# Ryan-Faulkner/Simultaneous-Diffusion-for-Pointclouds

Hardware: AMD Instinct MI355X
Metric: Langevin denoising steps/sec on 64×1024 range images, 1/2/4/8 MI355X (higher is better)
Workload: dtype fp32x3; 1 GPU; Line.yml simultaneous sampling step (score-net fwd + Langevin update + consistency merge), 64x1024x2 range images; views_per_gpu=4, megabatch_views=4, mode=viewsplit, conv_arithmetic=fp32x3, parallelism=views1

## Files before the change

### include/sdp.h

```cpp
#ifndef SDP_H
#define SDP_H

#include <stddef.h>
#include <stdint.h>

#ifdef __cplusplus
extern "C" {
#endif

#define SDP_VERSION 100

enum sdp_precision {
  SDP_PREC_FP32 = 0,
  SDP_PREC_FP32X3 = 1,
  SDP_PREC_BF16 = 2
};

typedef struct sdp_net_desc {
  int ngf;
  int channels;
  int H, W;
  int num_classes;
  int precision;
} sdp_net_desc;

typedef struct sdp_net sdp_net;

int sdp_version(void);
const char* sdp_last_error(void);

int sdp_net_create(const sdp_net_desc* desc, sdp_net** out);
int sdp_net_set_param(sdp_net* net, const char* key, const float* host_data, const int64_t* shape, int ndim);
int sdp_net_finalize(sdp_net* net);
int sdp_net_workspace_size(const sdp_net* net, int B, size_t* bytes);
int sdp_net_forward(sdp_net* net, const float* x, const int64_t* labels, float* out, int B,
                    void* workspace, size_t workspace_bytes, void* stream);
int sdp_net_destroy(sdp_net* net);
typedef struct {
  const float* ref;
  const int32_t* mask;
  const float* noise;
  uint64_t seed, offset;
  float step_size, noise_scale, grad_ref;
  int nan_to_num;
  float* lik_out;
  uint32_t* absmax_bits;
  float* grad_out;
} sdp_langevin_params;
int sdp_net_forward_langevin(sdp_net* net, float* x, const int64_t* labels, int B, const sdp_langevin_params* params,
                             void* workspace, size_t workspace_bytes, void* stream);
int sdp_net_set_split(sdp_net* net, int ways);
int sdp_net_profile_enable(sdp_net* net, int enable);
int sdp_net_profile_read(sdp_net* net, char* buf, size_t cap, int* n_launches);

int sdp_net_param_arena_floats(const sdp_net* net, size_t* n);
int sdp_net_param_count(const sdp_net* net, int* n);
int sdp_net_param_info(const sdp_net* net, int i, char* key, size_t cap, size_t* offset, size_t* numel);
int sdp_net_bind_params(sdp_net* net, float* arena, void* stream);
int sdp_net_repack(sdp_net* net, void* stream);

int sdp_net_train_workspace_size(sdp_net* net, int B, size_t* bytes);
int sdp_net_set_tape(sdp_net* net, int bf16);
int sdp_net_forward_train(sdp_net* net, const float* x, const int64_t* labels, float* out, int B,
                          void* workspace, size_t workspace_bytes, void* stream);
int sdp_net_backward(sdp_net* net, const float* dscore, int B, void* workspace, size_t workspace_bytes,
                     float* grads, void* stream);
int sdp_net_backward_buckets(sdp_net* net, const float* dscore, int B, void* workspace, size_t workspace_bytes,
                             float* grads, int n_buckets, const size_t* bucket_end, void* const* events,
                             void* stream);
int sdp_dsm_loss(const float* score, const float* noise, const float* mask, const float* used_sigma, int B,
                 int n_img, float anneal_power, float* dscore, float* loss, float* loss_per, float* part,
                 void* stream);
int sdp_adam_ema_step(float* params, const float* grads, float* exp_avg, float* exp_avg_sq, float* ema_shadow,
                      size_t n, double lr, double beta1, double beta2, double eps, int step, double ema_mu,
                      void* stream);
enum sdp_optim_kind { SDP_OPTIM_ADAM = 0, SDP_OPTIM_RMSPROP = 1, SDP_OPTIM_SGD = 2 };
int sdp_optim_ema_step(int kind, float* params, const float* grads, float* state0, float* state1, float* state2,
                       float* ema_shadow, size_t n, double lr, double beta1, double beta2, double eps,
                       double weight_decay, int step, double ema_mu, void* stream);

int sdp_langevin_step(float* x, const float* grad, const float* ref, const int32_t* mask,
                      const float* noise_or_null, uint64_t seed, uint64_t offset,
                      float step_size, float noise_scale, float grad_ref, int nan_to_num,
                      int B, int C, int HW, float* lik_out, uint32_t* absmax_bits, void* stream);
int sdp_axpy_step(float* x, const float* g, float a, const float* lik, const int32_t* mask,
                  const float* ref, float b, int n, void* stream);

enum sdp_merge_variant { SDP_MERGE_POSES = 0, SDP_MERGE_ORIGINS = 1 };

typedef struct sdp_merge_params {
  int variant;
  int setting;
  float sigma;
  float allowance;
  float cc;
} sdp_merge_params;

int sdp_merge_workspace_size(int n_src, int n_out, int H, int W, size_t* bytes);
int sdp_merge_workspace_bytes(int n_src, int aB, int n_out, int H, int W, size_t* bytes);
int sdp_consistency_merge(float* x_all, int n_src, int aB, int o_begin, int n_out, int H, int W,
                          const double* toWorld, const double* fromWorld, const float* origins,
                          const uint8_t* exist, const uint8_t* sky, const int32_t* refmask,
                          const sdp_merge_params* params, const uint32_t* absmax_bits,
                          float* new_images, void* workspace, size_t workspace_bytes, void* stream);
int sdp_consistency_merge_ev(float* x_all, int n_src, int aB, int o_begin, int n_out, int H, int W,
                             const double* toWorld, const double* fromWorld, const float* origins,
                             const uint8_t* exist, const uint8_t* sky, const int32_t* refmask,
                             const sdp_merge_params* params, const uint32_t* absmax_bits,
                             float* new_images, void* workspace, size_t workspace_bytes, void* stream,
                             void* absmax_event);

int sdp_range_project_workspace_size(int H, int W, size_t* bytes);
int sdp_range_project(const double* points, int N, int stride, int has_intensity, const double* origin,
                      int H, int W, double* depth, double* intensity, uint8_t* obfuscation, uint8_t* sky,
                      int64_t* index, void* workspace, size_t workspace_bytes, void* stream);

enum sdp_view_variant { SDP_VIEW_8BATCH = 0, SDP_VIEW_ALLFORONE = 1, SDP_VIEW_DENSIFICATION = 2, SDP_VIEW_COMPLETION = 3 };
int sdp_view_transform(const float* points, int64_t n, const double* m1, const double* m2, double* out, void* stream);
int sdp_view_gather(const int64_t* index, int H, int W, int blank_cols, const float* points, double* out, int* count,
                    void* stream);
int sdp_view_finalize(const double* depth, const double* intensity, const uint8_t* obfuscation, const uint8_t* sky,
                      const double* goal_depth, const double* goal_intensity, int H, int W, int channels, int roll,
                      int variant, int first_view, double* real, uint8_t* notmask, uint8_t* notsky, double* goal,
                      void* stream);

int sdp_grid_subsample(const float* points, int64_t n, const float* features, int fdim, const int32_t* classes,
                       int ldim, float sample_dl, int method, float* out_points, float* out_features,
                       int32_t* out_classes, int64_t* out_n);

#ifdef __cplusplus
}
#endif
#endif
```

### simultaneous-diffusion-for-pointclouds_amd/csrc/aux.hip

```cpp
#include "common.h"
#include "langevin.h"

namespace sdp {

SDP_DEV float linspace01(int i, int n) {
  if (n == 1) return 0.f;
  const float step = 1.0f / (float)(n - 1);
  return i < n / 2 ? step * (float)i : 1.0f - step * (float)(n - 1 - i);
}

SDP_DEV float wave_sum(float v) {
#pragma unroll
  for (int o = 32; o > 0; o >>= 1) v += __shfl_xor(v, o);
  return v;
}

typedef float f32x2v __attribute__((ext_vector_type(2)));
typedef float f32x4v __attribute__((ext_vector_type(4)));
constexpr int BC_TP = 128, BC_RS = 132;
#ifndef SDP_BC_KO
#define SDP_BC_KO 0
#endif
constexpr int BC_WG_PER_CU = 3;
__global__ __launch_bounds__(256, BC_WG_PER_CU) void begin_conv_kernel(const float* __restrict__ x, const float* __restrict__ w,
// ... 619 lines not shown
      } else {
        if (out) *reinterpret_cast<float4*>(out + e) = g4;
        float4 l;
        const float4 o = langevin_group(lg, e / 4, g4, l);
        reinterpret_cast<float4*>(lg.x)[e / 4] = o;
        if (lg.lik) reinterpret_cast<float4*>(lg.lik)[e / 4] = l;
        if (co == 0) lmax = max(lmax, absmax4(o));
      }
    }
  }
  if constexpr (LGV) {
    if (lg.absmax) block_absmax<4>(lmax, lg.absmax);
  }
}

constexpr int INPP_CPB = 8, INPP_G = 1024 / INPP_CPB;
__global__ __launch_bounds__(1024) void inpp_moments_kernel(const float2* __restrict__ stats, int T, float cnt, int C,
                                                            double2* __restrict__ mv) {
  __shared__ double red[1024];
  const int tid = threadIdx.x, l = tid % INPP_CPB, g = tid / INPP_CPB;
  const int nb = C / INPP_CPB;
  const int b = blockIdx.x / nb, c = (blockIdx.x % nb) * INPP_CPB + l;
  const float2* st = stats + (size_t)b * T * C + c;
  auto group_sum = [&](double v) {
    red[tid] = v;
    __syncthreads();
    for (int s = INPP_G / 2; s > 0; s >>= 1) {
      if (g < s) red[tid] += red[tid + s * INPP_CPB];
      __syncthreads();
    }
    const double r = red[l];
    __syncthreads();
    return r;
  };
  double sm = 0.0;
  for (int t = g; t < T; t += INPP_G) sm += st[(size_t)t * C].x;
  const double mean = group_sum(sm) / T;
  double m2 = 0.0;
  for (int t = g; t < T; t += INPP_G) {
    const float2 v = st[(size_t)t * C];
    const double dm = (double)v.x - mean;
    m2 += (double)v.y + dm * dm * cnt;
  }
  m2 = group_sum(m2);
  if (g == 0) mv[(size_t)b * C + c] = make_double2(mean, m2 / ((double)T * cnt));
}

__global__ __launch_bounds__(1024) void inpp_ss_kernel(const double2* __restrict__ mv, int C,
                                                       const float* __restrict__ alpha, const float* __restrict__ gamma,
                                                       const float* __restrict__ beta, float2* __restrict__ ss,
                                                       float4* __restrict__ nst) {
  __shared__ double red[1024];
  const int b = blockIdx.x, c = threadIdx.x;
  const double2 m_v = mv[(size_t)b * C + c];
  const double mean = m_v.x, var = m_v.y;
  red[c] = mean;
  __syncthreads();
  for (int s = C / 2; s > 0; s >>= 1) {
    if (c < s) red[c] += red[c + s];
    __syncthreads();
  }
  const double m = red[0] / C;
  __syncthreads();
  red[c] = (mean - m) * (mean - m);
  __syncthreads();
  for (int s = C / 2; s > 0; s >>= 1) {
    if (c < s) red[c] += red[c + s];
    __syncthreads();
  }
  const double v = red[0] / (C - 1);
  const double inv = 1.0 / sqrt(var + 1e-5);
  const double mn = (mean - m) / sqrt(v + 1e-5);
  const double gm = gamma[c];
  const double scale = gm * inv;
  const double shift = gm * (-mean * inv + mn * (double)alpha[c]) + (double)beta[c];
  ss[(size_t)b * C + c] = make_float2((float)scale, (float)shift);
  if (nst) nst[(size_t)b * C + c] = make_float4((float)mean, (float)inv, (float)mn, (float)(1.0 / sqrt(v + 1e-5)));
}

#ifndef SDP_MP_MIN_BLOCKS
#define SDP_MP_MIN_BLOCKS 512
#endif
constexpr int MP_COLS = 8, MP_NS = 6, MP_D = 2, MP_MIN_BLOCKS = SDP_MP_MIN_BLOCKS;
template <bool IDX>
__global__ __launch_bounds__(256) void maxpool5_kernel(const float* __restrict__ in, float* __restrict__ out,
                                                       uchar4* __restrict__ idx, int B, int H, int W, int C,
                                                       int rows) {
  constexpr int SC = MP_COLS + 4;
  constexpr int NUNIT = SC * 32;
  static_assert(NUNIT == 384 && MP_NS >= MP_D + 1 && 4 + MP_D <= MP_NS, "maxpool5 ring layout");
  __shared__ __attribute__((aligned(16))) float4 row_buf[MP_NS][NUNIT];
  const int tid = threadIdx.x, c4 = tid & 31, xl = tid >> 5;
  const int wave = tid >> 6;
  const int C4 = C / 4, CG = C4 / 32;
  const int strips = W / MP_COLS, RB = (H + rows - 1) / rows;
  const int nwg = gridDim.x;
  int t = (nwg & 7) ? (int)blockIdx.x : ((int)blockIdx.x & 7) * (nwg >> 3) + ((int)blockIdx.x >> 3);
  const int cg = t % CG;
  t /= CG;
  const int strip = t % strips;
  t /= strips;
  const int rb = t % RB, b = t / RB;
  const int x0 = strip * MP_COLS, y0 = rb * rows, y1 = min(H, y0 + rows);
  const int x = x0 + xl;
  const float NEG = -INFINITY;
  const i32x4 rs = buffer_desc(in + (size_t)b * H * W * C, (uint32_t)H * W * C * 4);
  const uint32_t ring = (uint32_t)reinterpret_cast<uintptr_t>(&row_buf[0][0]);
  int colo[2];
  bool colok[2];
#pragma unroll
  for (int k = 0; k < 2; ++k) {
    const int i = tid + k * 256, xx = x0 - 2 + (i >> 5);
    colok[k] = xx >= 0 && xx < W;
    colo[k] = ((min(max(xx, 0), W - 1) * C4) + cg * 32 + (i & 31)) * 16;
  }
  auto dma_row = [&](int yy, int slot) {
    const int rowo = min(max(yy, 0), H - 1) * W * C4 * 16;
#pragma unroll
    for (int k = 0; k < 2; ++k) {
      if (k == 1 && wave >= 2) break;
      dma16_lds_opaque(rs, ring + (slot * NUNIT + (tid & ~63) + k * 256) * 16, colo[k], rowo);
    }
  };
  auto pad_row = [&](int yy, int slot) {
    if constexpr (IDX) {
      const bool rowok = yy >= 0 && yy < H;
#pragma unroll
      for (int k = 0; k < 2; ++k)
        if ((k == 0 || wave < 2) && !(rowok && colok[k])) row_buf[slot][tid + k * 256] = make_float4(NEG, NEG, NEG, NEG);
    }
  };
  auto hmax = [&](int slot, float4& m, uchar4& c) {
    m = make_float4(NEG, NEG, NEG, NEG);
    c = make_uchar4(2, 2, 2, 2);
#pragma unroll
    for (int dx = 0; dx < 5; ++dx) {
      const float4 v = row_buf[slot][(xl + dx) * 32 + c4];
      const unsigned char k = (unsigned char)dx;
      if (v.x > m.x) { m.x = v.x; c.x = k; }
      if (v.y > m.y) { m.y = v.y; c.y = k; }
      if (v.z > m.z) { m.z = v.z; c.z = k; }
      if (v.w > m.w) { m.w = v.w; c.w = k; }
    }
  };
  float4 hm[5];
  uchar4 hc[5];
#pragma unroll
  for (int ri = 0; ri < 4 + MP_D; ++ri) dma_row(y0 - 2 + ri, ri);
  __builtin_amdgcn_s_waitcnt(0x0f70);
#pragma unroll
  for (int ri = 0; ri < 4 + MP_D; ++ri) pad_row(y0 - 2 + ri, ri);
  __syncthreads();
#pragma unroll
  for (int k = 0; k < 4; ++k) hmax(k, hm[k], hc[k]);
  constexpr int S = IDX ? 2 : 1;
  constexpr int WAIT01 = S + (MP_D - 1) * (2 + S), WAIT23 = S + (MP_D - 1) * (1 + S);
  static_assert(WAIT01 < 64, "vmcnt field");
  for (int y = y0; y < y1; ++y) {
    const int j = y - y0;
    const int slot = (j + 4) % MP_NS;
    if (wave < 2) __builtin_amdgcn_s_waitcnt(0x0f70 | (WAIT01 & 15) | ((WAIT01 >> 4) << 14));
    else __builtin_amdgcn_s_waitcnt(0x0f70 | (WAIT23 & 15) | ((WAIT23 >> 4) << 14));
    if (j >= MP_D) pad_row(y + 2, slot);
    __syncthreads();
    hmax(slot, hm[4], hc[4]);
    dma_row(y + 2 + MP_D, (j + 4 + MP_D) % MP_NS);
    float4 m = hm[0];
    uchar4 bi = hc[0];
#pragma unroll
    for (int r = 1; r < 5; ++r) {
      const unsigned char ro = (unsigned char)(5 * r);
      if (hm[r].x > m.x) { m.x = hm[r].x; bi.x = ro + hc[r].x; }
      if (hm[r].y > m.y) { m.y = hm[r].y; bi.y = ro + hc[r].y; }
      if (hm[r].z > m.z) { m.z = hm[r].z; bi.z = ro + hc[r].z; }
      if (hm[r].w > m.w) { m.w = hm[r].w; bi.w = ro + hc[r].w; }
    }
    const size_t o = (((size_t)b * H + y) * W + x) * C4 + cg * 32 + c4;
    reinterpret_cast<float4*>(out)[o] = m;
    if constexpr (IDX) idx[o] = bi;
#pragma unroll
    for (int r = 0; r < 4; ++r) {
      hm[r] = hm[r + 1];
      hc[r] = hc[r + 1];
    }
  }
  __builtin_amdgcn_s_waitcnt(0x0f70);
}

constexpr int MPH_COLS = 16, MPH_SC = MPH_COLS + 4, MPH_U = MPH_SC * 16;
__global__ __launch_bounds__(256) void maxpool5_h16_kernel(const __bf16* __restrict__ in, __bf16* __restrict__ out,
                                                           unsigned char* __restrict__ idx, int B, int H, int W, int C,
                                                           int rows) {
  __shared__ uint4 srow[2][MPH_U];
  const int tid = threadIdx.x, c8 = tid & 15, xl = tid >> 4;
  const int CG = C / 128, strips = W / MPH_COLS, RB = (H + rows - 1) / rows;
  int t = blockIdx.x;
  const int cg = t % CG;
  t /= CG;
  const int strip = t % strips;
  t /= strips;
  const int rb = t % RB, b = t / RB;
  const int x0 = strip * MPH_COLS, y0 = rb * rows, y1 = min(H, y0 + rows);
  constexpr uint32_t NEG2 = 0xff80ff80u;
  uint4 pre[2];
  auto fetch = [&](int yy) {
#pragma unroll
    for (int k = 0; k < 2; ++k) {
      const int i = tid + 256 * k, col = i >> 4, cc = i & 15, xx = x0 - 2 + col;
      pre[k] = make_uint4(NEG2, NEG2, NEG2, NEG2);
      if (i < MPH_U && yy >= 0 && yy < H && xx >= 0 && xx < W)
        pre[k] = *reinterpret_cast<const uint4*>(in + (((size_t)b * H + yy) * W + xx) * C + cg * 128 + cc * 8);
    }
  };
  auto put = [&](int slot) {
#pragma unroll
    for (int k = 0; k < 2; ++k) {
      const int i = tid + 256 * k;
      if (i < MPH_U) srow[slot][i] = pre[k];
    }
  };
  auto hmax = [&](int slot, float (&m)[8], unsigned char (&c)[8]) {
#pragma unroll
    for (int e = 0; e < 8; ++e) {
      m[e] = -INFINITY;
      c[e] = 2;
    }
#pragma unroll
    for (int dx = 0; dx < 5; ++dx) {
      const uint4 u = srow[slot][(xl + dx) * 16 + c8];
      const float4 lo = bf4_to_f4(make_uint2(u.x, u.y)), hi = bf4_to_f4(make_uint2(u.z, u.w));
      const float v[8] = {lo.x, lo.y, lo.z, lo.w, hi.x, hi.y, hi.z, hi.w};
#pragma unroll
      for (int e = 0; e < 8; ++e)
        if (v[e] > m[e]) {
          m[e] = v[e];
          c[e] = (unsigned char)dx;
        }
    }
  };
  float hm[5][8];
  unsigned char hc[5][8];
  fetch(y0 - 2);
#pragma unroll
  for (int r = 0; r < 5; ++r) {
    __syncthreads();
    put(r & 1);
    fetch(y0 - 1 + r);
    __syncthreads();
    if (r < 4) hmax(r & 1, hm[r], hc[r]);
  }
  int slot = 0;
  for (int y = y0; y < y1; ++y) {
    hmax(slot, hm[4], hc[4]);
    __syncthreads();
    slot ^= 1;
    put(slot);
    fetch(y + 4);
    float m[8];
    unsigned char bi[8];
#pragma unroll
    for (int e = 0; e < 8; ++e) {
// ... 39 lines not shown
  }
  if (mode != MODE_F32 && !SDP_HEAD_DIRECT) {
    const dim3 grid(std::min(ntiles, 256 * BM_WG_PER_CU));
    if (mode == MODE_F32X3)
      hipLaunchKernelGGL(begin_conv_mfma_kernel<MODE_F32X3>, grid, dim3(256), 0, st, x, w, bias, out, stats, B, H, W);
    else
      hipLaunchKernelGGL(begin_conv_mfma_kernel<MODE_BF16>, grid, dim3(256), 0, st, x, w, bias, out, stats, B, H, W);
    return hipGetLastError();
  }
  hipLaunchKernelGGL(begin_conv_kernel, dim3(std::min(ntiles, 256 * BC_WG_PER_CU)), dim3(256), 0, st, x, w, bias, out,
                     stats, B, H, W);
  return hipGetLastError();
}

hipError_t end_conv(const float* in, const float* ss, const float* w, const float* bias, const float* sigmas,
                    const int64_t* labels, float* out, int B, int H, int W, int Cin, hipStream_t st,
                    const LangevinArgs* lg, int mode, bool h16) {
  if (Cin != EC_CIN) return hipErrorInvalidValue;
  if (h16) {
    if (mode != MODE_BF16 || lg || H % E2_TR || W % E2_TC) return hipErrorInvalidValue;
    hipLaunchKernelGGL((end_conv_mfma_kernel<MODE_BF16, false, __bf16>), dim3(B * (H / E2_TR) * (W / E2_TC)), dim3(256), 0, st,
                       reinterpret_cast<const __bf16*>(in), ss, w, bias, sigmas, labels, out, H, W, LangevinArgs{});
    return hipGetLastError();
  }
  if (mode != MODE_F32 && !SDP_HEAD_DIRECT && H % E2_TR == 0 && W % E2_TC == 0) {
    const dim3 grid(B * (H / E2_TR) * (W / E2_TC));
    const LangevinArgs la = lg ? *lg : LangevinArgs{};
    if (mode == MODE_F32X3) {
      if (lg) hipLaunchKernelGGL((end_conv_mfma_kernel<MODE_F32X3, true>), grid, dim3(256), 0, st, in, ss, w, bias, sigmas, labels, out, H, W, la);
      else hipLaunchKernelGGL((end_conv_mfma_kernel<MODE_F32X3, false>), grid, dim3(256), 0, st, in, ss, w, bias, sigmas, labels, out, H, W, la);
    } else {
      if (lg) hipLaunchKernelGGL((end_conv_mfma_kernel<MODE_BF16, true>), grid, dim3(256), 0, st, in, ss, w, bias, sigmas, labels, out, H, W, la);
      else hipLaunchKernelGGL((end_conv_mfma_kernel<MODE_BF16, false>), grid, dim3(256), 0, st, in, ss, w, bias, sigmas, labels, out, H, W, la);
    }
    return hipGetLastError();
  }
  if (H % 4 || W % 64) return hipErrorInvalidValue;
  const dim3 grid(B * (H / 4) * (W / 64));
  if (lg)
    hipLaunchKernelGGL(end_conv_kernel<true>, grid, dim3(256), 0, st, in, ss, w, bias, sigmas, labels, out, H, W, *lg);
  else
    hipLaunchKernelGGL(end_conv_kernel<false>, grid, dim3(256), 0, st, in, ss, w, bias, sigmas, labels, out, H, W,
                       LangevinArgs{});
  return hipGetLastError();
}

hipError_t inpp_finalize(const float* stats, int B, int T, float cnt, int C, const float* alpha, const float* gamma,
                         const float* beta, float* ss, hipStream_t st, float* nst, void* scratch) {
  if (C % 64 || C > 1024 || (C & (C - 1))) return hipErrorInvalidValue;
  double2* mv = reinterpret_cast<double2*>(scratch);
  hipLaunchKernelGGL(inpp_moments_kernel, dim3(B * (C / INPP_CPB)), dim3(1024), 0, st,
                     reinterpret_cast<const float2*>(stats), T, cnt, C, mv);
  hipLaunchKernelGGL(inpp_ss_kernel, dim3(B), dim3(C), 0, st, mv, C, alpha, gamma, beta, reinterpret_cast<float2*>(ss),
                     reinterpret_cast<float4*>(nst));
  return hipGetLastError();
}

__global__ __launch_bounds__(256) void avgpool2_kernel(const float4* __restrict__ in, float4* __restrict__ out, int H,
                                                       int W, int C4, size_t n4) {
  const int Ho = H / 2, Wo = W / 2;
  for (size_t i = blockIdx.x * (size_t)blockDim.x + threadIdx.x; i < n4; i += (size_t)gridDim.x * blockDim.x) {
    const int c = (int)(i % C4);
    size_t p = i / C4;
    const int x = (int)(p % Wo);
    p /= Wo;
    const int y = (int)(p % Ho);
    const size_t b = p / Ho;
    const size_t r0 = ((b * H + 2 * y) * W + 2 * x) * C4 + c, r1 = r0 + (size_t)W * C4;
    const float4 a00 = in[r0], a01 = in[r0 + C4], a10 = in[r1], a11 = in[r1 + C4];
    out[i] = make_float4((((a00.x + a10.x) + a01.x) + a11.x) / 4.0f, (((a00.y + a10.y) + a01.y) + a11.y) / 4.0f,
                         (((a00.z + a10.z) + a01.z) + a11.z) / 4.0f, (((a00.w + a10.w) + a01.w) + a11.w) / 4.0f);
  }
}

hipError_t avgpool2(const float* in, float* out, int B, int H, int W, int C, hipStream_t st) {
  if ((H & 1) || (W & 1) || (C & 3)) return hipErrorInvalidValue;
  const size_t n4 = (size_t)B * (H / 2) * (W / 2) * (C / 4);
  const int grid = (int)std::min<size_t>((n4 + 255) / 256, 256 * 32);
  hipLaunchKernelGGL(avgpool2_kernel, dim3(grid), dim3(256), 0, st, reinterpret_cast<const float4*>(in),
                     reinterpret_cast<float4*>(out), H, W, C / 4, n4);
  return hipGetLastError();
}

hipError_t maxpool5(const float* in, float* out, int B, int H, int W, int C, hipStream_t st, uint8_t* idx, bool h16) {
  if (C % 128 || W % MP_COLS) return hipErrorInvalidValue;
  if (h16) {
    if (W % MPH_COLS) return hipErrorInvalidValue;
    auto hb = [&](int rows) { return B * ((H + rows - 1) / rows) * (W / MPH_COLS) * (C / 128); };
    const int rows = hb(32) >= 1024 ? 32 : (hb(16) >= 1024 ? 16 : 8), grid = hb(rows);
    hipLaunchKernelGGL(maxpool5_h16_kernel, dim3(grid), dim3(256), 0, st, reinterpret_cast<const __bf16*>(in),
                       reinterpret_cast<__bf16*>(out), idx, B, H, W, C, rows);
    return hipGetLastError();
  }
  auto blocks = [&](int rows) { return B * ((H + rows - 1) / rows) * (W / MP_COLS) * (C / 128); };
  const int rows = blocks(32) >= MP_MIN_BLOCKS ? 32 : 16, grid = blocks(rows);
  if (idx)
    hipLaunchKernelGGL(maxpool5_kernel<true>, dim3(grid), dim3(256), 0, st, in, out, reinterpret_cast<uchar4*>(idx), B, H,
                       W, C, rows);
  else
    hipLaunchKernelGGL(maxpool5_kernel<false>, dim3(grid), dim3(256), 0, st, in, out, nullptr, B, H, W, C, rows);
  return hipGetLastError();
}

}
```

### simultaneous-diffusion-for-pointclouds_amd/csrc/common.h

```cpp
#pragma once
#include <hip/hip_runtime.h>
#include <stdint.h>
#include <stdlib.h>

#include <type_traits>

#define SDP_DEV __device__ __forceinline__

typedef __attribute__((ext_vector_type(8))) __bf16 bf16x8;
typedef __attribute__((ext_vector_type(4))) __bf16 bf16x4;
typedef __attribute__((ext_vector_type(16))) float f32x16;
typedef __attribute__((ext_vector_type(4))) float f32x4;

namespace sdp {

template <int B, int E, class F>
SDP_DEV void static_for(F&& f) {
  if constexpr (B < E) {
    f(std::integral_constant<int, B>{});
    static_for<B + 1, E>(f);
  }
}

enum { MODE_F32 = 0, MODE_F32X3 = 1, MODE_BF16 = 2 };
enum { PRO_NONE = 0, PRO_ELU = 1, PRO_AFFINE_ELU = 2 };

typedef __attribute__((ext_vector_type(4))) int i32x4;
SDP_DEV i32x4 buffer_desc(const void* base, uint32_t bytes) {
  const uint64_t p = reinterpret_cast<uint64_t>(base);
  return i32x4{__builtin_amdgcn_readfirstlane((int)(uint32_t)p), __builtin_amdgcn_readfirstlane((int)((p >> 32) & 0xffff)),
               __builtin_amdgcn_readfirstlane((int)bytes), 0x00020000};
}
SDP_DEV void dma16_lds_opaque(i32x4 rsrc, uint32_t lds_byte, int voff, int soff) {
  asm volatile("s_mov_b32 m0, %0\n\ts_nop 0\n\tbuffer_load_dwordx4 %1, %2, %3 offen lds"
               :
               : "s"(__builtin_amdgcn_readfirstlane((int)lds_byte)), "v"(voff), "s"(rsrc),
                 "s"(__builtin_amdgcn_readfirstlane(soff))
               : "memory");
}

SDP_DEV float4 ldg4(const float* p, size_t i) { return *reinterpret_cast<const float4*>(p + i); }
SDP_DEV float4 bf4_to_f4(uint2 u) {
  return make_float4(__uint_as_float(u.x << 16), __uint_as_float(u.x & 0xffff0000u), __uint_as_float(u.y << 16),
                     __uint_as_float(u.y & 0xffff0000u));
}
SDP_DEV float4 ldg4(const __bf16* p, size_t i) { return bf4_to_f4(*reinterpret_cast<const uint2*>(p + i)); }
SDP_DEV uint32_t pack_bf2(float a, float b) {
  typedef __attribute__((ext_vector_type(2))) __bf16 bf16x2_t;
  const bf16x2_t v = {(__bf16)a, (__bf16)b};
  return __builtin_bit_cast(uint32_t, v);
}
SDP_DEV uint2 f4_to_bf4(float4 v) { return make_uint2(pack_bf2(v.x, v.y), pack_bf2(v.z, v.w)); }
SDP_DEV void stg4(float* p, size_t i, float4 v) { *reinterpret_cast<float4*>(p + i) = v; }
SDP_DEV void stg4(__bf16* p, size_t i, float4 v) { *reinterpret_cast<uint2*>(p + i) = f4_to_bf4(v); }
SDP_DEV float ldg1(const float* p, size_t i) { return p[i]; }
SDP_DEV float ldg1(const __bf16* p, size_t i) { return (float)p[i]; }

SDP_DEV float elu(float x) { return x > 0.f ? x : (__expf(x) - 1.0f); }
SDP_DEV float elu_max(float x) { return fmaxf(x, __expf(fminf(x, 0.f)) - 1.0f); }
SDP_DEV float elu_grad(float t, int form) {
  if (form == 2) return t > 0.f ? 1.f : t + 1.f;
  return t > 0.f ? 1.f : __expf(t);
}

struct ConvArgs {
  const float* in;
  const uint4* wf;
  const uint4* wf16;
  const float* bias;
  float* out;
  const float* res;
  float* out2;
  const float* res2;
  const float* up;
  const float* pro_ss;
  int ss_bstride;
  float* stats;
  int B, H, W, Cin, Cout;
  int dil, circular, pro_mode, epi_elu;
  int tiles_per_img;
  int strip_w;
  int groups_per_img;
  int cpair;
  unsigned long long* dbg;
  const float* aux;
  const float* epi_ss;
  int dact;
  int io16;
  int s2;
};

struct WgradArgs {
  const float* in;
  const float* pro_ss;
  int ss_bstride;
  int pro_mode;
  const float* dy;
  float* part;
  size_t part_floats;
  float* bpart;
  int B, H, W, Cin, Cout, dil, circular;
};

inline int conv_strip_w(int tile_rows, int tile_cols) {
  int sw = 1;
  while (sw * 2 * tile_rows <= 32 && tile_cols % (sw * 2) == 0) sw *= 2;
  return sw;
}
// ... 3 lines not shown
```

### simultaneous-diffusion-for-pointclouds_amd/csrc/conv.hip

```cpp
#include "conv_launch.h"

namespace sdp {

#ifndef SDP_CONV_NJ2
#define SDP_CONV_NJ2 1
#endif
#ifndef SDP_CONV_NJ2_BF16_W8
#define SDP_CONV_NJ2_BF16_W8 1
#endif

template <int MODE, bool PELU>
static hipError_t launch_elu(const ConvArgs& a, int ks, bool pool, int wm, int tc, bool half, hipStream_t st) {
  if (ks == 1)
    return pool ? conv_launch<MODE, 1, 64, 1, true, PELU>(a, st) : conv_launch<MODE, 1, 64, 1, false, PELU>(a, st);
  if (pool) return conv_launch<MODE, 1, 64, 3, true, PELU>(a, st);
  if constexpr (MODE != MODE_F32) {
    if (half) return SDP_CONV_NJ2 ? conv_launch_nj2<MODE, PELU, 4>(a, st) : conv_launch_half<MODE, PELU>(a, st);
    if (tc == 16) {
      if (!SDP_CONV_NJ2) return conv_launch<MODE, 1, 16, 3, false, PELU>(a, st);
      return (MODE == MODE_BF16 && SDP_CONV_NJ2_BF16_W8) ? conv_launch_nj2<MODE, PELU, 8>(a, st)
                                                         : conv_launch_nj2<MODE, PELU, 4>(a, st);
    }
  }
  if (wm == 2) return conv_launch<MODE, 2, 32, 3, false, PELU>(a, st);
  return tc == 64 ? conv_launch<MODE, 1, 64, 3, false, PELU>(a, st) : conv_launch<MODE, 1, 32, 3, false, PELU>(a, st);
}

template <int MODE>
static hipError_t launch_mode(const ConvArgs& a, int ks, bool pool, int wm, int tc, hipStream_t st, bool half = false) {
#ifdef SDP_CONV_BENCH_ONLY
  if constexpr (MODE != MODE_F32) {
    if (half) return SDP_CONV_NJ2 ? conv_launch_nj2<MODE, true, 4>(a, st) : conv_launch_half<MODE, true>(a, st);
    if (!SDP_CONV_NJ2) return conv_launch<MODE, 1, 16, 3, false, true>(a, st);
    return (MODE == MODE_BF16 && SDP_CONV_NJ2_BF16_W8) ? conv_launch_nj2<MODE, true, 8>(a, st)
                                                       : conv_launch_nj2<MODE, true, 4>(a, st);
  }
  if (wm == 2) return conv_launch<MODE, 2, 32, 3, false, true>(a, st);
  return conv_launch<MODE, 1, 32, 3, false, true>(a, st);
#else
  return a.pro_mode == PRO_NONE ? launch_elu<MODE, false>(a, ks, pool, wm, tc, half, st)
                                : launch_elu<MODE, true>(a, ks, pool, wm, tc, half, st);
#endif
}

hipError_t conv_mfma(int mode, ConvArgs a, int ks, bool pool, hipStream_t st, const char** why) {
  const int d = a.dil;
  if (a.Cin % 64 || a.Cout % 128) { *why = "conv: Cin%64 and Cout%128 required"; return hipErrorInvalidValue; }
  if (a.H % d || a.W % d) { *why = "conv: H,W must be multiples of the dilation"; return hipErrorInvalidValue; }
  const int Hs = a.H / d, Ws = a.W / d;
  const int wm = (a.Cout % 256 == 0) ? 1 : 2;
  const bool sh16 = mode != MODE_F32;
  int tc;
  if (sh16 && Ws % 16 == 0 && Hs % 8 == 0) tc = 16;
  else if (wm == 2) tc = 32;
  else tc = (Ws % 32 == 0 && Hs % 4 == 0) ? 32 : 64;
  if (!sh16 && tc == 16) tc = 32;
  if (ks == 1 || pool) tc = 64;
  const bool half = sh16 && wm == 2 && tc == 16 && ks == 3 && !pool;
  const int tr = (half ? 128 : wm * 128) / tc;
  if (Ws % tc || Hs % tr) { *why = "conv: sub-grid not divisible by the pixel tile"; return hipErrorInvalidValue; }
  if (sh16 && !a.wf16) { *why = "conv: bf16 modes need the 16x16 weight packing (#frag16)"; return hipErrorInvalidValue; }
  if (!sh16 && !a.wf) { *why = "conv: exact fp32 needs the 32x32 weight packing (#frag)"; return hipErrorInvalidValue; }
  if (ks == 1 && !pool && (d != 1 || wm != 1)) { *why = "conv: 1x1 needs d=1 and 256-multiple Cout"; return hipErrorInvalidValue; }
  if (pool && (d != 1 || wm != 1 || (a.H & 1) || (a.W & 1))) {
    *why = "conv: pooling needs d=1, even H,W and 256-multiple Cout";
    return hipErrorInvalidValue;
  }
  if (a.up && ((a.H & 1) || (a.W & 1) || a.H < 2 || a.W < 2)) { *why = "conv: upsample needs even H,W"; return hipErrorInvalidValue; }
  if (!a.circular && d != 1) { *why = "conv: zero padding only for d=1"; return hipErrorInvalidValue; }
  if (!a.pro_ss) { *why = "conv: prologue scale/shift table missing"; return hipErrorInvalidValue; }
  if (a.Cin > 1024 && a.ss_bstride == 0) { *why = "conv: identity table holds 1024 channels"; return hipErrorInvalidValue; }
  if (a.s2) {
    if (!sh16 || a.io16 || ks != 3 || pool || d != 1 || a.circular || a.up || a.pro_mode == PRO_NONE || a.dact ||
        (a.H % 16) || (a.W % 32)) {
      *why = "conv: the 4x4 stride-2 form needs a bf16 mode, a zero-padded 3x3 with an ELU prologue, H%16 and W%32";
      return hipErrorInvalidValue;
    }
#ifndef SDP_CONV_BENCH_ONLY
    return mode == MODE_F32X3 ? conv_launch_s2<MODE_F32X3>(a, st) : conv_launch_s2<MODE_BF16>(a, st);
#else
    *why = "conv: the 4x4 stride-2 form is not built into conv_bench";
    return hipErrorInvalidValue;
#endif
  }
  if (a.io16) {
#ifdef SDP_CONV_BENCH_ONLY
    if (mode == MODE_BF16 && ks == 3 && tc == 16 && !pool) return conv_launch_nj2<MODE_BF16, true, 4, true>(a, st);
#else
    if (mode != MODE_BF16) { *why = "conv: bf16 tensors (io16) need bf16 mode"; return hipErrorInvalidValue; }
    const bool pe = a.pro_mode != PRO_NONE;
    if (pool && ks == 1) return pe ? conv_launch<MODE_BF16, 1, 64, 1, true, true, true>(a, st)
                                   : conv_launch<MODE_BF16, 1, 64, 1, true, false, true>(a, st);
    if (pool) return pe ? conv_launch<MODE_BF16, 1, 64, 3, true, true, true>(a, st)
                        : conv_launch<MODE_BF16, 1, 64, 3, true, false, true>(a, st);
    if (ks == 3 && tc == 16)
      return pe ? conv_launch_nj2<MODE_BF16, true, 4, true>(a, st) : conv_launch_nj2<MODE_BF16, false, 4, true>(a, st);
#endif
    *why = "conv: no bf16-tensor (io16) kernel for this shape";
    return hipErrorInvalidValue;
  }
  switch (mode) {
    case MODE_F32: return launch_mode<MODE_F32>(a, ks, pool, wm, tc, st);
    case MODE_F32X3: return launch_mode<MODE_F32X3>(a, ks, pool, wm, tc, st, half);
    default: return launch_mode<MODE_BF16>(a, ks, pool, wm, tc, st, half);
  }
}

}
```

### simultaneous-diffusion-for-pointclouds_amd/csrc/conv_inst.hip

```cpp
#include "conv_kernel.h"
#include "conv_launch.h"

namespace sdp {


#ifndef SDP_FWD_TRN
#define SDP_FWD_TRN 0
#endif

#ifndef SDP_CONV_CPAIR
#define SDP_CONV_CPAIR 1
#endif

#ifndef SDP_NJ2_STRIP
#define SDP_NJ2_STRIP 1
#endif

template <int MODE, int WM, int TC, int KS, bool POOL, bool PELU, bool IO16>
hipError_t conv_launch(ConvArgs a, hipStream_t st) {
  using T = ConvTile<WM, TC, KS, 4, 4, IO16>;
  a.tiles_per_img = a.H * a.W / (T::TR * TC);
  a.groups_per_img = a.H * a.W / 128;
  a.strip_w = conv_strip_w(a.H / a.dil / T::TR, a.W / a.dil / TC);
  dim3 grid(a.B * a.tiles_per_img, a.Cout / T::NTILE);
  if constexpr (MODE != MODE_F32) {
    hipLaunchKernelGGL((conv_mfma_kernel<MODE, WM, TC, KS, POOL, POOL, PELU, 16, 4, (SDP_FWD_TRN && TC == 16 && !POOL), 4, IO16>),
                       grid, dim3(256), 0, st, a);
    return hipGetLastError();
  } else if constexpr (TC >= 32) {
    hipLaunchKernelGGL((conv_mfma_kernel<MODE, WM, TC, KS, POOL, POOL, PELU>), grid, dim3(256), 0, st, a);
    return hipGetLastError();
  }
  return hipErrorInvalidValue;
}

template <int MODE, bool PELU>
hipError_t conv_launch_half(ConvArgs a, hipStream_t st) {
  using T = ConvTile<1, 16, 3, 2>;
  a.tiles_per_img = a.H * a.W / (T::TR * 16);
  a.groups_per_img = a.H * a.W / 128;
  a.strip_w = 0;
  dim3 grid(a.B * a.tiles_per_img, a.Cout / T::NTILE);
  hipLaunchKernelGGL((conv_mfma_kernel<MODE, 1, 16, 3, false, false, PELU, 16, 2, (SDP_FWD_TRN != 0)>), grid,
                     dim3(T::NTH), 0, st, a);
  return hipGetLastError();
}

template <int MODE, bool PELU, int NW, bool IO16>
hipError_t conv_launch_nj2(ConvArgs a, hipStream_t st) {
  using T = ConvTile<1, 16, 3, NW, 2, IO16>;
  a.tiles_per_img = a.H * a.W / (T::TR * 16);
  a.groups_per_img = a.H * a.W / 128;
  a.cpair = (SDP_CONV_CPAIR && a.Cout == 2 * T::NTILE) ? 1 : 0;
  const bool strip = NW == 8 || SDP_NJ2_STRIP == 2 || (SDP_NJ2_STRIP == 1 && a.cpair);
  a.strip_w = strip ? conv_strip_w(a.H / a.dil / T::TR, a.W / a.dil / 16) : 0;
  dim3 grid(a.B * a.tiles_per_img * (a.cpair ? 2 : 1), a.cpair ? 1 : a.Cout / T::NTILE);
  hipLaunchKernelGGL((conv_mfma_kernel<MODE, 1, 16, 3, false, false, PELU, 16, NW, false, 2, IO16>), grid, dim3(T::NTH), 0,
                     st, a);
  return hipGetLastError();
}

template <int MODE>
hipError_t conv_launch_s2(ConvArgs a, hipStream_t st) {
  using T = ConvTile<1, 16, 3, 4, 2>;
  const int Ho = a.H / 2, Wo = a.W / 2;
  a.tiles_per_img = Ho * Wo / (T::TR * 16);
  a.groups_per_img = Ho * Wo / 128;
  a.cpair = (SDP_CONV_CPAIR && a.Cout == 2 * T::NTILE) ? 1 : 0;
  a.strip_w = a.cpair ? conv_strip_w(Ho / T::TR, Wo / 16) : 0;
  dim3 grid(a.B * a.tiles_per_img * (a.cpair ? 2 : 1), a.cpair ? 1 : a.Cout / T::NTILE);
  hipLaunchKernelGGL((conv_mfma_kernel<MODE, 1, 16, 3, false, true, true, 16, 4, false, 2, false, true>), grid, dim3(T::NTH),
                     0, st, a);
  return hipGetLastError();
}

template <int MODE, int WM, int TC, int KS, bool ZP, bool IO16>
hipError_t dgrad_launch(ConvArgs a, hipStream_t st) {
  using T = ConvTile<WM, TC, KS, 4, 4, IO16>;
  a.tiles_per_img = a.H * a.W / (T::TR * TC);
  a.groups_per_img = a.H * a.W / 128;
  dim3 grid(a.B * a.tiles_per_img, a.Cout / T::NTILE);
  if constexpr (TC < 32) {
    hipLaunchKernelGGL((conv_mfma_kernel<MODE, WM, TC, KS, false, ZP, false, 16, 4, true, 4, IO16>), grid, dim3(256), 0, st, a);
  } else {
    hipLaunchKernelGGL((conv_mfma_kernel<MODE, WM, TC, KS, false, ZP, false, 16, 4, false, 4, IO16>), grid, dim3(256), 0, st, a);
  }
  return hipGetLastError();
}

template <int S> struct FwdShape;
template <> struct FwdShape<0> { static constexpr int WM = 1, TC = 64, KS = 1; static constexpr bool POOL = true; };
template <> struct FwdShape<1> { static constexpr int WM = 1, TC = 64, KS = 3; static constexpr bool POOL = true; };
template <> struct FwdShape<2> { static constexpr int WM = 2, TC = 32, KS = 3; static constexpr bool POOL = false; };
template <> struct FwdShape<3> { static constexpr int WM = 1, TC = 64, KS = 3; static constexpr bool POOL = false; };
template <> struct FwdShape<4> { static constexpr int WM = 1, TC = 32, KS = 3; static constexpr bool POOL = false; };
template <> struct FwdShape<5> { static constexpr int WM = 1, TC = 16, KS = 3; static constexpr bool POOL = false; };
template <> struct FwdShape<8> { static constexpr int WM = 1, TC = 64, KS = 1; static constexpr bool POOL = false; };
template <int MODE>
hipError_t dgrad_launch_half(ConvArgs a, hipStream_t st) {
  using T = ConvTile<1, 16, 3, 2>;
  a.tiles_per_img = a.H * a.W / (T::TR * 16);
  a.groups_per_img = a.H * a.W / 128;
  dim3 grid(a.B * a.tiles_per_img, a.Cout / T::NTILE);
  hipLaunchKernelGGL((conv_mfma_kernel<MODE, 1, 16, 3, false, false, false, 16, 2, true>), grid, dim3(T::NTH), 0, st, a);
  return hipGetLastError();
}

template <int MODE, int NW, bool IO16>
hipError_t dgrad_launch_nj2(ConvArgs a, hipStream_t st) {
  using T = ConvTile<1, 16, 3, NW, 2, IO16>;
  a.tiles_per_img = a.H * a.W / (T::TR * 16);
  a.groups_per_img = a.H * a.W / 128;
  dim3 grid(a.B * a.tiles_per_img, a.Cout / T::NTILE);
  hipLaunchKernelGGL((conv_mfma_kernel<MODE, 1, 16, 3, false, false, false, 16, NW, true, 2, IO16>), grid, dim3(T::NTH), 0,
                     st, a);
  return hipGetLastError();
}

template <int S> struct DgradShape;
template <> struct DgradShape<0> { static constexpr int WM = 2, TC = 32, KS = 1; static constexpr bool ZP = false; };
template <> struct DgradShape<1> { static constexpr int WM = 2, TC = 32, KS = 3; static constexpr bool ZP = true; };
template <> struct DgradShape<2> { static constexpr int WM = 2, TC = 32, KS = 3; static constexpr bool ZP = false; };
template <> struct DgradShape<3> { static constexpr int WM = 1, TC = 64, KS = 3; static constexpr bool ZP = false; };
template <> struct DgradShape<4> { static constexpr int WM = 1, TC = 32, KS = 3; static constexpr bool ZP = false; };
template <> struct DgradShape<5> { static constexpr int WM = 1, TC = 16, KS = 3; static constexpr bool ZP = false; };

#if defined(SDP_INST) && SDP_INST >= 4000
static_assert(SDP_INST - 4000 == MODE_F32X3 || SDP_INST - 4000 == MODE_BF16, "SDP_INST: bad 4x4 stride-2 code");
template hipError_t conv_launch_s2<SDP_INST - 4000>(ConvArgs, hipStream_t);
#elif defined(SDP_INST) && SDP_INST >= 3000
constexpr int kS = SDP_INST % 10;
static_assert(kS == 0 || kS == 1 || kS == 7 || kS == 8, "SDP_INST: bad IO16 dgrad code");
#if SDP_INST % 10 == 0
template hipError_t dgrad_launch<MODE_BF16, 2, 32, 1, false, true>(ConvArgs, hipStream_t);
#elif SDP_INST % 10 == 1
template hipError_t dgrad_launch<MODE_BF16, 2, 32, 3, true, true>(ConvArgs, hipStream_t);
#else
template hipError_t dgrad_launch_nj2<MODE_BF16, kS == 7 ? 4 : 8, true>(ConvArgs, hipStream_t);
#endif
#elif defined(SDP_INST) && SDP_INST >= 2000
constexpr int kPelu = (SDP_INST / 10) % 10, kS = SDP_INST % 10;
static_assert(kPelu <= 1 && (kS == 0 || kS == 1 || kS == 6 || kS == 9), "SDP_INST: bad IO16 forward code");
#if SDP_INST % 10 == 0
template hipError_t conv_launch<MODE_BF16, 1, 64, 1, true, (kPelu != 0), true>(ConvArgs, hipStream_t);
#elif SDP_INST % 10 == 1
template hipError_t conv_launch<MODE_BF16, 1, 64, 3, true, (kPelu != 0), true>(ConvArgs, hipStream_t);
#else
template hipError_t conv_launch_nj2<MODE_BF16, (kPelu != 0), kS == 9 ? 4 : 8, true>(ConvArgs, hipStream_t);
#endif
#elif defined(SDP_INST) && SDP_INST < 1000 && (SDP_INST % 10 == 6 || SDP_INST % 10 == 9)
constexpr int kMode = SDP_INST / 100 - 1, kPelu = (SDP_INST / 10) % 10;
static_assert(kMode >= 1 && kMode <= 2 && kPelu <= 1, "SDP_INST: bad 32-Cout-wave forward code");
template hipError_t conv_launch_nj2<kMode, (kPelu != 0), SDP_INST % 10 == 9 ? 4 : 8>(ConvArgs, hipStream_t);
#elif defined(SDP_INST) && SDP_INST < 1000 && SDP_INST % 10 == 7
constexpr int kMode = SDP_INST / 100 - 1, kPelu = (SDP_INST / 10) % 10;
static_assert(kMode >= 1 && kMode <= 2 && kPelu <= 1, "SDP_INST: bad 2-wave forward code");
template hipError_t conv_launch_half<kMode, (kPelu != 0)>(ConvArgs, hipStream_t);
#elif defined(SDP_INST) && SDP_INST < 1000
constexpr int kMode = SDP_INST / 100 - 1, kPelu = (SDP_INST / 10) % 10, kShape = SDP_INST % 10;
static_assert(kMode >= 0 && kMode <= 2 && kPelu <= 1 && (kShape <= 5 || kShape == 8) &&
                  (kShape < 5 || kShape == 8 || kMode != MODE_F32),
              "SDP_INST: bad forward code");
using FS = FwdShape<kShape>;
template hipError_t conv_launch<kMode, FS::WM, FS::TC, FS::KS, FS::POOL, (kPelu != 0)>(ConvArgs, hipStream_t);
#elif defined(SDP_INST) && (SDP_INST % 10 == 7 || SDP_INST % 10 == 8)
constexpr int kMode = (SDP_INST / 10) % 10;
static_assert(SDP_INST / 100 == 10 && (kMode == MODE_F32X3 || kMode == MODE_BF16), "SDP_INST: bad dgrad code");
template hipError_t dgrad_launch_nj2<kMode, SDP_INST % 10 == 7 ? 4 : 8>(ConvArgs, hipStream_t);
#elif defined(SDP_INST) && SDP_INST % 10 == 6
constexpr int kMode = (SDP_INST / 10) % 10;
static_assert(SDP_INST / 100 == 10 && (kMode == MODE_F32X3 || kMode == MODE_BF16), "SDP_INST: bad dgrad code");
template hipError_t dgrad_launch_half<kMode>(ConvArgs, hipStream_t);
#elif defined(SDP_INST)
constexpr int kMode = (SDP_INST / 10) % 10, kShape = SDP_INST % 10;
static_assert(SDP_INST / 100 == 10 && (kMode == MODE_F32X3 || kMode == MODE_BF16) && kShape <= 5,
              "SDP_INST: bad dgrad code");
using DS = DgradShape<kShape>;
template hipError_t dgrad_launch<kMode, DS::WM, DS::TC, DS::KS, DS::ZP>(ConvArgs, hipStream_t);
#elif defined(SDP_CONV_BENCH_ONLY)
template hipError_t conv_launch<MODE_F32, 2, 32, 3, false, true>(ConvArgs, hipStream_t);
template hipError_t conv_launch<MODE_F32, 1, 32, 3, false, true>(ConvArgs, hipStream_t);
template hipError_t conv_launch<MODE_F32X3, 1, 16, 3, false, true>(ConvArgs, hipStream_t);
template hipError_t conv_launch<MODE_BF16, 1, 16, 3, false, true>(ConvArgs, hipStream_t);
template hipError_t conv_launch_half<MODE_F32X3, true>(ConvArgs, hipStream_t);
template hipError_t conv_launch_half<MODE_BF16, true>(ConvArgs, hipStream_t);
template hipError_t conv_launch_nj2<MODE_F32X3, true, 4>(ConvArgs, hipStream_t);
template hipError_t conv_launch_nj2<MODE_F32X3, true, 8>(ConvArgs, hipStream_t);
template hipError_t conv_launch_nj2<MODE_BF16, true, 4>(ConvArgs, hipStream_t);
template hipError_t conv_launch_nj2<MODE_BF16, true, 8>(ConvArgs, hipStream_t);
template hipError_t conv_launch_nj2<MODE_BF16, true, 4, true>(ConvArgs, hipStream_t);
template hipError_t dgrad_launch_nj2<MODE_BF16, 4, true>(ConvArgs, hipStream_t);
#else
#error "conv_inst.hip: build with -DSDP_INST=<code> (Makefile) or -DSDP_CONV_BENCH_ONLY (tools/conv_bench)"
#endif

}
```

### simultaneous-diffusion-for-pointclouds_amd/csrc/conv_kernel.h

```cpp
#pragma once
#include <type_traits>

#include "common.h"

namespace sdp {

#ifndef SDP_KO
#define SDP_KO 0
#endif

#ifndef SDP_DMA_AUX
#define SDP_DMA_AUX 0
#endif
#ifndef SDP_STORE_AUX
#define SDP_STORE_AUX 0
#endif
#ifndef SDP_STORE_AUX16
#define SDP_STORE_AUX16 SDP_STORE_AUX
#endif

#ifndef SDP_S2_RING
#define SDP_S2_RING 4
#endif

#ifdef SDP_TIMING
#define SDP_T(i) do { if (tid == 0) tclk[i] = __builtin_amdgcn_s_memtime(); } while (0)
#else
#define SDP_T(i) do { } while (0)
#endif

constexpr int PSTRIDE = 144;

template <int WM, int TC, int KS, int NW = 4, int NJ = 4, bool IO16 = false>
struct ConvTile {
  static constexpr int NTH = 64 * NW;
  static constexpr int WN = NW / WM;
  static constexpr int RW = 128 / TC;
  static constexpr int TR = WM * RW;
  static constexpr int NTILE = WN * 16 * NJ;
  static constexpr int WPC = 4 * (NJ == 2 ? 2 : 1) / NW;
  static constexpr int HALO = KS == 3 ? 1 : 0;
  static constexpr int PC = TC + 2 * HALO;
  static constexpr int PR = TR + 2 * HALO;
  static constexpr int NPIX = PR * PC;
  static constexpr int UPP = IO16 ? 4 : 8;
  static constexpr int NU = (NPIX * UPP + NTH - 1) / NTH;
  static constexpr int PATCH_BYTES = NU * (NTH / UPP) * PSTRIDE;
  static constexpr int RAW_BYTES = NU * NTH * 16;
  static constexpr int PIPE_BYTES = 2 * PATCH_BYTES + RAW_BYTES;
  static constexpr int EPI_BYTES = WM * 64 * (NTILE + 8) * 4;
  static constexpr int LDS_BYTES = PIPE_BYTES > EPI_BYTES ? PIPE_BYTES : EPI_BYTES;
  static_assert(LDS_BYTES * WPC <= 160 * 1024, "LDS budget (WPC workgroups per CU)");
};

SDP_DEV float4 ld4(const float* p) { return *reinterpret_cast<const float4*>(p); }

template <int NU, int NT, int NSTG_ = 5>
struct XformPlan {
  static constexpr int tap_of(int k) { return k * NT / NU; }
  static constexpr int first(int tap) {
    int k = 0;
    while (k < NU && tap_of(k) < tap) ++k;
    return k;
  }
  static constexpr int count(int tap) {
    int n = 0;
    for (int k = 0; k < NU; ++k) n += tap_of(k) == tap ? 1 : 0;
    return n;
  }
  static constexpr int max_count() {
    int m = 0;
    for (int t = 0; t < NT; ++t) m = count(t) > m ? count(t) : m;
    return m;
  }
  static constexpr int NSTG = NSTG_;
  static constexpr int stage_blk(int q, int Q, int NBLK) { return 2 + q * (NBLK - 2) / (Q > 0 ? Q : 1); }
};

constexpr int s2_pos(int phase, int t) {
  const int rho = phase >> 1, gamma = phase & 1;
  return ((rho ? 0 : 1) + (t >> 1)) * 3 + (gamma ? 0 : 1) + (t & 1);
}

template <int MODE, int WM, int TC, int KS, bool POOL, bool ZP, bool PELU, int SH = 32, int NW = 4, bool TRN = false,
          int NJ = 4, bool IO16 = false, bool S2 = false>
__global__ __launch_bounds__(64 * NW, NJ == 2 ? 2 : 1) void conv_mfma_kernel(ConvArgs a) {
#if defined(__HIP_DEVICE_COMPILE__)
  static_assert(!IO16 || MODE == MODE_BF16, "the bf16 tape runs in bf16 mode");
  constexpr int ES = IO16 ? 2 : 4;
  constexpr int CPU = IO16 ? 8 : 4;
  constexpr int USH = IO16 ? 2 : 3;
  constexpr int PPU = CPU / 2;
  constexpr bool COPY = IO16 && !PELU;
  static_assert((SH == 32) == (MODE == MODE_F32), "bf16 modes: 16x16 shape; exact fp32: 32x32");
  static_assert(NW == 4 || (SH == 16 && !POOL), "2-wave workgroups: the 16x16 non-pooled forward only");
  static_assert(NJ == 4 || (SH == 16 && !POOL && KS == 3 && WM == 1), "32-Cout waves: the 16x16 3x3 tiles only");
  static_assert(!S2 || (NJ == 2 && NW == 4 && TC == 16 && ZP && !TRN && !IO16), "4x4 stride-2: zero-padded 32-Cout-wave tiles");
  using T = ConvTile<WM, TC, KS, NW, NJ, IO16>;
  constexpr int NTH = T::NTH;
  constexpr int NT = S2 ? 4 : KS * KS;
  constexpr bool TRANS = TRN && SH == 16 && !POOL;
  constexpr int NU = T::NU;
  constexpr int XT = NT >= 4 ? 4 : NT;
  __shared__ __attribute__((aligned(16))) char lds[T::LDS_BYTES];
  char* const raw = lds + 2 * T::PATCH_BYTES;

  const int tid = threadIdx.x, lane = tid & 63, wave = tid >> 6;
#ifdef SDP_TIMING
  unsigned long long tclk[8] = {0, 0, 0, 0, 0, 0, 0, 0};
  unsigned long long tbar = 0;
  const unsigned long long rt0 = __builtin_amdgcn_s_memrealtime();
#endif
  SDP_T(0);
  const int wm = WM == 1 ? 0 : (wave & 1), wn = WM == 1 ? wave : (wave >> 1);
  const int d = S2 ? 2 : a.dil, Hs = a.H / d, Ws = a.W / d;
  const int tiles_c = Ws / TC, tiles_rc = (Hs / T::TR) * tiles_c;
  const int nwg = gridDim.x;
  int t = (nwg & 7) ? (int)blockIdx.x : ((int)blockIdx.x & 7) * (nwg >> 3) + ((int)blockIdx.x >> 3);
  const int cblk = a.cpair ? (t & 1) : (int)blockIdx.y;
  if (a.cpair) t >>= 1;
  const int b = t / a.tiles_per_img;
  const int tile = t - b * a.tiles_per_img;
  t = tile;
  const int ph = t / tiles_rc;
  t -= ph * tiles_rc;
  const int ph_r = ph / d, ph_c = ph - (ph / d) * d;
  int trow, tcol;
  if (a.strip_w) {
    const int R = Hs / T::TR, sw = a.strip_w;
    const int strip = t / (R * sw), w_ = t - strip * (R * sw);
    trow = w_ / sw;
    tcol = strip * sw + (w_ - trow * sw);
  } else {
    trow = t / tiles_c;
    tcol = t % tiles_c;
  }
  const int sr0 = trow * T::TR, sc0 = tcol * TC;
  const int n0 = cblk * T::NTILE;
  const int wrow0 = wm * T::RW;

  const int Cin = a.Cin, Cout = a.Cout;
  const int nck = Cin / 32;
  const int nchunks = S2 ? 4 * nck : nck;
  const int NB = Cout / 32;
  const int f0 = n0 / 16 + wn * NJ;
  const int nbg0 = f0 / 2;

  f32x16 acc[4][2];
  f32x4 acc4[8][NJ];
  if constexpr (SH == 32) {
    static_for<0, 4>([&](auto i) {
      static_for<0, 2>([&](auto j) {
#pragma unroll
        for (int r = 0; r < 16; ++r) acc[i][j][r] = 0.f;
      });
    });
  } else {
    static_for<0, 8>([&](auto i) {
      static_for<0, NJ>([&](auto j) {
#pragma unroll
        for (int r = 0; r < 4; ++r) acc4[i][j][r] = 0.f;
      });
    });
  }

  const bool c16 = SH == 16 && a.wf16 != nullptr;
  const __amdgpu_buffer_rsrc_t wrs =
      __builtin_amdgcn_make_buffer_rsrc((void*)(c16 ? a.wf16 : a.wf), 0, 0x7fffffff, 0x00020000);
  const int wv0 = ((nbg0 + 0) * 64 + lane) * 64, wv1 = ((nbg0 + 1) * 64 + lane) * 64;
  typedef __attribute__((ext_vector_type(4))) unsigned u32x4;
  constexpr int NBUF = S2 ? SDP_S2_RING : (NT % 3 == 0) ? 3 : 2;
  uint4 bq[NBUF][NJ / 2][4];
  int wq16[NJ];
  const int wlo16 = __builtin_amdgcn_readfirstlane(c16 ? 1024 : 16);
  {
    const int g = lane >> 4, h = g & 1, sg = g >> 1;
    static_for<0, NJ>([&](auto njc) {
      constexpr int nj = decltype(njc)::value;
      const int L = 16 * (nj & 1) + (lane & 15) + 32 * h;
      wq16[nj] = c16 ? ((f0 + nj) * 128 + lane) * 16 : ((nbg0 + (nj >> 1)) * 64 + L) * 64 + sg * 32;
    });
  }
  auto load_b = [&](auto buf, int chunk, int tap) __attribute__((always_inline)) {
    constexpr int J = decltype(buf)::value;
    if constexpr (SDP_KO & 4) return;
    const int so = __builtin_amdgcn_readfirstlane(((chunk * NT + tap) * NB) * 4096);
    if constexpr (SH == 32) {
      static_for<0, 4>([&](auto q) {
        const u32x4 v0 = __builtin_amdgcn_raw_buffer_load_b128(wrs, wv0 + q * 16, so, 0);
        const u32x4 v1 = __builtin_amdgcn_raw_buffer_load_b128(wrs, wv1 + q * 16, so, 0);
        bq[J][0][q] = make_uint4(v0.x, v0.y, v0.z, v0.w);
        bq[J][1][q] = make_uint4(v1.x, v1.y, v1.z, v1.w);
      });
    } else {
      static_for<0, NJ>([&](auto njc) {
        constexpr int nj = decltype(njc)::value;
        const u32x4 vh = __builtin_amdgcn_raw_buffer_load_b128(wrs, wq16[nj], so, 0);
        bq[J][nj >> 1][2 * (nj & 1)] = make_uint4(vh.x, vh.y, vh.z, vh.w);
        if constexpr (MODE != MODE_BF16) {
          const u32x4 vl = __builtin_amdgcn_raw_buffer_load_b128(wrs, wq16[nj] + wlo16, so, 0);
          bq[J][nj >> 1][2 * (nj & 1) + 1] = make_uint4(vl.x, vl.y, vl.z, vl.w);
        }
      });
    }
  };

  const char* inb = reinterpret_cast<const char*>(a.in) + (size_t)b * a.H * a.W * Cin * ES;
  const float* ssb = a.pro_ss + (size_t)b * a.ss_bstride;
  auto chunk_cc = [&](int c) __attribute__((always_inline)) {
    if constexpr (S2) return (c >= 2 * nck ? c - 2 * nck : c) >> 1;
    else return c;
  };
  auto chunk_soff = [&](int c) __attribute__((always_inline)) {
    if constexpr (S2) {
      c = min(c, nchunks - 1);
      const int rho = c >= 2 * nck ? 1 : 0, r = c - rho * 2 * nck;
      return ((rho * a.W + (r & 1)) * Cin + (r >> 1) * 32) * ES;
    } else {
      return c * 32 * ES;
    }
  };
  const int my_cv = tid & (T::UPP - 1);
  float4 ssv[2][PPU];
  auto load_ss = [&](auto buf, int chunk) __attribute__((always_inline)) {
    constexpr int SB = decltype(buf)::value;
    static_for<0, PPU>([&](auto kc) { ssv[SB][kc] = ld4(ssb + (chunk * 32 + my_cv * CPU) * 2 + 4 * decltype(kc)::value); });
  };

  const __amdgpu_buffer_rsrc_t irs =
      __builtin_amdgcn_make_buffer_rsrc((void*)inb, 0, a.H * a.W * Cin * ES, 0x00020000);
  int uoff[NU];
  unsigned uvalid = 0;
  static_for<0, NU>([&](auto kc) {
    constexpr int k = decltype(kc)::value;
    int u = tid + k * NTH;
    bool valid = u < T::NPIX * T::UPP;
    u = valid ? u : 0;
    const int pix = u >> USH, cv = u & (T::UPP - 1);
    const int pr = pix / T::PC, pc = pix - pr * T::PC;
    int sr = sr0 - T::HALO + pr, sc = sc0 - T::HALO + pc;
    if (a.circular) {
      sr = sr < 0 ? sr + Hs : (sr >= Hs ? sr - Hs : sr);
      sc = sc < 0 ? sc + Ws : (sc >= Ws ? sc - Ws : sc);
    } else {
      valid = valid && sr >= 0 && sr < Hs && sc >= 0 && sc < Ws;
      sr = min(max(sr, 0), Hs - 1);
      sc = min(max(sc, 0), Ws - 1);
    }
    const int y = sr * d + ph_r, x = sc * d + ph_c;
    uoff[k] = ((y * a.W + x) * Cin + cv * CPU) * ES;
    uvalid |= (valid ? 1u : 0u) << k;
  });
  auto load_unit = [&](auto kc, int chunk) __attribute__((always_inline)) {
    constexpr int k = decltype(kc)::value;
    if constexpr (SDP_KO & 1) return;
    const int base = __builtin_amdgcn_readfirstlane(((tid & ~63) + k * NTH) * 16);
    __builtin_amdgcn_raw_ptr_buffer_load_lds(
        irs, reinterpret_cast<__attribute__((address_space(3))) void*>(reinterpret_cast<uintptr_t>(raw + base)), 16,
        uoff[k], chunk_soff(chunk), 0, SDP_DMA_AUX);
  };
  const i32x4 irs_o = buffer_desc(inb, (uint32_t)(a.H * a.W * Cin * ES));
  auto load_unit_o = [&](auto kc, int chunk) __attribute__((always_inline)) {
    constexpr int k = decltype(kc)::value;
    if constexpr (SDP_KO & 1) return;
    const uint32_t base = (uint32_t)(uintptr_t)(raw + ((tid & ~63) + k * NTH) * 16);
    dma16_lds_opaque(irs_o, base, uoff[k], chunk_soff(chunk));
  };
  auto xform_load = [&](auto kc) __attribute__((always_inline)) {
    constexpr int k = decltype(kc)::value;
    return *reinterpret_cast<const float4*>(raw + (tid + k * NTH) * 16);
  };
  auto xform_store = [&](auto kc, auto pb, float4 v) __attribute__((always_inline)) {
    constexpr int k = decltype(kc)::value;
    constexpr int PB = decltype(pb)::value;
    const int pix = (tid + k * NTH) >> USH;
    if constexpr (COPY) {
      uint4 u = __builtin_bit_cast(uint4, v);
      if constexpr (ZP) {
        if (!((uvalid >> k) & 1u)) u = make_uint4(0u, 0u, 0u, 0u);
      }
      *reinterpret_cast<uint4*>(lds + PB * T::PATCH_BYTES + pix * PSTRIDE + my_cv * 16) = u;
      return;
    }
    if constexpr (IO16) {
      const uint4 u = __builtin_bit_cast(uint4, v);
      const float4 lo = bf4_to_f4(make_uint2(u.x, u.y)), hi = bf4_to_f4(make_uint2(u.z, u.w));
      float x8[8] = {lo.x, lo.y, lo.z, lo.w, hi.x, hi.y, hi.z, hi.w};
#pragma unroll
      for (int e = 0; e < 8; ++e) {
        const float4 sv = ssv[PB][e >> 1];
        x8[e] = fmaf(x8[e], (e & 1) ? sv.z : sv.x, (e & 1) ? sv.w : sv.y);
        if constexpr (PELU) x8[e] = elu_max(x8[e]);
        if constexpr (ZP) {
          if (!((uvalid >> k) & 1u)) x8[e] = 0.f;
        }
      }
      *reinterpret_cast<uint4*>(lds + PB * T::PATCH_BYTES + pix * PSTRIDE + my_cv * 16) =
          make_uint4(pack_bf2(x8[0], x8[1]), pack_bf2(x8[2], x8[3]), pack_bf2(x8[4], x8[5]), pack_bf2(x8[6], x8[7]));
      return;
    }
    const float4 ssv0 = ssv[PB][0], ssv1 = ssv[PB][1];
    v.x = fmaf(v.x, ssv0.x, ssv0.y);
    v.y = fmaf(v.y, ssv0.z, ssv0.w);
    v.z = fmaf(v.z, ssv1.x, ssv1.y);
    v.w = fmaf(v.w, ssv1.z, ssv1.w);
    if constexpr (PELU) {
      v.x = elu_max(v.x); v.y = elu_max(v.y); v.z = elu_max(v.z); v.w = elu_max(v.w);
    }
    if constexpr (ZP) {
      if (!((uvalid >> k) & 1u)) v = make_float4(0.f, 0.f, 0.f, 0.f);
    }
    char* dst = lds + PB * T::PATCH_BYTES + pix * PSTRIDE;
    if constexpr (MODE == MODE_F32) {
      *reinterpret_cast<float4*>(dst + my_cv * 16) = v;
    } else {
      bf16x4 hi;
      hi[0] = (__bf16)v.x; hi[1] = (__bf16)v.y; hi[2] = (__bf16)v.z; hi[3] = (__bf16)v.w;
      *reinterpret_cast<bf16x4*>(dst + my_cv * 8) = hi;
      if constexpr (MODE == MODE_F32X3) {
        bf16x4 lo;
        lo[0] = (__bf16)(v.x - (float)hi[0]);
        lo[1] = (__bf16)(v.y - (float)hi[1]);
        lo[2] = (__bf16)(v.z - (float)hi[2]);
        lo[3] = (__bf16)(v.w - (float)hi[3]);
        *reinterpret_cast<bf16x4*>(dst + 64 + my_cv * 8) = lo;
      }
    }
  };
  auto xform_unit = [&](auto kc, auto pb) __attribute__((always_inline)) { xform_store(kc, pb, xform_load(kc)); };
  auto xform_piece = [&](auto kc, auto hc, auto pb, float4 v4) __attribute__((always_inline)) {
    constexpr int k = decltype(kc)::value, h = decltype(hc)::value, PB = decltype(pb)::value;
    if constexpr (SDP_KO & 2) return;
    const int pix = (tid + k * NTH) >> USH;
    float x0, x1;
    if constexpr (IO16) {
      const uint32_t w = __float_as_uint(h == 0 ? v4.x : h == 1 ? v4.y : h == 2 ? v4.z : v4.w);
      x0 = __uint_as_float(w << 16);
      x1 = __uint_as_float(w & 0xffff0000u);
    } else {
      x0 = h ? v4.z : v4.x;
      x1 = h ? v4.w : v4.y;
    }
    const float4 sv = ssv[PB][h];
    x0 = fmaf(x0, sv.x, sv.y);
    x1 = fmaf(x1, sv.z, sv.w);
    if constexpr (PELU) {
      x0 = elu_max(x0);
      x1 = elu_max(x1);
    }
    if constexpr (ZP) {
      const bool ok = (uvalid >> k) & 1u;
      x0 = ok ? x0 : 0.f;
      x1 = ok ? x1 : 0.f;
    }
    typedef __attribute__((ext_vector_type(2))) __bf16 bf16x2;
    bf16x2 hi;
    hi[0] = (__bf16)x0;
    hi[1] = (__bf16)x1;
    char* dst = lds + PB * T::PATCH_BYTES + pix * PSTRIDE + my_cv * (2 * CPU) + h * 4;
    *reinterpret_cast<bf16x2*>(dst) = hi;
    if constexpr (MODE == MODE_F32X3) {
      bf16x2 lo;
      lo[0] = (__bf16)(x0 - (float)hi[0]);
      lo[1] = (__bf16)(x1 - (float)hi[1]);
      *reinterpret_cast<bf16x2*>(dst + 64) = lo;
    }
  };

  SDP_T(1);
  load_b(std::integral_constant<int, 0>{}, 0, 0);
  static_for<1, NBUF - 1>([&](auto j) { load_b(j, 0, decltype(j)::value); });
  load_ss(std::integral_constant<int, 0>{}, 0);
  static_for<0, NU>([&](auto k) { load_unit(k, 0); });
  static_for<0, NU>([&](auto k) { xform_unit(k, std::integral_constant<int, 0>{}); });
  if (nchunks > 1) {
    load_ss(std::integral_constant<int, 1>{}, chunk_cc(1));
    static_for<0, NU>([&](auto k) { load_unit(k, 1); });
  }
  __syncthreads();
  SDP_T(2);

  const int a_lane_off16 = (lane & 15) * PSTRIDE + (lane >> 4) * 16;
  auto read_a = [&](const char* pat, auto tap_c, auto s_c, bf16x8* hi, bf16x8* lo) __attribute__((always_inline)) {
    constexpr int tap = decltype(tap_c)::value, s = decltype(s_c)::value;
    constexpr int kh = (KS == 3) ? tap / 3 : 0, kw = (KS == 3) ? tap % 3 : 0;
    static_for<0, 4>([&](auto mbc) {
      constexpr int i = decltype(mbc)::value, mb = 4 * s + i;
      constexpr int mr = mb / (TC / 16), mc = (mb % (TC / 16)) * 16;
      const char* src = pat + ((wrow0 + mr + kh) * T::PC + mc + kw) * PSTRIDE + a_lane_off16;
      hi[i] = *reinterpret_cast<const bf16x8*>(src);
      if constexpr (MODE == MODE_F32X3) lo[i] = *reinterpret_cast<const bf16x8*>(src + 64);
    });
  };

  auto do_chunk = [&](auto parity, int chunk) __attribute__((always_inline)) {
    constexpr int P = decltype(parity)::value;
    const char* pat = lds + P * T::PATCH_BYTES;
    bf16x8 pre_hi[4], pre_lo[4];
    if constexpr (MODE != MODE_F32) read_a(pat, std::integral_constant<int, 0>{}, std::integral_constant<int, 0>{},
                                           pre_hi, pre_lo);
    static_for<0, NT>([&](auto tap_c) {
      constexpr int tap = decltype(tap_c)::value;
      constexpr int DIST = NBUF - 1;
      constexpr int CUR = NBUF >= 3 ? tap % NBUF : (tap + P) & 1;
      constexpr int NXT = NBUF >= 3 ? (tap + DIST) % NBUF : (tap + 1 + P) & 1;
      if constexpr (tap + DIST < NT) load_b(std::integral_constant<int, NXT>{}, chunk, tap + DIST);
      else load_b(std::integral_constant<int, NXT>{}, min(chunk + 1, nchunks - 1), tap + DIST - NT);
      __builtin_amdgcn_sched_barrier(0);
      constexpr int NX = (tap < XT) ? (NU - tap + XT - 1) / XT : 0;
      float4 xv[NX > 0 ? NX : 1];
      auto xform_loads = [&]() __attribute__((always_inline)) {
        static_for<0, NX>([&](auto j) { xv[j] = xform_load(std::integral_constant<int, tap + XT * j>{}); });
      };
      auto xform_stores = [&]() __attribute__((always_inline)) {
        static_for<0, NX>([&](auto j) {
          xform_store(std::integral_constant<int, tap + XT * j>{}, std::integral_constant<int, 1 - P>{}, xv[j]);
        });
      };
      auto dmas = [&]() __attribute__((always_inline)) {
        if constexpr (tap == NT - 1) load_ss(std::integral_constant<int, P>{}, min(chunk + 2, nchunks - 1));
        static_for<0, NU>([&](auto kc) {
          constexpr int dt = NT > XT ? XT : 0;
          if constexpr (dt == tap) load_unit(kc, chunk + 2);
        });
      };
      if constexpr (MODE == MODE_F32) {
        xform_loads();
        xform_stores();
        if constexpr (NT == 1) __builtin_amdgcn_sched_barrier(0);
        dmas();
        const int kh = (KS == 3) ? tap / 3 : 0, kw = (KS == 3) ? tap % 3 : 0;
#pragma unroll
        for (int half = 0; half < 2; ++half) {
          float av[4][8];
          static_for<0, 4>([&](auto mbc) {
            constexpr int mb = decltype(mbc)::value;
            constexpr int mr = mb / (TC / 32), mc = (mb % (TC / 32)) * 32;
            const int pix = (wrow0 + mr + kh) * T::PC + mc + (lane & 31) + kw;
            const char* src = pat + pix * PSTRIDE + (lane >> 5) * 64 + half * 32;
            const float4 f0 = *reinterpret_cast<const float4*>(src);
            const float4 f1 = *reinterpret_cast<const float4*>(src + 16);
            av[mb][0] = f0.x; av[mb][1] = f0.y; av[mb][2] = f0.z; av[mb][3] = f0.w;
            av[mb][4] = f1.x; av[mb][5] = f1.y; av[mb][6] = f1.z; av[mb][7] = f1.w;
          });
#pragma unroll
          for (int kk = 0; kk < 8; ++kk) {
            const int k = half * 8 + kk;
            static_for<0, 2>([&](auto nbc) {
              constexpr int nb = decltype(nbc)::value;
              const uint4 bv = bq[CUR][nb][k >> 2];
              const uint32_t bw = (k & 3) == 0 ? bv.x : (k & 3) == 1 ? bv.y : (k & 3) == 2 ? bv.z : bv.w;
              const float bf = __uint_as_float(bw);
              static_for<0, 4>([&](auto mbc) {
                constexpr int mb = decltype(mbc)::value;
                acc[mb][nb] = __builtin_amdgcn_mfma_f32_32x32x2f32(av[mb][kk], bf, acc[mb][nb], 0, 0, 0);
              });
            });
          }
        }
      } else {
        float4 xv[NX > 0 ? NX : 1];
        static_for<0, NX>([&](auto j) { xv[j] = xform_load(std::integral_constant<int, tap + XT * j>{}); });
        bf16x8 c0_hi[4], c0_lo[4], c1_hi[4], c1_lo[4];
        static_for<0, 4>([&](auto mb) {
          c0_hi[mb] = pre_hi[mb];
          if constexpr (MODE == MODE_F32X3) c0_lo[mb] = pre_lo[mb];
        });
        read_a(pat, tap_c, std::integral_constant<int, 1>{}, c1_hi, c1_lo);
        if constexpr (tap + 1 < NT)
          read_a(pat, std::integral_constant<int, tap + 1>{}, std::integral_constant<int, 0>{}, pre_hi, pre_lo);
        if constexpr (NT > 1) dmas();
        constexpr int NBLK = 8 * NJ;
        static_for<0, NBLK>([&](auto blk_c) {
          constexpr int blk = decltype(blk_c)::value;
          {
            constexpr int s = blk / (4 * NJ), nj = (blk / 4) % NJ, i = blk & 3, mb = 4 * s + i;
            const uint4 h4 = bq[CUR][nj >> 1][2 * (nj & 1)], l4 = bq[CUR][nj >> 1][2 * (nj & 1) + 1];
            const bf16x8 bhi = *reinterpret_cast<const bf16x8*>(&h4);
            const bf16x8 blo = *reinterpret_cast<const bf16x8*>(&l4);
            const bf16x8 ahi = s == 0 ? c0_hi[i] : c1_hi[i];
            if constexpr (TRANS) {
              if constexpr (MODE == MODE_F32X3) {
                const bf16x8 alo = s == 0 ? c0_lo[i] : c1_lo[i];
                acc4[mb][nj] = __builtin_amdgcn_mfma_f32_16x16x32_bf16(bhi, alo, acc4[mb][nj], 0, 0, 0);
                acc4[mb][nj] = __builtin_amdgcn_mfma_f32_16x16x32_bf16(blo, ahi, acc4[mb][nj], 0, 0, 0);
              }
              acc4[mb][nj] = __builtin_amdgcn_mfma_f32_16x16x32_bf16(bhi, ahi, acc4[mb][nj], 0, 0, 0);
            } else {
              if constexpr (MODE == MODE_F32X3) {
                const bf16x8 alo = s == 0 ? c0_lo[i] : c1_lo[i];
                acc4[mb][nj] = __builtin_amdgcn_mfma_f32_16x16x32_bf16(alo, bhi, acc4[mb][nj], 0, 0, 0);
                acc4[mb][nj] = __builtin_amdgcn_mfma_f32_16x16x32_bf16(ahi, blo, acc4[mb][nj], 0, 0, 0);
              }
              acc4[mb][nj] = __builtin_amdgcn_mfma_f32_16x16x32_bf16(ahi, bhi, acc4[mb][nj], 0, 0, 0);
            }
          }
          if constexpr (COPY) {
            if constexpr (blk < NX) xform_store(std::integral_constant<int, tap + XT * blk>{}, std::integral_constant<int, 1 - P>{},
                                                xv[blk]);
          } else if constexpr (blk < PPU * NX) {
            xform_piece(std::integral_constant<int, tap + XT * (blk / PPU)>{}, std::integral_constant<int, blk % PPU>{},
                        std::integral_constant<int, 1 - P>{}, xv[blk / PPU]);
          }
          __builtin_amdgcn_sched_barrier(0);
        });
        if constexpr (NT == 1) dmas();
      }
    });
#ifdef SDP_TIMING
    const unsigned long long tb0 = __builtin_amdgcn_s_memtime();
#endif
    __builtin_amdgcn_s_waitcnt(0xc07f);
    if constexpr (!(SDP_KO & 8)) __builtin_amdgcn_s_barrier();
#ifdef SDP_TIMING
    tbar += __builtin_amdgcn_s_memtime() - tb0;
#endif
  };
  using XP = XformPlan<NU, NT, (MODE == MODE_BF16 && !IO16 && !S2) ? 8 : 5>;
  constexpr int NQ = MODE == MODE_F32X3 ? 8 : 4;
  constexpr int NWL = NJ * (MODE == MODE_F32X3 ? 2 : 1);
  constexpr int NBLK = 8 * NJ;
  static_assert(NQ <= NBLK / 2 && 2 * NWL <= NBLK, "the tap's fillers fit its blocks");
  using I0 = std::integral_constant<int, 0>;
  using I1 = std::integral_constant<int, 1>;
  auto read_a1 = [&](const char* pat, auto pos_c, auto s_c, auto i_c, auto lo_c) __attribute__((always_inline)) {
    constexpr int pos = decltype(pos_c)::value, s = decltype(s_c)::value, i = decltype(i_c)::value;
    constexpr int kh = pos / 3, kw = pos % 3, mb = 4 * s + i;
    constexpr int mr = mb / (TC / 16), mc = (mb % (TC / 16)) * 16;
    return *reinterpret_cast<const bf16x8*>(pat + ((wrow0 + mr + kh) * T::PC + mc + kw) * PSTRIDE + a_lane_off16 +
                                            (decltype(lo_c)::value ? 64 : 0));
  };
  auto load_b1 = [&](auto buf, auto q_c, int chunk, int tap) __attribute__((always_inline)) {
    constexpr int J = decltype(buf)::value, q = decltype(q_c)::value;
    constexpr int nj = MODE == MODE_F32X3 ? (q >> 1) : q, part = MODE == MODE_F32X3 ? (q & 1) : 0;
    if constexpr (SDP_KO & 4) return;
    const int so = __builtin_amdgcn_readfirstlane(((chunk * NT + tap) * NB) * 4096 + (part ? wlo16 : 0));
    const u32x4 v = __builtin_amdgcn_raw_buffer_load_b128(wrs, wq16[nj], so, 0);
    bq[J][nj >> 1][2 * (nj & 1) + part] = make_uint4(v.x, v.y, v.z, v.w);
  };
  auto do_chunk9 = [&](auto parity, auto phase_c, int chunk) __attribute__((always_inline)) {
    constexpr int P = decltype(parity)::value, PHS = decltype(phase_c)::value;
    const char* pat = lds + P * T::PATCH_BYTES;
    bf16x8 ca[2][4], cb[2][4];
    static_for<0, 4>([&](auto i) {
      using POS0 = std::integral_constant<int, S2 ? s2_pos(PHS, 0) : 0>;
      ca[0][i] = read_a1(pat, POS0{}, I0{}, i, I0{});
      if constexpr (MODE == MODE_F32X3) ca[1][i] = read_a1(pat, POS0{}, I0{}, i, I1{});
    });
    load_ss(std::integral_constant<int, P>{}, chunk_cc(min(chunk + 2, nchunks - 1)));
    static_for<0, NT>([&](auto tap_c) {
      constexpr int tap = decltype(tap_c)::value;
      constexpr int DIST = NBUF - 1;
      constexpr int CUR = tap % NBUF, NXT = (tap + DIST) % NBUF;
      using POS = std::integral_constant<int, S2 ? s2_pos(PHS, tap) : tap>;
      using POSN = std::integral_constant<int, S2 ? s2_pos(PHS, tap + 1 < NT ? tap + 1 : 0) : tap + 1>;
      constexpr int U0 = XP::first(tap), UN = XP::count(tap), Q = COPY ? UN : UN * PPU * XP::NSTG;
      constexpr int UNA = UN > 0 ? UN : 1;
      const int wchunk = tap + DIST < NT ? chunk : min(chunk + 1, nchunks - 1);
      constexpr int wtap = tap + DIST < NT ? tap + DIST : tap + DIST - NT;
      float4 xr[UNA];
      float py0[PPU * UNA], py1[PPU * UNA], pe0[PPU * UNA], pe1[PPU * UNA];
      uint32_t phi[PPU * UNA], plo[PPU * UNA];
      auto stage = [&](auto pc_c, auto st_c) __attribute__((always_inline)) {
        constexpr int pc = decltype(pc_c)::value, st = decltype(st_c)::value;
        constexpr int j = pc / PPU, h = pc % PPU, k = U0 + j, PB = 1 - P;
        if constexpr (SDP_KO & 2) return;
        if constexpr (COPY) {
          xform_store(std::integral_constant<int, U0 + decltype(pc_c)::value>{}, std::integral_constant<int, PB>{},
                      xr[decltype(pc_c)::value]);
          return;
        }
        auto raw2 = [&](float& r0, float& r1) __attribute__((always_inline)) {
          const float4 v = xr[j];
          if constexpr (IO16) {
            const uint32_t w = __float_as_uint(h == 0 ? v.x : h == 1 ? v.y : h == 2 ? v.z : v.w);
            r0 = __uint_as_float(w << 16);
            r1 = __uint_as_float(w & 0xffff0000u);
          } else {
            r0 = h ? v.z : v.x;
            r1 = h ? v.w : v.y;
          }
        };
        if constexpr (XP::NSTG == 8) {
          const float4 v = xr[j];
          const float4 sv = ssv[PB][h];
          if constexpr (st == 0) {
            py0[pc] = fmaf(h ? v.z : v.x, sv.x, sv.y);
            if constexpr (PELU) pe0[pc] = fminf(py0[pc], 0.f);
          } else if constexpr (st == 1) {
            py1[pc] = fmaf(h ? v.w : v.y, sv.z, sv.w);
            if constexpr (PELU) pe1[pc] = fminf(py1[pc], 0.f);
          } else if constexpr (st == 2) {
            if constexpr (PELU) pe0[pc] = __expf(pe0[pc]);
          } else if constexpr (st == 3) {
            if constexpr (PELU) pe1[pc] = __expf(pe1[pc]);
          } else if constexpr (st == 4) {
            if constexpr (PELU) py0[pc] = fmaxf(py0[pc], pe0[pc] - 1.0f);
            if constexpr (ZP) py0[pc] = ((uvalid >> k) & 1u) ? py0[pc] : 0.f;
          } else if constexpr (st == 5) {
            if constexpr (PELU) py1[pc] = fmaxf(py1[pc], pe1[pc] - 1.0f);
            if constexpr (ZP) py1[pc] = ((uvalid >> k) & 1u) ? py1[pc] : 0.f;
          } else if constexpr (st == 6) {
            typedef __attribute__((ext_vector_type(2))) __bf16 bf16x2;
            bf16x2 hi;
            hi[0] = (__bf16)py0[pc];
            hi[1] = (__bf16)py1[pc];
            phi[pc] = *reinterpret_cast<const uint32_t*>(&hi);
          } else {
            const int pix = (tid + k * NTH) >> 3;
            *reinterpret_cast<uint32_t*>(lds + PB * T::PATCH_BYTES + pix * PSTRIDE + my_cv * 8 + h * 4) = phi[pc];
          }
          return;
        }
        if constexpr (st == 0) {
          float r0, r1;
          raw2(r0, r1);
          const float4 sv = ssv[PB][h];
          py0[pc] = fmaf(r0, sv.x, sv.y);
          py1[pc] = fmaf(r1, sv.z, sv.w);
          if constexpr (PELU) {
            pe0[pc] = fminf(py0[pc], 0.f);
            pe1[pc] = fminf(py1[pc], 0.f);
          }
        } else if constexpr (st == 1) {
          if constexpr (PELU) {
            pe0[pc] = __expf(pe0[pc]);
            pe1[pc] = __expf(pe1[pc]);
          }
        } else if constexpr (st == 2) {
          if constexpr (PELU) {
            py0[pc] = fmaxf(py0[pc], pe0[pc] - 1.0f);
            py1[pc] = fmaxf(py1[pc], pe1[pc] - 1.0f);
          }
          if constexpr (ZP) {
            const bool ok = (uvalid >> k) & 1u;
            py0[pc] = ok ? py0[pc] : 0.f;
            py1[pc] = ok ? py1[pc] : 0.f;
          }
        } else if constexpr (st == 3) {
          typedef __attribute__((ext_vector_type(2))) __bf16 bf16x2;
          bf16x2 hi;
          hi[0] = (__bf16)py0[pc];
          hi[1] = (__bf16)py1[pc];
          phi[pc] = *reinterpret_cast<const uint32_t*>(&hi);
          if constexpr (MODE == MODE_F32X3) {
            bf16x2 lo;
            lo[0] = (__bf16)(py0[pc] - (float)hi[0]);
            lo[1] = (__bf16)(py1[pc] - (float)hi[1]);
            plo[pc] = *reinterpret_cast<const uint32_t*>(&lo);
          }
        } else {
          const int pix = (tid + k * NTH) >> USH;
          char* dst = lds + PB * T::PATCH_BYTES + pix * PSTRIDE + my_cv * (2 * CPU) + h * 4;
          *reinterpret_cast<uint32_t*>(dst) = phi[pc];
          if constexpr (MODE == MODE_F32X3) *reinterpret_cast<uint32_t*>(dst + 64) = plo[pc];
        }
      };
      static_for<0, NBLK>([&](auto blk_c) {
        constexpr int blk = decltype(blk_c)::value;
        constexpr int s = blk / (4 * NJ), nj = (blk / 4) % NJ, i = blk & 3, mb = 4 * s + i;
        if constexpr (blk < UN) xr[blk] = xform_load(std::integral_constant<int, U0 + blk>{});
        {
          const uint4 h4 = bq[CUR][nj >> 1][2 * (nj & 1)], l4 = bq[CUR][nj >> 1][2 * (nj & 1) + 1];
          const bf16x8 bhi = *reinterpret_cast<const bf16x8*>(&h4);
          const bf16x8 blo = *reinterpret_cast<const bf16x8*>(&l4);
          const bf16x8 ahi = s == 0 ? ca[0][i] : cb[0][i];
          if constexpr (TRANS) {
            if constexpr (MODE == MODE_F32X3) {
              const bf16x8 alo = s == 0 ? ca[1][i] : cb[1][i];
              acc4[mb][nj] = __builtin_amdgcn_mfma_f32_16x16x32_bf16(bhi, alo, acc4[mb][nj], 0, 0, 0);
              acc4[mb][nj] = __builtin_amdgcn_mfma_f32_16x16x32_bf16(blo, ahi, acc4[mb][nj], 0, 0, 0);
            }
            acc4[mb][nj] = __builtin_amdgcn_mfma_f32_16x16x32_bf16(bhi, ahi, acc4[mb][nj], 0, 0, 0);
          } else {
            if constexpr (MODE == MODE_F32X3) {
              const bf16x8 alo = s == 0 ? ca[1][i] : cb[1][i];
              acc4[mb][nj] = __builtin_amdgcn_mfma_f32_16x16x32_bf16(alo, bhi, acc4[mb][nj], 0, 0, 0);
              acc4[mb][nj] = __builtin_amdgcn_mfma_f32_16x16x32_bf16(ahi, blo, acc4[mb][nj], 0, 0, 0);
            }
            acc4[mb][nj] = __builtin_amdgcn_mfma_f32_16x16x32_bf16(ahi, bhi, acc4[mb][nj], 0, 0, 0);
          }
        }
        if constexpr (blk < NQ) {
          constexpr int q = blk, ii = MODE == MODE_F32X3 ? (q >> 1) : q, lo = MODE == MODE_F32X3 ? (q & 1) : 0;
          cb[lo][ii] = read_a1(pat, POS{}, I1{}, std::integral_constant<int, ii>{}, std::integral_constant<int, lo>{});
        }
        if constexpr ((blk & 1) && (blk >> 1) < NWL)
          load_b1(std::integral_constant<int, NXT>{}, std::integral_constant<int, (blk >> 1)>{}, wchunk, wtap);
        if constexpr (tap + 1 < NT && blk >= NBLK / 2 && blk < NBLK / 2 + NQ) {
          constexpr int q = blk - NBLK / 2, ii = MODE == MODE_F32X3 ? (q >> 1) : q, lo = MODE == MODE_F32X3 ? (q & 1) : 0;
          ca[lo][ii] = read_a1(pat, POSN{}, I0{}, std::integral_constant<int, ii>{},
                               std::integral_constant<int, lo>{});
        }
        static_for<0, Q>([&](auto q_c) {
          constexpr int q = decltype(q_c)::value;
          if constexpr (XP::stage_blk(q, Q, NBLK) == blk) {
            if constexpr (COPY) stage(std::integral_constant<int, q>{}, std::integral_constant<int, 0>{});
            else stage(std::integral_constant<int, q / XP::NSTG>{}, std::integral_constant<int, q % XP::NSTG>{});
          }
        });
        if constexpr (UN > 0 && blk >= NBLK - UN)
          load_unit_o(std::integral_constant<int, U0 + blk - (NBLK - UN)>{}, chunk + 2);
        __builtin_amdgcn_sched_barrier(0);
      });
    });
    __builtin_amdgcn_s_waitcnt(0xc07f);
    if constexpr (!(SDP_KO & 8)) __builtin_amdgcn_s_barrier();
  };
  static_assert(NT % 2 == 1 || (S2 && NT % NBUF == 0), "weight-ring slots repeat from chunk to chunk");
#ifndef SDP_DGRAD16_TAPS
#define SDP_DGRAD16_TAPS 0
#endif
  if constexpr (S2) {
    static_assert(MODE != MODE_F32 && NT % NBUF == 0, "4x4 stride-2: the tap schedule of the bf16 modes");
    static_assert(XP::max_count() * PPU * XP::NSTG <= 2 * (NBLK - 2), "at most two transform stages per block");
    for (int chunk = 0; chunk < 2 * nck; chunk += 2) {
      do_chunk9(I0{}, I0{}, chunk);
      do_chunk9(I1{}, I1{}, chunk + 1);
    }
    for (int chunk = 2 * nck; chunk < nchunks; chunk += 2) {
      do_chunk9(I0{}, std::integral_constant<int, 2>{}, chunk);
      do_chunk9(I1{}, std::integral_constant<int, 3>{}, chunk + 1);
    }
  } else if constexpr (MODE != MODE_F32 && NT == 9 && (!TRANS || (IO16 && SDP_DGRAD16_TAPS))) {
    static_assert(XP::max_count() * PPU * XP::NSTG <= 2 * (NBLK - 2), "at most two transform stages per block");
    for (int chunk = 0; chunk < nchunks; chunk += 2) {
      do_chunk9(I0{}, I0{}, chunk);
      do_chunk9(I1{}, I0{}, chunk + 1);
    }
  } else {
    for (int chunk = 0; chunk < nchunks; chunk += 2) {
      do_chunk(std::integral_constant<int, 0>{}, chunk);
      do_chunk(std::integral_constant<int, 1>{}, chunk + 1);
    }
  }

  SDP_T(3);
  if (TRANS && (!a.dact || TC < 32 || NW != 4)) {
    if constexpr (TRANS) {
    __builtin_amdgcn_s_waitcnt(0);
    const int Ho = a.H, Wo = a.W;
    const size_t bo = (size_t)b * Ho * Wo * Cout;
    const int img_bytes = Ho * Wo * Cout * ES;
    auto rs = [&](const float* p) {
      return __builtin_amdgcn_make_buffer_rsrc((void*)(reinterpret_cast<const char*>(p) + bo * ES), 0, img_bytes, 0x00020000);
    };
    const int lq = lane >> 4, lcol = lane & 15;
    constexpr int CB = TC / 16;
    const int voff = (lcol * d * Cout + 4 * lq) * ES;
    auto soff = [&](int mb, int nj) {
      const int mr = mb / CB, mc = (mb % CB) * 16;
      const int y = (sr0 + wrow0 + mr) * d + ph_r, x = (sc0 + mc) * d + ph_c;
      return __builtin_amdgcn_readfirstlane(((y * Wo + x) * Cout + n0 + wn * 16 * NJ + nj * 16) * ES);
    };
    auto ld = [&](__amdgpu_buffer_rsrc_t r, int so) {
      if constexpr (IO16) {
        typedef __attribute__((ext_vector_type(2))) unsigned u32x2;
        const u32x2 q = __builtin_amdgcn_raw_buffer_load_b64(r, voff, so, 0);
        return bf4_to_f4(make_uint2(q.x, q.y));
      } else {
        const u32x4 q = __builtin_amdgcn_raw_buffer_load_b128(r, voff, so, 0);
        return make_float4(__uint_as_float(q.x), __uint_as_float(q.y), __uint_as_float(q.z), __uint_as_float(q.w));
      }
    };
    auto st = [&](float4 v, __amdgpu_buffer_rsrc_t r, int so, auto aux_c) {
      constexpr int AUX = decltype(aux_c)::value;
      if constexpr (IO16) {
        typedef __attribute__((ext_vector_type(2))) unsigned u32x2;
        const uint2 w = f4_to_bf4(v);
        __builtin_amdgcn_raw_buffer_store_b64(u32x2{w.x, w.y}, r, voff, so, AUX);
      } else {
        const u32x4 q = {__float_as_uint(v.x), __float_as_uint(v.y), __float_as_uint(v.z), __float_as_uint(v.w)};
        __builtin_amdgcn_raw_buffer_store_b128(q, r, voff, so, AUX);
      }
    };
    auto rs_or_out = [&](const float* p) { return rs(p ? p : a.out); };
    const __amdgpu_buffer_rsrc_t ors = rs(a.out), xrs = rs_or_out(a.aux), rrs = rs_or_out(a.res), o2rs = rs_or_out(a.out2),
                                 r2rs = rs_or_out(a.res2);
    static_for<0, NJ>([&](auto njc) {
      constexpr int nj = decltype(njc)::value;
      __builtin_amdgcn_sched_barrier(0);
      const int co0 = n0 + wn * 16 * NJ + nj * 16 + 4 * lq;
      float4 hq[8], rq[8], s0 = make_float4(1.f, 0.f, 1.f, 0.f), s1 = s0;
      if (a.dact) static_for<0, 8>([&](auto mb) { hq[mb] = ld(xrs, soff(mb, nj)); });
      if (a.dact == 3) {
        s0 = ld4(a.epi_ss + ((size_t)b * Cout + co0) * 2);
        s1 = ld4(a.epi_ss + ((size_t)b * Cout + co0) * 2 + 4);
      }
      if (a.res) static_for<0, 8>([&](auto mb) { rq[mb] = ld(rrs, soff(mb, nj)); });
      const float4 bias4 = a.bias ? ld4(a.bias + co0) : make_float4(0.f, 0.f, 0.f, 0.f);
      const float4 esc = make_float4(s0.x, s0.z, s1.x, s1.z), esh = make_float4(s0.y, s0.w, s1.y, s1.w);
      float4 v[8];
      static_for<0, 8>([&](auto mbc) {
        constexpr int mb = decltype(mbc)::value;
        const f32x4 q = acc4[mb][nj];
        v[mb] = make_float4(q[0] + bias4.x, q[1] + bias4.y, q[2] + bias4.z, q[3] + bias4.w);
      });
      if (a.up) {
        const int Hi = a.H / 2, Wi = a.W / 2;
        const float shh = (float)(Hi - 1) / (float)(a.H - 1), sww = (float)(Wi - 1) / (float)(a.W - 1);
        const size_t ub = (size_t)b * Hi * Wi * Cout + co0;
        auto lup = [&](size_t e) { return IO16 ? ldg4(reinterpret_cast<const __bf16*>(a.up), e) : ldg4(a.up, e); };
#pragma unroll
        for (int mb = 0; mb < 8; ++mb) {
          const int mr = mb / CB, mc = (mb % CB) * 16;
          const int y = (sr0 + wrow0 + mr) * d + ph_r, x = (sc0 + mc + lcol) * d + ph_c;
          const float fy = shh * (float)y, fx = sww * (float)x;
          const int y0 = (int)fy, x0 = (int)fx;
          const int yp = y0 < Hi - 1 ? 1 : 0, xp = x0 < Wi - 1 ? 1 : 0;
          const float ly1 = fy - (float)y0, ly0 = 1.f - ly1, lx1 = fx - (float)x0, lx0 = 1.f - lx1;
          const float4 v00 = lup(ub + ((size_t)y0 * Wi + x0) * Cout), v01 = lup(ub + ((size_t)y0 * Wi + x0 + xp) * Cout);
// ... 61 lines not shown
          m2[r] = q2;
        });
        auto merge = [&](auto ctl_c, float n) {
          constexpr int CTL = decltype(ctl_c)::value;
#pragma unroll
          for (int r = 0; r < 4; ++r) {
            const float mp = __int_as_float(__builtin_amdgcn_mov_dpp(__float_as_int(mean[r]), CTL, 0xf, 0xf, false));
            const float qp = __int_as_float(__builtin_amdgcn_mov_dpp(__float_as_int(m2[r]), CTL, 0xf, 0xf, false));
            const float dm = mean[r] - mp;
            m2[r] = m2[r] + qp + dm * dm * (0.5f * n);
            mean[r] = 0.5f * (mean[r] + mp);
          }
        };
        merge(std::integral_constant<int, 0xB1>{}, 8.f);
        merge(std::integral_constant<int, 0x4E>{}, 16.f);
        merge(std::integral_constant<int, 0x141>{}, 32.f);
        merge(std::integral_constant<int, 0x140>{}, 64.f);
        if (lcol == 0) {
          float4* sp = reinterpret_cast<float4*>(reinterpret_cast<float2*>(a.stats) +
                                                 ((size_t)b * a.groups_per_img + tile * WM + wm) * Cout + co0);
          sp[0] = make_float4(mean[0], m2[0], mean[1], m2[1]);
          sp[1] = make_float4(mean[2], m2[2], mean[3], m2[3]);
        }
      }
    });
    }
  } else if (SH == 16 && !TRANS && (!a.dact || TC < 32 || NW != 4)) {
    if constexpr (SH == 16 && !TRANS) {
    __builtin_amdgcn_s_waitcnt(0);
    const int Ho = (POOL || S2) ? a.H / 2 : a.H, Wo = (POOL || S2) ? a.W / 2 : a.W;
    const int de = S2 ? 1 : d;
    const size_t bo = (size_t)b * Ho * Wo * Cout;
    const int img_bytes = Ho * Wo * Cout * ES;
    auto rs = [&](const float* p) {
      return __builtin_amdgcn_make_buffer_rsrc((void*)(reinterpret_cast<const char*>(p ? p : a.out) + bo * ES), 0, img_bytes,
                                               0x00020000);
    };
    const __amdgpu_buffer_rsrc_t ors = rs(a.out), rrs = rs(a.res), o2rs = rs(a.out2), r2rs = rs(a.res2), xrs = rs(a.aux);
    const int lq = lane >> 4, lcol = lane & 15;
    constexpr int CB = TC / 16;
    constexpr int NF = POOL ? CB : 8;
    constexpr int PER = POOL ? 2 : 4;
    constexpr int NV = NF * PER;
    const int xs = (POOL ? 1 : de) * Cout * ES;
    int vbase[NF];
    static_for<0, NF>([&](auto fc) {
      constexpr int f = decltype(fc)::value;
      const int co = n0 + wn * 16 * NJ + lcol;
      if constexpr (POOL) {
        vbase[f] = (((sr0 >> 1) * Wo + ((sc0 + f * 16) >> 1) + 2 * lq) * Cout + co) * ES;
      } else {
        constexpr int mr = f / CB, mc = (f % CB) * 16;
        const int y = (sr0 + wrow0 + mr) * de + ph_r, x = (sc0 + mc + 4 * lq) * de + ph_c;
        vbase[f] = ((y * Wo + x) * Cout + co) * ES;
      }
    });
#define SDP_EPI16_OFF(i, nj) vbase[(i) / PER], __builtin_amdgcn_readfirstlane(((i) % PER) * xs + (nj) * 16 * ES)
    auto ld1 = [&](__amdgpu_buffer_rsrc_t r, int vo, int so) __attribute__((always_inline)) {
      if constexpr (IO16) return __uint_as_float((uint32_t)__builtin_amdgcn_raw_buffer_load_b16(r, vo, so, 0) << 16);
      else return __uint_as_float(__builtin_amdgcn_raw_buffer_load_b32(r, vo, so, 0));
    };
    auto store_vals = [&](const float (&w)[NV], __amdgpu_buffer_rsrc_t r, auto nj_c, auto aux_c) __attribute__((always_inline)) {
      constexpr int NJC = decltype(nj_c)::value, AUX = decltype(aux_c)::value;
      if constexpr (IO16) {
        constexpr int HP = PER / 2;
        const bool odd = lane & 1;
#pragma unroll
        for (int f = 0; f < NF; ++f) {
          const int vb = vbase[f] + (odd ? HP * xs - 2 : 0);
#pragma unroll
          for (int k = 0; k < HP; ++k) {
            const float mine = odd ? w[f * PER + HP + k] : w[f * PER + k];
            const float send = odd ? w[f * PER + k] : w[f * PER + HP + k];
            const float got = __int_as_float(__builtin_amdgcn_mov_dpp(__float_as_int(send), 0xB1, 0xf, 0xf, false));
            const uint32_t pk = odd ? pack_bf2(got, mine) : pack_bf2(mine, got);
            __builtin_amdgcn_raw_buffer_store_b32(pk, r, vb, __builtin_amdgcn_readfirstlane(k * xs + NJC * 16 * ES), AUX);
          }
        }
      } else {
#pragma unroll
        for (int i = 0; i < NV; ++i) __builtin_amdgcn_raw_buffer_store_b32(__float_as_uint(w[i]), r, SDP_EPI16_OFF(i, NJC), AUX);
      }
    };
    float pre[NJ][NV], biasv[NJ];
    static_for<0, NJ>([&](auto nj) { biasv[nj] = a.bias ? a.bias[n0 + wn * 16 * NJ + nj * 16 + lcol] : 0.f; });
    if (a.res || a.out2) {
      const __amdgpu_buffer_rsrc_t prs = a.res ? rrs : r2rs;
      static_for<0, NJ>([&](auto njc) {
#pragma unroll
        for (int i = 0; i < NV; ++i) pre[njc][i] = ld1(prs, SDP_EPI16_OFF(i, decltype(njc)::value));
      });
    }
    static_for<0, NJ>([&](auto njc) {
      constexpr int nj = decltype(njc)::value;
      const int co = n0 + wn * 16 * NJ + nj * 16 + lcol;
      const float bias = biasv[nj];
      float v[NV];
      if constexpr (POOL) {
        static_for<0, CB>([&](auto fc) {
          constexpr int f = decltype(fc)::value;
          static_for<0, 2>([&](auto kc) {
            constexpr int k = decltype(kc)::value;
            const float a00 = acc4[f][nj][2 * k], a01 = acc4[f][nj][2 * k + 1];
            const float a10 = acc4[f + CB][nj][2 * k], a11 = acc4[f + CB][nj][2 * k + 1];
            v[f * 2 + k] = ((((a00 + bias) + (a10 + bias)) + (a01 + bias)) + (a11 + bias)) / 4.0f;
          });
        });
      } else {
        static_for<0, 8>([&](auto fc) {
          constexpr int f = decltype(fc)::value;
#pragma unroll
          for (int r = 0; r < 4; ++r) v[f * 4 + r] = acc4[f][nj][r] + bias;
        });
      }
      if (!S2 && a.up) {
        const int Hi = a.H / 2, Wi = a.W / 2;
        const float shh = (float)(Hi - 1) / (float)(a.H - 1), sww = (float)(Wi - 1) / (float)(a.W - 1);
        const size_t ub = (size_t)b * Hi * Wi * Cout + co;
        auto lu = [&](size_t e) { return IO16 ? ldg1(reinterpret_cast<const __bf16*>(a.up), e) : ldg1(a.up, e); };
#pragma unroll
        for (int i = 0; i < NV; ++i) {
          const int f = i / PER, k = i % PER;
          const int mr = f / CB, mc = (f % CB) * 16;
          const int y = (sr0 + wrow0 + mr) * de + ph_r, x = (sc0 + mc + 4 * lq + k) * de + ph_c;
          const float fy = shh * (float)y, fx = sww * (float)x;
          const int y0 = (int)fy, x0 = (int)fx;
          const int yp = y0 < Hi - 1 ? 1 : 0, xp = x0 < Wi - 1 ? 1 : 0;
          const float ly1 = fy - (float)y0, ly0 = 1.f - ly1, lx1 = fx - (float)x0, lx0 = 1.f - lx1;
          const float v00 = lu(ub + ((size_t)y0 * Wi + x0) * Cout), v01 = lu(ub + ((size_t)y0 * Wi + x0 + xp) * Cout);
          const float v10 = lu(ub + ((size_t)(y0 + yp) * Wi + x0) * Cout);
          const float v11 = lu(ub + ((size_t)(y0 + yp) * Wi + x0 + xp) * Cout);
          v[i] = v[i] + (ly0 * (lx0 * v00 + lx1 * v01) + ly1 * (lx0 * v10 + lx1 * v11));
        }
      }
      if (a.dact) {
        float esc = 1.f, esh = 0.f;
        if (a.dact == 3) {
          esc = a.epi_ss[((size_t)b * Cout + co) * 2];
          esh = a.epi_ss[((size_t)b * Cout + co) * 2 + 1];
        }
#pragma unroll
        for (int i = 0; i < NV; ++i) {
          float h = ld1(xrs, SDP_EPI16_OFF(i, nj));
          if (a.dact == 3) h = fmaf(h, esc, esh);
          v[i] = v[i] * elu_grad(h, a.dact);
        }
      }
      if (a.res) {
#pragma unroll
        for (int i = 0; i < NV; ++i) v[i] = pre[nj][i] + v[i];
      }
      if (a.out2) {
        float r2[NV];
#pragma unroll
        for (int i = 0; i < NV; ++i)
          r2[i] = a.res ? ld1(r2rs, SDP_EPI16_OFF(i, nj)) : pre[nj][i];
#pragma unroll
        for (int i = 0; i < NV; ++i) r2[i] = v[i] + r2[i];
        store_vals(r2, o2rs, njc, std::integral_constant<int, 0>{});
      }
      if (a.epi_elu) {
#pragma unroll
        for (int i = 0; i < NV; ++i) v[i] = elu(v[i]);
      }
      if constexpr (!(SDP_KO & 16))
        store_vals(v, ors, njc, std::integral_constant<int, IO16 ? SDP_STORE_AUX16 : SDP_STORE_AUX>{});
      if (a.stats) {
        float sum = 0.f;
#pragma unroll
        for (int i = 0; i < NV; ++i) sum += v[i];
        float mean = sum * (1.0f / NV);
        float m2 = 0.f;
#pragma unroll
        for (int i = 0; i < NV; ++i) {
          const float dv = v[i] - mean;
          m2 = fmaf(dv, dv, m2);
        }
        float mp = __shfl_xor(mean, 16), qp = __shfl_xor(m2, 16), dm = mean - mp;
        m2 = m2 + qp + dm * dm * (0.5f * NV);
        mean = 0.5f * (mean + mp);
        mp = __shfl_xor(mean, 32);
        qp = __shfl_xor(m2, 32);
        dm = mean - mp;
        m2 = m2 + qp + dm * dm * (float)NV;
        mean = 0.5f * (mean + mp);
        if (lq == 0) {
          float2* st = reinterpret_cast<float2*>(a.stats) + ((size_t)b * a.groups_per_img + tile * WM + wm) * Cout + co;
          *st = make_float2(mean, m2);
        }
      }
    });
#undef SDP_EPI16_OFF
    }
  } else if (a.dact) {
    if constexpr (TC >= 32 && NW == 4 && SH == 16) {
    __builtin_amdgcn_s_waitcnt(0);
    __syncthreads();
    constexpr int SROW = T::NTILE + 8;
    constexpr int SP = WM * 64;
    constexpr int CG = T::NTILE / 4;
    constexpr int PL = 256 / CG;
    constexpr int NPO = POOL ? SP / 4 : SP;
    static_assert(SP * SROW * 4 <= T::LDS_BYTES, "epilogue staging fits the LDS");
    float* stage = reinterpret_cast<float*>(lds);
    const int cg = tid % CG, pl = tid / CG;
    const int co0 = n0 + cg * 4;
    const float4 bias4 = a.bias ? ld4(a.bias + co0) : make_float4(0.f, 0.f, 0.f, 0.f);
    float4 es0 = make_float4(1.f, 0.f, 1.f, 0.f), es1 = es0;
    if (a.dact == 3) {
      es0 = ld4(a.epi_ss + ((size_t)b * Cout + co0) * 2);
      es1 = ld4(a.epi_ss + ((size_t)b * Cout + co0) * 2 + 4);
    }
    const int Ho = POOL ? a.H / 2 : a.H, Wo = POOL ? a.W / 2 : a.W;
    using TA = std::conditional_t<IO16, __bf16, float>;
    auto tp = [](const float* p) { return reinterpret_cast<const TA*>(p); };
    TA* const outb = reinterpret_cast<TA*>(a.out) + (size_t)b * Ho * Wo * Cout;
    float4 sK[WM], s1[WM], s2[WM];
    int sn[WM];
    static_for<0, WM>([&](auto g) {
      sK[g] = make_float4(0.f, 0.f, 0.f, 0.f); s1[g] = sK[g]; s2[g] = sK[g]; sn[g] = 0;
    });
    static_for<0, 2>([&](auto hc) {
      constexpr int h = decltype(hc)::value;
      {
        if constexpr (!POOL && TRANS) {
          static_for<0, 4>([&](auto ic) {
            constexpr int i = decltype(ic)::value;
            static_for<0, 4>([&](auto njc) {
              constexpr int nj = decltype(njc)::value;
              float* dst = stage + (wm * 64 + 16 * i + (lane & 15)) * SROW + wn * 64 + nj * 16 + 4 * (lane >> 4);
              const f32x4 q = acc4[4 * h + i][nj];
              *reinterpret_cast<float4*>(dst) = make_float4(q[0], q[1], q[2], q[3]);
            });
          });
        } else if constexpr (!POOL) {
          static_for<0, 4>([&](auto ic) {
            constexpr int i = decltype(ic)::value;
            static_for<0, 4>([&](auto njc) {
              constexpr int nj = decltype(njc)::value;
              float* dst = stage + (wm * 64 + 16 * i + 4 * (lane >> 4)) * SROW + wn * 64 + nj * 16 + (lane & 15);
  #pragma unroll
              for (int r = 0; r < 4; ++r) dst[r * SROW] = acc4[4 * h + i][nj][r];
            });
          });
        }
      }
      __syncthreads();
      auto pix = [&](int j, int& y, int& x, int& g) __attribute__((always_inline)) {
        if constexpr (POOL) {
// ... 278 lines not shown
```

### simultaneous-diffusion-for-pointclouds_amd/csrc/conv_launch.h

```cpp
#pragma once
#include "common.h"

namespace sdp {

template <int MODE, int WM, int TC, int KS, bool POOL, bool PELU, bool IO16 = false>
hipError_t conv_launch(ConvArgs a, hipStream_t st);

template <int MODE, bool PELU>
hipError_t conv_launch_half(ConvArgs a, hipStream_t st);

template <int MODE, bool PELU, int NW, bool IO16 = false>
hipError_t conv_launch_nj2(ConvArgs a, hipStream_t st);

template <int MODE>
hipError_t conv_launch_s2(ConvArgs a, hipStream_t st);

template <int MODE>
hipError_t dgrad_launch_half(ConvArgs a, hipStream_t st);

template <int MODE, int NW, bool IO16 = false>
hipError_t dgrad_launch_nj2(ConvArgs a, hipStream_t st);

template <int MODE, int WM, int TC, int KS, bool ZP, bool IO16 = false>
hipError_t dgrad_launch(ConvArgs a, hipStream_t st);


}
```

### simultaneous-diffusion-for-pointclouds_amd/csrc/kernel_entry.hip

```cpp
#include <string>

#include "../../include/sdp_kernels.h"
#include "kernels.h"

int sdp_fail(const std::string& m);

using namespace sdp;

namespace {

hipStream_t S(void* stream) { return reinterpret_cast<hipStream_t>(stream); }
const float* F(const void* p) { return reinterpret_cast<const float*>(p); }
float* F(void* p) { return reinterpret_cast<float*>(p); }

int done(hipError_t e, const char* what, const char* why = nullptr) {
  if (e == hipSuccess) return 0;
  return sdp_fail(std::string(what) + ": " + (why ? why : hipGetErrorString(e)));
}

ConvArgs conv_args(const sdpk_conv& c) {
  ConvArgs a{};
  a.in = F(c.in);
  a.wf = reinterpret_cast<const uint4*>(c.wf);
  a.wf16 = reinterpret_cast<const uint4*>(c.wf16);
// ... 6 lines not shown
  a.pro_ss = c.pro_ss;
  a.ss_bstride = c.ss_bstride;
  a.stats = c.stats;
  a.B = c.B;
  a.H = c.H;
  a.W = c.W;
  a.Cin = c.Cin;
  a.Cout = c.Cout;
  a.dil = c.dil;
  a.circular = c.circular;
  a.pro_mode = c.pro_mode;
  a.epi_elu = c.epi_elu;
  a.aux = F(c.aux);
  a.epi_ss = c.epi_ss;
  a.dact = c.dact;
  a.io16 = c.io16;
  a.s2 = c.s2;
  return a;
}

}

extern "C" {

int sdpk_pack_weights(const float* w, uint32_t* out, int Cout, int Cin, int k, int mode, int packing, void* desc_scratch,
                      void* stream) {
  if (!w || !out || !desc_scratch) return sdp_fail("sdpk_pack_weights: null argument");
  if (packing != SDPK_PACK_FRAG && packing != SDPK_PACK_FRAG16 && packing != SDPK_PACK_DFRAG16 &&
      packing != SDPK_PACK_POOL4X4)
    return sdp_fail("sdpk_pack_weights: unknown packing");
  if (packing == SDPK_PACK_POOL4X4 && k != 3) return sdp_fail("sdpk_pack_weights: the 4x4 stride-2 packing merges a 3x3");
  const int nt = packing == SDPK_PACK_POOL4X4 ? 16 : k * k;
  const PackDesc d{w, out, Cout, Cin, nt, packing, 0};
  static_assert(sizeof(PackDesc) <= 64, "sdpk_pack_weights: desc_scratch holds one descriptor");
  hipError_t e = hipMemcpyAsync(desc_scratch, &d, sizeof d, hipMemcpyHostToDevice, S(stream));
  if (e != hipSuccess) return done(e, "sdpk_pack_weights");
  return done(pack_weights_multi(reinterpret_cast<const PackDesc*>(desc_scratch), 1, (size_t)Cout * Cin * nt, mode,
                                 S(stream)),
              "sdpk_pack_weights");
}

int sdpk_conv_mfma(int mode, const sdpk_conv* c, int ks, int pool, void* stream) {
  if (!c) return sdp_fail("sdpk_conv_mfma: null argument");
  const char* why = nullptr;
  return done(conv_mfma(mode, conv_args(*c), ks, pool != 0, S(stream), &why), "sdpk_conv_mfma", why);
}

int sdpk_conv_dgrad(int mode, const sdpk_conv* c, int ks, void* stream) {
  if (!c) return sdp_fail("sdpk_conv_dgrad: null argument");
  const char* why = nullptr;
  return done(conv_dgrad(mode, conv_args(*c), ks, S(stream), &why), "sdpk_conv_dgrad", why);
}

int sdpk_conv_wgrad(int mode, const sdpk_wgrad* g, int ks, float* out, float* bias_out, int accumulate, int h16,
                    void* stream) {
  if (!g) return sdp_fail("sdpk_conv_wgrad: null argument");
  WgradArgs a{};
  a.in = F(g->in);
  a.pro_ss = g->pro_ss;
  a.ss_bstride = g->ss_bstride;
  a.pro_mode = g->pro_mode;
  a.dy = F(g->dy);
  a.part = g->part;
  a.part_floats = g->part_floats;
  a.bpart = g->bpart;
  a.B = g->B;
  a.H = g->H;
  a.W = g->W;
  a.Cin = g->Cin;
  a.Cout = g->Cout;
  a.dil = g->dil;
  a.circular = g->circular;
  const char* why = nullptr;
  return done(conv_wgrad(mode, a, ks, out, bias_out, accumulate, S(stream), &why, h16 != 0), "sdpk_conv_wgrad", why);
}

int sdpk_wgrad_splits(int B, int H, int W, int dil, int Cin, int Cout, int ks) {
  return wgrad_splits(B, H, W, dil, Cin, Cout, ks);
}

size_t sdpk_wgrad_part_floats(int splits, int Cin, int Cout, int ks) { return wgrad_part_floats(splits, Cin, Cout, ks); }

int sdpk_maxpool5(const void* in, void* out, uint8_t* idx, int B, int H, int W, int C, int h16, void* stream) {
  return done(maxpool5(F(in), F(out), B, H, W, C, S(stream), idx, h16 != 0), "sdpk_maxpool5");
}

int sdpk_maxpool5_backward(const uint8_t* idx, const void* dp, const void* res, void* dst, int B, int H, int W, int C,
                           int h16, void* stream) {
  return done(maxpool5_backward(idx, F(dp), F(res), F(dst), B, H, W, C, S(stream), h16 != 0), "sdpk_maxpool5_backward");
}

int sdpk_avgpool2(const float* in, float* out, int B, int H, int W, int C, void* stream) {
  return done(avgpool2(in, out, B, H, W, C, S(stream)), "sdpk_avgpool2");
}

int sdpk_unpool(const void* dout, void* dst, int B, int H, int W, int C, int h16, void* stream) {
  return done(unpool(F(dout), F(dst), B, H, W, C, S(stream), h16 != 0), "sdpk_unpool");
}

int sdpk_upsample_backward(const void* g, void* dlow, int B, int H, int W, int C, int accumulate, int h16, void* stream) {
  return done(upsample_backward(F(g), F(dlow), B, H, W, C, accumulate, S(stream), h16 != 0), "sdpk_upsample_backward");
}

int sdpk_elu_backward_post(const void* dy, const void* y, const void* res, void* dst, size_t n, int h16, void* stream) {
  return done(elu_backward_post(F(dy), F(y), F(res), F(dst), n, S(stream), h16 != 0), "sdpk_elu_backward_post");
}

int sdpk_add_tensors(const void* a, const void* b, void* dst, size_t n, int h16, void* stream) {
  return done(add_tensors(F(a), F(b), F(dst), n, S(stream), h16 != 0), "sdpk_add_tensors");
}

int sdpk_inpp_finalize(const float* stats, int B, int T, float cnt, int C, const float* alpha, const float* gamma,
                       const float* beta, float* ss, float* nst, void* scratch, void* stream) {
  return done(inpp_finalize(stats, B, T, cnt, C, alpha, gamma, beta, ss, S(stream), nst, scratch), "sdpk_inpp_finalize");
}

int sdpk_inpp_backward(const void* g, const void* h, const float* nst, const float* alpha, const float* gamma, int B,
                       int HW, int C, float* part, float* coef, float* ppart, float* dalpha, float* dgamma, float* dbeta,
                       const void* r1, const void* r2, void* out, int h16, void* stream) {
  return done(inpp_backward(F(g), F(h), nst, alpha, gamma, B, HW, C, part, coef, ppart, dalpha, dgamma, dbeta, F(r1), F(r2),
                            F(out), S(stream), h16 != 0),
              "sdpk_inpp_backward");
}

}
```

### simultaneous-diffusion-for-pointclouds_amd/csrc/kernels.h

```cpp
#pragma once
#include "common.h"
#include "langevin.h"

namespace sdp {

hipError_t conv_mfma(int mode, ConvArgs a, int ks, bool pool, hipStream_t st, const char** why);
hipError_t begin_conv(const float* x, const float* w, const float* bias, float* out, float* stats, int B, int H, int W,
                      hipStream_t st, int mode = MODE_F32, bool h16 = false);
hipError_t end_conv(const float* in, const float* ss, const float* w, const float* bias, const float* sigmas,
                    const int64_t* labels, float* out, int B, int H, int W, int Cin, hipStream_t st,
                    const LangevinArgs* lg = nullptr, int mode = MODE_F32, bool h16 = false);
hipError_t inpp_finalize(const float* stats, int B, int T, float cnt, int C, const float* alpha, const float* gamma,
                         const float* beta, float* ss, hipStream_t st, float* nst, void* scratch);
hipError_t maxpool5(const float* in, float* out, int B, int H, int W, int C, hipStream_t st, uint8_t* idx = nullptr,
                    bool h16 = false);
hipError_t avgpool2(const float* in, float* out, int B, int H, int W, int C, hipStream_t st);
hipError_t langevin_step(float* x, const float* g, const float* ref, const int32_t* mask, const float* noise,
                         uint64_t seed, uint64_t offset, float step, float nscale, float gref, int n2n, int B, int C,
                         int HW, float* lik_out, uint32_t* absmax, hipStream_t st);
hipError_t axpy_step(float* x, const float* g, float a, const float* lik, const int32_t* mask, const float* ref, float b,
                     size_t n, hipStream_t st);

struct PackDesc {
  const float* w;
  uint32_t* out;
  int Cout, Cin, NT, dgrad;
  size_t begin;
};
hipError_t pack_weights_multi(const PackDesc* d, int nd, size_t total, int mode, hipStream_t st);
hipError_t pack_weights(const float* w, uint32_t* out, int Cout, int Cin, int k, int mode, int dgrad, hipStream_t st);
hipError_t inpp_backward(const float* g, const float* h, const float* nst, const float* alpha, const float* gamma, int B,
                         int HW, int C, float* part, float* coef, float* ppart, float* dalpha, float* dgamma,
                         float* dbeta, const float* r1, const float* r2, float* out, hipStream_t st, bool h16 = false);
hipError_t unpool(const float* dout, float* dst, int B, int H, int W, int C, hipStream_t st, bool h16 = false);
hipError_t maxpool5_backward(const uint8_t* idx, const float* dp, const float* res, float* dst, int B, int H, int W, int C,
                             hipStream_t st, bool h16 = false);
hipError_t upsample_backward(const float* g, float* dlow, int B, int H, int W, int C, int accumulate, hipStream_t st,
                             bool h16 = false);
hipError_t elu_backward_post(const float* dy, const float* y, const float* res, float* dst, size_t n, hipStream_t st,
                             bool h16 = false);
hipError_t add_tensors(const float* a, const float* b, float* dst, size_t n, hipStream_t st, bool h16 = false);
size_t head_wgrad_part_floats(int B, int H, int W);
hipError_t begin_conv_wgrad(const float* x, const float* dy, float* part, float* dw, float* db, int B, int H, int W,
                            hipStream_t st, bool h16 = false);
hipError_t end_conv_backward(const float* dscore, const float* sigmas, const int64_t* labels, const float* w,
                             const float* o, const float* ss, float* g, float* part, float* dw, float* db, int B, int H,
                             int W, hipStream_t st, bool h16 = false);
hipError_t dsm_loss(const float* score, const float* noise, const float* mask, const float* used_sigma, int B, int n_img,
                    float power, float* dscore, float* loss, float* loss_per, float* part, hipStream_t st);
enum { OPT_ADAM = 0, OPT_RMSPROP = 1, OPT_SGD = 2 };
struct OptimHyper {
  float b1, b2;
  float eps, weight_decay;
  float step_size;
  float bc2_sqrt;
  float mu;
  float omb1, omb2, ommu;
  int first;
};
hipError_t optim_ema(int kind, float* p, const float* g, float* s0, float* s1, float* s2, float* shadow, size_t n,
                     const OptimHyper& h, hipStream_t st);
hipError_t conv_dgrad(int mode, ConvArgs a, int ks, hipStream_t st, const char** why);
#ifndef SDP_WGRAD_BLOCKS
#define SDP_WGRAD_BLOCKS 512
#endif
constexpr int WGRAD_TARGET_BLOCKS = SDP_WGRAD_BLOCKS;
int wgrad_splits(int B, int H, int W, int d, int Cin, int Cout, int ks);
size_t wgrad_part_floats(int S, int Cin, int Cout, int ks);
hipError_t conv_wgrad(int mode, WgradArgs a, int ks, float* out, float* bias_out, int accumulate, hipStream_t st,
                      const char** why, bool h16 = false);

}
```

### simultaneous-diffusion-for-pointclouds_amd/csrc/net.hip

```cpp
#include <algorithm>
#include <cmath>
#include <cstdlib>
#include <cstring>
#include <map>
#include <stdexcept>
#include <string>
#include <vector>


#include "net_internal.h"

using namespace sdp;

namespace {

struct Buf {
  float* p;
  int H, W, C;
};

struct Fwd {
  sdp_net* net;
  int B;
  hipStream_t st;
  float* stats;
  float* ss;
  float* mv;

  struct Opt {
    int pro = PRO_NONE;
    bool bias = true;
    const float* res = nullptr;
    const float* up = nullptr;
    float* out2 = nullptr;
    const float* res2 = nullptr;
    bool epi_elu = false;
    bool stats = false;
    int dil = 1;
    bool circular = true;
    bool pool = false;
    bool s2 = false;
  };

  void conv(const Buf& in, const std::string& wkey, const Buf& out, const Opt& o) {
    const auto& hp = net->host.at(wkey + ".weight");
    ConvArgs a{};
    a.in = in.p;
    a.wf = net->mode == MODE_F32 ? reinterpret_cast<const uint4*>(net->P(wkey + ".weight#frag")) : nullptr;
    a.wf16 = net->mode == MODE_F32 ? nullptr
                                   : reinterpret_cast<const uint4*>(net->P(wkey + (o.s2 ? ".weight#pool4x4" : ".weight#frag16")));
    a.s2 = o.s2 ? 1 : 0;
    a.bias = o.bias ? net->P(wkey + ".bias") : nullptr;
    a.out = out.p;
    a.res = o.res;
    a.out2 = o.out2;
    a.res2 = o.res2;
    a.up = o.up;
    a.pro_ss = o.pro == PRO_AFFINE_ELU ? ss : net->P("#ident_ss");
    a.ss_bstride = o.pro == PRO_AFFINE_ELU ? 2 * in.C : 0;
    a.stats = o.stats ? stats : nullptr;
    a.B = B;
    a.H = in.H;
    a.W = in.W;
    a.Cin = in.C;
    a.Cout = out.C;
    a.dil = o.dil;
    a.circular = o.circular ? 1 : 0;
    a.pro_mode = o.pro;
    a.epi_elu = o.epi_elu ? 1 : 0;
    if ((int)hp.shape[1] != in.C || (int)hp.shape[0] != out.C) throw std::runtime_error("conv shape mismatch " + wkey);
    const char* why = "conv launch";
    const int ks = (int)hp.shape[2];
    sdp_net::ProfRec rec;
    if (net->profile) {
      rec.cls = "conv" + std::to_string(ks) + "x" + std::to_string(ks) + " " + std::to_string(in.C) + "->" +
                std::to_string(out.C) + " @" + std::to_string(in.H) + "x" + std::to_string(in.W) + " d" +
                std::to_string(o.dil) + (o.pool ? " pool" : "");
      rec.flops = 2.0 * B * in.H * in.W * (double)in.C * out.C * ks * ks;
      if (o.s2) {
        rec.cls = "conv4x4s2 " + std::to_string(in.C) + "->" + std::to_string(out.C) + " @" + std::to_string(in.H) + "x" +
                  std::to_string(in.W);
        rec.flops = 2.0 * B * out.H * out.W * (double)in.C * out.C * 16;
      }
      rec.bytes = 4.0 * B * ((double)in.H * in.W * in.C + (double)out.H * out.W * out.C) + 4.0 * out.C * in.C * ks * ks;
      rec.a = net->event();
      rec.b = net->event();
      chk(hipEventRecord(rec.a, st), "hipEventRecord");
    }
    hipError_t e = conv_mfma(net->mode, a, ks, o.pool, st, &why);
    if (e != hipSuccess) throw std::runtime_error(std::string(why) + " (" + wkey + ")");
    if (net->profile) {
      chk(hipEventRecord(rec.b, st), "hipEventRecord");
      net->prof.push_back(rec);
    }
  }

  template <class F>
  void prof_launch(const std::string& cls, double bytes, F&& launch) {
    sdp_net::ProfRec rec;
    if (net->profile) {
      rec.cls = cls;
      rec.flops = 0;
      rec.bytes = bytes;
      rec.a = net->event();
      rec.b = net->event();
      chk(hipEventRecord(rec.a, st), "hipEventRecord");
    }
    launch();
    if (net->profile) {
      chk(hipEventRecord(rec.b, st), "hipEventRecord");
      net->prof.push_back(rec);
    }
  }

  void norm(const std::string& nkey, int T, float cnt, int C) {
    prof_launch("inpp_finalize C" + std::to_string(C), (double)B * T * C * 8 + (double)B * C * 8, [&] {
      chk(inpp_finalize(stats, B, T, cnt, C, net->P(nkey + ".alpha"), net->P(nkey + ".gamma"), net->P(nkey + ".beta"),
                        ss, st, nullptr, mv),
          "inpp_finalize");
    });
  }
  void pool(const Buf& X, const Buf& P) {
    const double bytes = 2.0 * B * X.H * X.W * X.C * 4;
    prof_launch("maxpool5 " + std::to_string(X.C) + " @" + std::to_string(X.H) + "x" + std::to_string(X.W), bytes,
                [&] { chk(maxpool5(X.p, P.p, B, X.H, X.W, X.C, st), "maxpool5"); });
  }
  static int tiles(const Buf& b) { return b.H * b.W / 128; }

  bool pool_as_s2() const { return net->mode != MODE_F32; }

  void resblock(const std::string& k, const Buf& x, const Buf& t1, const Buf& t2, const Buf& out, bool down, int dil,
                bool want_stats, int x_tiles, float x_cnt) {
    norm(k + ".normalize1", x_tiles, x_cnt, x.C);
    Opt o1;
    o1.pro = PRO_AFFINE_ELU;
    o1.stats = true;
    o1.dil = dil;
    conv(x, k + ".conv1", t1, o1);
    norm(k + ".normalize2", tiles(t1), 128.f, t1.C);
    Opt o2;
    o2.pro = PRO_AFFINE_ELU;
    o2.stats = want_stats;
    o2.dil = dil;
    if (down && dil == 1) {
      const Buf xp{out.p, x.H / 2, x.W / 2, x.C};
      prof_launch("avgpool2 " + std::to_string(x.C) + " @" + std::to_string(x.H) + "x" + std::to_string(x.W),
                  1.25 * B * x.H * x.W * x.C * 4, [&] { chk(avgpool2(x.p, xp.p, B, x.H, x.W, x.C, st), "avgpool2"); });
      Opt os;
      os.circular = false;
      conv(xp, k + ".shortcut.conv", t2, os);
      o2.circular = false;
      o2.pool = !pool_as_s2();
      o2.s2 = pool_as_s2();
      o2.res = t2.p;
      conv(t1, k + ".conv2.conv", out, o2);
    } else if (down) {
      Opt os;
      os.dil = dil;
      conv(x, k + ".shortcut", t2, os);
      o2.res = t2.p;
      conv(t1, k + ".conv2", out, o2);
    } else {
      o2.res = x.p;
      conv(t1, k + ".conv2", out, o2);
    }
  }

  Buf rcu(const std::string& k, Buf x, int nblocks, const Buf& tmp, const Buf& o0, const Buf& o1, bool final_elu,
          bool final_stats) {
    Buf outs[2] = {o0, o1};
    for (int i = 0; i < nblocks; ++i) {
      Opt a;
      a.pro = PRO_ELU;
      a.bias = false;
      conv(x, k + "." + std::to_string(i + 1) + "_1_conv", tmp, a);
      Opt b;
      b.pro = PRO_ELU;
      b.bias = false;
      b.res = x.p;
      b.epi_elu = final_elu && i == nblocks - 1;
      b.stats = final_stats && i == nblocks - 1;
      const Buf& y = outs[i & 1];
      conv(tmp, k + "." + std::to_string(i + 1) + "_2_conv", y, b);
      x = y;
    }
    return x;
  }

  Buf crp(const std::string& k, const Buf& X, const Buf& P, const Buf& Qp, const Buf& R, const Buf& S) {
    pool(X, P);
    Opt a;
    a.bias = false;
    a.out2 = R.p;
    a.res2 = X.p;
    conv(P, k + ".convs.0", Qp, a);
    pool(Buf{Qp.p, X.H, X.W, X.C}, P);
    Opt b;
    b.bias = false;
    b.res = R.p;
    conv(P, k + ".convs.1", S, b);
    return S;
  }
};

}

static void forward_impl(sdp_net* net, const float* x, const int64_t* labels, float* out, int B, void* ws,
                         size_t ws_bytes, hipStream_t st, const LangevinArgs* lg = nullptr) {
  const int H = net->d.H, W = net->d.W, C = net->d.ngf, C2 = 2 * C;
  const int h = H / 2, w = W / 2;
  const size_t F = (size_t)B * H * W * C, Q = (size_t)B * h * w * C2;
  char* p = reinterpret_cast<char*>(ws);
  char* end = p + ws_bytes;
  auto take = [&](size_t n) {
    float* q = reinterpret_cast<float*>(p);
    p += ((n * 4 + 255) / 256) * 256;
    if (p > end) throw std::runtime_error("workspace too small");
    return q;
  };
  Fwd f{net, B, st, nullptr, nullptr, nullptr};
  f.stats = take((size_t)B * (H * W / 64) * C2 * 2);
  f.ss = take((size_t)B * C2 * 2);
  f.mv = take((size_t)B * C2 * 4);
  auto full = [&]() { return Buf{take(F), H, W, C}; };
  auto half = [&]() { return Buf{take(Q), h, w, C2}; };
  Buf L1 = full(), FA = full(), FB = full(), FC = full(), FD = full(), FE = full();
  Buf L2 = half(), L3 = half(), L4 = half(), QA = half(), QB = half(), QC = half(), QD = half(), QE = half();
  auto half128 = [&](const Buf& b) { return Buf{b.p, h, w, C}; };

  using Opt = Fwd::Opt;
  f.prof_launch("begin_conv 4->128 @" + std::to_string(H) + "x" + std::to_string(W),
                (double)B * H * W * (2 * 4 + C * 4) + (double)B * (H * W / 64) * C * 8, [&] {
                  chk(begin_conv(x, net->P("begin_conv.weight"), net->P("begin_conv.bias"), FA.p, f.stats, B, H, W, st, net->mode),
                      "begin_conv");
                });
  f.resblock("res1.0", FA, FB, FD, FC, false, 1, true, H * W / 64, 64.f);
  f.resblock("res1.1", FC, FB, FD, L1, false, 1, true, Fwd::tiles(FC), 128.f);
  f.resblock("res2.0", L1, FB, QA, QB, true, 1, true, Fwd::tiles(L1), 128.f);
  if (f.pool_as_s2()) f.resblock("res2.1", QB, QA, QC, L2, false, 1, true, Fwd::tiles(QB), 128.f);
  else f.resblock("res2.1", QB, QA, QC, L2, false, 1, true, Fwd::tiles(L1), 32.f);
  f.resblock("res3.0", L2, QA, QB, QC, true, 2, true, Fwd::tiles(L2), 128.f);
  f.resblock("res3.1", QC, QA, QB, L3, false, 2, true, Fwd::tiles(QC), 128.f);
  f.resblock("res4.0", L3, QA, QB, QC, true, 4, true, Fwd::tiles(L3), 128.f);
  f.resblock("res4.1", QC, QA, QB, L4, false, 4, false, Fwd::tiles(QC), 128.f);

  Buf a1 = f.rcu("refine1.adapt_convs.0", L4, 2, QA, QB, QC, true, false);
  Buf x2 = f.crp("refine1.crp", a1, QA, QB, QD, QE);
  Buf ref1 = f.rcu("refine1.output_convs", x2, 1, QA, QB, QC, false, false);
  Buf hA = f.rcu("refine2.adapt_convs.0", L3, 2, QA, QC, QD, false, false);
  Buf hB = f.rcu("refine2.adapt_convs.1", ref1, 2, QA, QC, QE, false, false);
  {
    Opt o;
    f.conv(hA, "refine2.msf.convs.0", QA, o);
    Opt o1;
    o1.res = QA.p;
    o1.epi_elu = true;
    f.conv(hB, "refine2.msf.convs.1", QB, o1);
  }
  x2 = f.crp("refine2.crp", QB, QA, QC, QD, QE);
  Buf ref2 = f.rcu("refine2.output_convs", x2, 1, QA, QB, QC, false, false);
  hA = f.rcu("refine3.adapt_convs.0", L2, 2, QA, QC, QD, false, false);
  hB = f.rcu("refine3.adapt_convs.1", ref2, 2, QA, QC, QE, false, false);
  {
    Opt o;
    f.conv(hA, "refine3.msf.convs.0", half128(QA), o);
    Opt o1;
    o1.res = QA.p;
    o1.epi_elu = true;
    f.conv(hB, "refine3.msf.convs.1", half128(QB), o1);
  }
  x2 = f.crp("refine3.crp", half128(QB), half128(QA), half128(QC), half128(QD), half128(QE));
  Buf ref3 = f.rcu("refine3.output_convs", x2, 1, half128(QA), half128(QB), half128(QC), false, false);
  hA = f.rcu("refine4.adapt_convs.0", L1, 2, FA, FB, FC, false, false);
  hB = f.rcu("refine4.adapt_convs.1", ref3, 2, half128(QA), half128(QC), half128(QD), false, false);
  {
    Opt o;
    f.conv(hB, "refine4.msf.convs.1", half128(QA), o);
    Opt o1;
    o1.up = QA.p;
    o1.epi_elu = true;
    f.conv(hA, "refine4.msf.convs.0", FD, o1);
  }
  x2 = f.crp("refine4.crp", FD, FA, FB, FE, FC);
  Buf o = f.rcu("refine4.output_convs", x2, 3, FA, FB, FD, false, true);
  f.norm("normalizer", Fwd::tiles(o), 128.f, C);
  const double lg_bytes = lg ? (double)B * 2 * H * W * (20 + (out ? 4 : 0) + (lg->noise ? 4 : 0)) : B * 2.0 * H * W * 4;
  f.prof_launch(std::string(lg ? "end_conv+langevin" : "end_conv") + " 128->2 @" + std::to_string(H) + "x" +
                    std::to_string(W),
                (double)B * H * W * C * 4 + lg_bytes, [&] {
                  chk(end_conv(o.p, f.ss, net->P("end_conv.weight"), net->P("end_conv.bias"), net->P("sigmas"), labels,
                               out, B, H, W, C, st, lg, net->mode),
                      "end_conv");
                });
}

static size_t workspace_bytes_one(const sdp_net* net, int B) {
  const int H = net->d.H, W = net->d.W, C = net->d.ngf, C2 = 2 * C;
  const size_t F = (size_t)B * H * W * C, Q = (size_t)B * (H / 2) * (W / 2) * C2;
  auto r = [](size_t n) { return ((n * 4 + 255) / 256) * 256; };
  return r((size_t)B * (H * W / 64) * C2 * 2) + r((size_t)B * C2 * 2) + r((size_t)B * C2 * 4) + 6 * r(F) + 8 * r(Q);
}

constexpr int kSplitDefault = 2;
static int split_ways(const sdp_net* net) { return net->split > 0 ? net->split : kSplitDefault; }

static void split_part(int B, int k, int p, int& first, int& count) {
  first = (int)((long)B * p / k);
  count = (int)((long)B * (p + 1) / k) - first;
}

static size_t workspace_bytes(const sdp_net* net, int B) {
  size_t need = workspace_bytes_one(net, B);
  const int k = std::min(B, split_ways(net));
  if (k > 1) {
    size_t sum = 0;
    for (int p = 0; p < k; ++p) {
      int f, c;
      split_part(B, k, p, f, c);
      sum += workspace_bytes_one(net, c);
    }
    need = std::max(need, sum);
  }
  return need;
}

static void forward_split(sdp_net* net, const float* x, const int64_t* labels, float* out, int B, void* ws,
                          size_t ws_bytes, hipStream_t st, const LangevinArgs* lg) {
  const int k = std::min(B, split_ways(net));
  if (k < 2 || net->profile) {
    forward_impl(net, x, labels, out, B, ws, ws_bytes, st, lg);
    return;
  }
  for (int p = 0; p + 1 < k; ++p) {
    if (!net->aux_stream[p])
      chk(hipStreamCreateWithFlags(&net->aux_stream[p], hipStreamNonBlocking), "hipStreamCreate");
    if (!net->ev_join[p]) chk(hipEventCreateWithFlags(&net->ev_join[p], hipEventDisableTiming), "hipEventCreate");
  }
  if (!net->ev_fork) chk(hipEventCreateWithFlags(&net->ev_fork, hipEventDisableTiming), "hipEventCreate");
  const size_t per = (size_t)2 * net->d.H * net->d.W;
  char* w = reinterpret_cast<char*>(ws);
  chk(hipEventRecord(net->ev_fork, st), "hipEventRecord");
  for (int p = k - 1; p >= 0; --p) {
    int f, c;
    split_part(B, k, p, f, c);
    const size_t wb = workspace_bytes_one(net, c);
    hipStream_t s = p ? net->aux_stream[p - 1] : st;
    if (p) chk(hipStreamWaitEvent(s, net->ev_fork, 0), "hipStreamWaitEvent");
    LangevinArgs l{};
    if (lg) {
      l = *lg;
      l.x = lg->x + f * per;
      l.ref = lg->ref + f * per;
      l.mask = lg->mask + f * per;
      if (lg->noise) l.noise = lg->noise + f * per;
      if (lg->lik) l.lik = lg->lik + f * per;
      l.offset = lg->offset + f * per / 4;
    }
    forward_impl(net, x + f * per, labels + f, out ? out + f * per : nullptr, c, w, wb, s, lg ? &l : nullptr);
    w += wb;
    if (p) chk(hipEventRecord(net->ev_join[p - 1], s), "hipEventRecord");
  }
// ... 108 lines not shown
  return 0;
}

int sdp_net_param_info(const sdp_net* net, int i, char* key, size_t cap, size_t* offset, size_t* numel) {
  if (!net || !net->finalized || i < 0 || i >= (int)net->layout.size() || !key || cap == 0)
    return fail("sdp_net_param_info: bad argument");
  const auto& e = net->layout[i];
  std::strncpy(key, e.key.c_str(), cap - 1);
  key[cap - 1] = 0;
  if (offset) *offset = e.offset;
  if (numel) *numel = e.numel;
  return 0;
}

int sdp_net_bind_params(sdp_net* net, float* arena, void* stream) {
  if (!net || !arena || !net->finalized) return fail("sdp_net_bind_params: bad argument");
  try {
    hipStream_t st = reinterpret_cast<hipStream_t>(stream);
    if (arena != net->arena)
      chk(hipMemcpyAsync(arena, net->arena, net->arena_floats * 4, hipMemcpyDeviceToDevice, st), "hipMemcpyAsync");
    chk(hipStreamSynchronize(st), "hipStreamSynchronize");
    if (net->arena_owned) chk(hipFree(net->arena), "hipFree");
    net->arena = arena;
    net->arena_owned = false;
    for (auto& e : net->layout) net->dev[e.key] = arena + e.offset;
  } catch (const std::exception& e) {
    return fail(std::string("sdp_net_bind_params: ") + e.what());
  }
  return 0;
}

int sdp_net_repack(sdp_net* net, void* stream) {
  if (!net || !net->finalized) return fail("sdp_net_repack: finalize first");
  try {
    net->repack(reinterpret_cast<hipStream_t>(stream));
  } catch (const std::exception& e) {
    return fail(std::string("sdp_net_repack: ") + e.what());
  }
  return 0;
}

int sdp_net_workspace_size(const sdp_net* net, int B, size_t* bytes) {
  if (!net || !bytes || B <= 0) return fail("sdp_net_workspace_size: bad argument");
  *bytes = workspace_bytes(net, B);
  return 0;
}

int sdp_net_forward(sdp_net* net, const float* x, const int64_t* labels, float* out, int B, void* ws, size_t ws_bytes,
                    void* stream) {
  if (!net || !x || !labels || !out || !ws || B <= 0) return fail("sdp_net_forward: bad argument");
  if (!net->finalized) return fail("sdp_net_forward: call sdp_net_finalize first");
  if (ws_bytes < workspace_bytes(net, B)) return fail("sdp_net_forward: workspace too small");
  const hipStream_t st = reinterpret_cast<hipStream_t>(stream);
  try {
    forward_split(net, x, labels, out, B, ws, ws_bytes, st, nullptr);
  } catch (const std::exception& e) {
    return fail(std::string("sdp_net_forward: ") + e.what());
  }
  return 0;
}

int sdp_net_forward_langevin(sdp_net* net, float* x, const int64_t* labels, int B, const sdp_langevin_params* lp,
                             void* ws, size_t ws_bytes, void* stream) {
  if (!net || !x || !labels || !lp || !lp->ref || !lp->mask || !ws || B <= 0)
    return fail("sdp_net_forward_langevin: bad argument");
  if (!net->finalized) return fail("sdp_net_forward_langevin: call sdp_net_finalize first");
  if (ws_bytes < workspace_bytes(net, B)) return fail("sdp_net_forward_langevin: workspace too small");
  const LangevinArgs lg{x,         lp->ref,          lp->mask,  lp->noise,    lp->seed,         lp->offset, lp->step_size,
                        lp->noise_scale, lp->grad_ref, lp->nan_to_num, lp->lik_out, lp->absmax_bits};
  try {
    forward_split(net, x, labels, lp->grad_out, B, ws, ws_bytes, reinterpret_cast<hipStream_t>(stream), &lg);
  } catch (const std::exception& e) {
    return fail(std::string("sdp_net_forward_langevin: ") + e.what());
  }
  return 0;
}

int sdp_net_set_split(sdp_net* net, int ways) {
  if (!net || ways < 0 || ways > SDP_MAX_SPLIT) return fail("sdp_net_set_split: ways must be 0 (default) .. 4");
  net->split = ways;
  return 0;
}

int sdp_net_profile_enable(sdp_net* net, int enable) {
  if (!net) return fail("sdp_net_profile_enable: null net");
  net->profile = enable != 0;
  return 0;
}

int sdp_net_profile_read(sdp_net* net, char* buf, size_t cap, int* n_launches) {
  if (!net || !buf || cap == 0) return fail("sdp_net_profile_read: bad argument");
  struct Agg { int n = 0; double ms = 0, flops = 0, bytes = 0; };
  std::map<std::string, Agg> agg;
  try {
    for (auto& r : net->prof) {
      chk(hipEventSynchronize(r.b), "hipEventSynchronize");
      float ms = 0.f;
      chk(hipEventElapsedTime(&ms, r.a, r.b), "hipEventElapsedTime");
      Agg& g = agg[r.cls];
      g.n += 1;
      g.ms += ms;
      g.flops = r.flops;
      g.bytes = r.bytes;
      net->ev_pool.push_back(r.a);
      net->ev_pool.push_back(r.b);
    }
  } catch (const std::exception& e) {
    return fail(std::string("sdp_net_profile_read: ") + e.what());
  }
  if (n_launches) *n_launches = (int)net->prof.size();
  net->prof.clear();
  std::string out;
  for (auto& kv : agg)
    out += kv.first + "\t" + std::to_string(kv.second.n) + "\t" + std::to_string(kv.second.ms) + "\t" +
           std::to_string(kv.second.flops) + "\t" + std::to_string(kv.second.bytes) + "\n";
  std::strncpy(buf, out.c_str(), cap - 1);
  buf[cap - 1] = 0;
  return 0;
}

int sdp_net_destroy(sdp_net* net) {
  delete net;
  return 0;
}

int sdp_langevin_step(float* x, const float* grad, const float* ref, const int32_t* mask, const float* noise,
                      uint64_t seed, uint64_t offset, float step_size, float noise_scale, float grad_ref, int nan_to_num,
                      int B, int C, int HW, float* lik_out, uint32_t* absmax_bits, void* stream) {
  if (!x || !grad || !ref || !mask || B <= 0 || C <= 0 || HW <= 0) return fail("sdp_langevin_step: bad argument");
  if (HW % 4) return fail("sdp_langevin_step: H*W must be a multiple of 4");
  hipError_t e = langevin_step(x, grad, ref, mask, noise, seed, offset, step_size, noise_scale, grad_ref, nan_to_num, B,
                               C, HW, lik_out, absmax_bits, reinterpret_cast<hipStream_t>(stream));
  return e == hipSuccess ? 0 : fail(std::string("sdp_langevin_step: ") + hipGetErrorString(e));
}

int sdp_axpy_step(float* x, const float* g, float a, const float* lik, const int32_t* mask, const float* ref, float b,
                  int n, void* stream) {
  if (!x || n <= 0 || (g && !lik) || (!g && (!mask || !ref))) return fail("sdp_axpy_step: bad argument");
  hipError_t e = axpy_step(x, g, a, lik, mask, ref, b, (size_t)n, reinterpret_cast<hipStream_t>(stream));
  return e == hipSuccess ? 0 : fail(std::string("sdp_axpy_step: ") + hipGetErrorString(e));
}

}
```

### simultaneous-diffusion-for-pointclouds_amd/csrc/net_internal.h

```cpp
#pragma once
#include <cstring>
#include <map>
#include <memory>
#include <stdexcept>
#include <string>
#include <vector>

#include "../../include/sdp.h"
#include "kernels.h"

namespace sdp {

struct HostParam {
  std::vector<int64_t> shape;
  std::vector<float> data;
};

struct ParamEntry {
  std::string key;
  size_t offset, numel;
};

inline void chk(hipError_t e, const char* what) {
  if (e != hipSuccess) throw std::runtime_error(std::string(what) + ": " + hipGetErrorString(e));
}

constexpr int SDP_MAX_SPLIT = 4;

struct TrainPlan;
void destroy_plan(TrainPlan* p);

}

struct sdp_net {
  struct ProfRec {
    std::string cls;
    double flops;
    double bytes = 0;
    hipEvent_t a, b;
  };
  sdp_net_desc d;
  bool profile = false;
  std::vector<ProfRec> prof;
  std::vector<hipEvent_t> ev_pool;
  std::map<std::string, sdp::HostParam> host;
  std::map<std::string, void*> dev;
  std::vector<sdp::ParamEntry> layout;
  float* arena = nullptr;
  size_t arena_floats = 0;
  bool arena_owned = false;
  bool finalized = false;
  bool train_packs = false;
  bool tape16 = true;
  int mode = sdp::MODE_F32X3;
  sdp::TrainPlan* plan = nullptr;
  int split = 0;
  hipStream_t aux_stream[sdp::SDP_MAX_SPLIT - 1] = {};
  hipEvent_t ev_fork = nullptr, ev_join[sdp::SDP_MAX_SPLIT - 1] = {};

  ~sdp_net() {
    release();
    for (auto& s : aux_stream)
      if (s) (void)hipStreamDestroy(s);
    for (auto& e : ev_join)
      if (e) (void)hipEventDestroy(e);
    if (ev_fork) (void)hipEventDestroy(ev_fork);
    for (auto& r : prof) {
      (void)hipEventDestroy(r.a);
      (void)hipEventDestroy(r.b);
    }
    for (auto e : ev_pool) (void)hipEventDestroy(e);
  }
  void release() {
    for (auto& kv : dev) {
      const bool in_arena = arena && kv.second >= (void*)arena && kv.second < (void*)(arena + arena_floats);
      if (!in_arena) (void)hipFree(kv.second);
    }
    dev.clear();
    if (pack_dev) (void)hipFree(pack_dev);
    pack_dev = nullptr;
    pack_dev_n = 0;
    pack_host.clear();
    if (arena_owned && arena) (void)hipFree(arena);
    arena = nullptr;
    arena_owned = false;
    if (plan) sdp::destroy_plan(plan);
    plan = nullptr;
  }
  hipEvent_t event() {
    if (!ev_pool.empty()) {
      hipEvent_t e = ev_pool.back();
      ev_pool.pop_back();
      return e;
    }
    hipEvent_t e;
    if (hipEventCreate(&e) != hipSuccess) throw std::runtime_error("hipEventCreate");
    return e;
  }
  const float* P(const std::string& k) const {
    auto it = dev.find(k);
    if (it == dev.end()) throw std::runtime_error("missing parameter " + k);
    return reinterpret_cast<const float*>(it->second);
  }
  float* grad_of(float* grads, const std::string& k) const {
    for (auto& e : layout)
      if (e.key == k) return grads + e.offset;
    throw std::runtime_error("no parameter " + k);
  }
  bool is_conv_w(const std::string& k) const {
    auto it = host.find(k);
    return it != host.end() && it->second.shape.size() == 4 && k != "begin_conv.weight" && k != "end_conv.weight";
  }
  bool is_pool3x3_w(const std::string& k) const {
    static const std::string suffix = ".conv2.conv.weight";
    auto it = host.find(k);
    return k.size() > suffix.size() && k.compare(k.size() - suffix.size(), suffix.size(), suffix) == 0 &&
           it != host.end() && it->second.shape.size() == 4 && it->second.shape[2] == 3 && it->second.shape[3] == 3;
  }
  std::vector<sdp::PackDesc> pack_host;
  sdp::PackDesc* pack_dev = nullptr;
  size_t pack_dev_n = 0, pack_total = 0;
  void repack(hipStream_t st) {
    std::vector<sdp::PackDesc> d;
    size_t total = 0;
    for (auto& kv : host) {
      if (!is_conv_w(kv.first)) continue;
      const auto& s = kv.second.shape;
      for (int dg = 0; dg < 6; ++dg) {
        if (dg == 0 && mode != sdp::MODE_F32) continue;
        if (dg == 1 || dg == 2) continue;
        if (dg == 3 && mode == sdp::MODE_F32) continue;
        if (dg == 4 && (!train_packs || mode == sdp::MODE_F32)) continue;
        if (dg == 5 && (mode == sdp::MODE_F32 || !is_pool3x3_w(kv.first))) continue;
        const std::string fk = kv.first + (dg == 0 ? "#frag" : dg == 3 ? "#frag16" : dg == 4 ? "#dfrag16" : "#pool4x4");
        const int nt = dg == 5 ? 16 : (int)(s[2] * s[3]);
        const size_t n = (size_t)s[0] * s[1] * nt;
        if (!dev.count(fk)) {
          void* p = nullptr;
          sdp::chk(hipMalloc(&p, n * 4), "hipMalloc");
// ... 32 lines not shown
```

### simultaneous-diffusion-for-pointclouds_amd/sdp/_lib.py

```python
from __future__ import annotations

import ctypes as C
import os

import torch

_HERE = os.path.dirname(os.path.abspath(__file__))
LIB_PATH = os.environ.get("SDP_LIB", os.path.join(_HERE, "_lib", "libsdp.so"))

P = C.c_void_p
I = C.c_int
F = C.c_float
D = C.c_double
U64 = C.c_uint64
SZ = C.c_size_t


class NetDesc(C.Structure):
    _fields_ = [("ngf", I), ("channels", I), ("H", I), ("W", I), ("num_classes", I), ("precision", I)]


class MergeParams(C.Structure):
    _fields_ = [("variant", I), ("setting", I), ("sigma", F), ("allowance", F), ("cc", F)]


class LangevinParams(C.Structure):
    _fields_ = [("ref", P), ("mask", P), ("noise", P), ("seed", U64), ("offset", U64), ("step_size", F),
                ("noise_scale", F), ("grad_ref", F), ("nan_to_num", I), ("lik_out", P), ("absmax_bits", P),
                ("grad_out", P)]


PREC = {"fp32": 0, "fp32x3": 1, "bf16": 2}
MERGE_POSES, MERGE_ORIGINS = 0, 1

_SIGS = {
    "sdp_version": (I, []),
    "sdp_last_error": (C.c_char_p, []),
    "sdp_net_create": (I, [C.POINTER(NetDesc), C.POINTER(P)]),
    "sdp_net_set_param": (I, [P, C.c_char_p, P, C.POINTER(C.c_int64), I]),
    "sdp_net_finalize": (I, [P]),
    "sdp_net_workspace_size": (I, [P, I, C.POINTER(SZ)]),
    "sdp_net_forward": (I, [P, P, P, P, I, P, SZ, P]),
    "sdp_net_forward_langevin": (I, [P, P, P, I, C.POINTER(LangevinParams), P, SZ, P]),
    "sdp_net_set_split": (I, [P, I]),
    "sdp_net_set_tape": (I, [P, I]),
    "sdp_net_destroy": (I, [P]),
    "sdp_net_profile_enable": (I, [P, I]),
    "sdp_net_profile_read": (I, [P, C.c_char_p, SZ, C.POINTER(I)]),
    "sdp_net_param_arena_floats": (I, [P, C.POINTER(SZ)]),
    "sdp_net_param_count": (I, [P, C.POINTER(I)]),
    "sdp_net_param_info": (I, [P, I, C.c_char_p, SZ, C.POINTER(SZ), C.POINTER(SZ)]),
    "sdp_net_bind_params": (I, [P, P, P]),
    "sdp_net_repack": (I, [P, P]),
    "sdp_net_train_workspace_size": (I, [P, I, C.POINTER(SZ)]),
    "sdp_net_forward_train": (I, [P, P, P, P, I, P, SZ, P]),
    "sdp_net_backward": (I, [P, P, I, P, SZ, P, P]),
    "sdp_net_backward_buckets": (I, [P, P, I, P, SZ, P, I, C.POINTER(SZ), C.POINTER(P), P]),
    "sdp_dsm_loss": (I, [P, P, P, P, I, I, F, P, P, P, P, P]),
    "sdp_adam_ema_step": (I, [P, P, P, P, P, SZ, D, D, D, D, I, D, P]),
    "sdp_optim_ema_step": (I, [I, P, P, P, P, P, P, SZ, D, D, D, D, D, I, D, P]),
    "sdp_range_project_workspace_size": (I, [I, I, C.POINTER(SZ)]),
    "sdp_range_project": (I, [P, I, I, I, P, I, I, P, P, P, P, P, P, SZ, P]),
    "sdp_view_transform": (I, [P, C.c_int64, P, P, P, P]),
    "sdp_view_gather": (I, [P, I, I, I, P, P, P, P]),
    "sdp_view_finalize": (I, [P, P, P, P, P, P, I, I, I, I, I, I, P, P, P, P, P]),
    "sdp_grid_subsample": (I, [P, C.c_int64, P, I, P, I, F, I, P, P, P, C.POINTER(C.c_int64)]),
    "sdp_langevin_step": (I, [P, P, P, P, P, U64, U64, F, F, F, I, I, I, I, P, P, P]),
    "sdp_axpy_step": (I, [P, P, F, P, P, P, F, I, P]),
    "sdp_merge_workspace_size": (I, [I, I, I, I, C.POINTER(SZ)]),
    "sdp_merge_workspace_bytes": (I, [I, I, I, I, I, C.POINTER(SZ)]),
    "sdp_consistency_merge": (I, [P, I, I, I, I, I, I, P, P, P, P, P, P, C.POINTER(MergeParams), P, P, P, SZ, P]),
    "sdp_consistency_merge_ev": (I, [P, I, I, I, I, I, I, P, P, P, P, P, P, C.POINTER(MergeParams), P, P, P, SZ, P, P]),
}

_lib = None


def lib():
    global _lib
    if _lib is None:
        from . import _build
        _build.ensure_built()
        if not os.path.exists(LIB_PATH):
            raise RuntimeError(f"libsdp.so not found at {LIB_PATH}: build it with `python __graft_entry__.py build` "
                               "(or `make -C simultaneous-diffusion-for-pointclouds_amd/csrc`)")
        L = C.CDLL(LIB_PATH)
        for name, (res, args) in _SIGS.items():
            fn = getattr(L, name)
            fn.restype = res
            fn.argtypes = args
        _lib = L
    return _lib


def check(rc: int, what: str = "") -> None:
    if rc != 0:
        raise RuntimeError(f"libsdp {what}: {lib().sdp_last_error().decode()}")


def ptr(t) -> int | None:
    return None if t is None else t.data_ptr()


def stream() -> int:
    return torch.cuda.current_stream().cuda_stream


def exported_symbols():
    return list(_SIGS)
```

### simultaneous-diffusion-for-pointclouds_amd/sdp/scorenet.py

```python
from __future__ import annotations

import numpy as np
import torch

from . import _lib
from .weights import param_spec, synthetic_state_dict


class ScoreNet:
    def __init__(self, H: int = 64, W: int = 1024, ngf: int = 128, channels: int = 2, num_classes: int = 232,
                 precision: str = "fp32x3"):
        L = _lib.lib()
        self.H, self.W, self.ngf, self.channels, self.num_classes = H, W, ngf, channels, num_classes
        self.precision = precision
        d = _lib.NetDesc(ngf, channels, H, W, num_classes, _lib.PREC[precision])
        h = _lib.P()
        _lib.check(L.sdp_net_create(_lib.C.byref(d), _lib.C.byref(h)), "net_create")
        self._h = h
        self._ws = {}
        self._ready = False
        self.sigmas = None

    def load_state_dict(self, sd, ema_shadow=None):
        L = _lib.lib()
# ... 2 lines not shown
            sd.update({k[7:] if k.startswith("module.") else k: v for k, v in ema_shadow.items()})
        need = set(param_spec(self.ngf, self.channels)) | {"sigmas"}
        missing = need - set(sd)
        if missing:
            raise KeyError(f"missing parameters: {sorted(missing)[:5]} ...")
        for k in need:
            a = np.ascontiguousarray(np.asarray(sd[k].detach().cpu() if torch.is_tensor(sd[k]) else sd[k],
                                                dtype=np.float32))
            shape = (_lib.C.c_int64 * a.ndim)(*a.shape)
            _lib.check(L.sdp_net_set_param(self._h, k.encode(), a.ctypes.data, shape, a.ndim), "set_param " + k)
        _lib.check(L.sdp_net_finalize(self._h), "finalize")
        s = sd["sigmas"]
        self.sigmas = torch.as_tensor(np.asarray(s.cpu() if torch.is_tensor(s) else s, np.float32))
        self._ready = True
        return self

    def param_shapes(self):
        return param_spec(self.ngf, self.channels).items()

    def load_synthetic(self):
        return self.load_state_dict(synthetic_state_dict(self.ngf, self.channels, self.num_classes))

    def load_checkpoint(self, path):
        states = torch.load(path, map_location="cpu", weights_only=True)
        return self.load_state_dict(states[0], states[-1] if len(states) >= 5 else None)

    def workspace(self, B: int, device) -> torch.Tensor:
        key = (B, str(device))
        ws = self._ws.get(key)
        if ws is None:
            n = _lib.SZ()
            _lib.check(_lib.lib().sdp_net_workspace_size(self._h, B, _lib.C.byref(n)), "workspace_size")
            ws = torch.empty(n.value, dtype=torch.uint8, device=device)
            self._ws[key] = ws
        return ws

    def forward(self, x: torch.Tensor, y: torch.Tensor, out: torch.Tensor | None = None) -> torch.Tensor:
        if not self._ready:
            raise RuntimeError("ScoreNet: load weights first")
        if not x.is_cuda or x.dtype != torch.float32 or x.dim() != 4 or x.shape[1:] != (self.channels, self.H, self.W):
            raise ValueError(f"ScoreNet expects cuda float32 [B,{self.channels},{self.H},{self.W}], got "
                             f"{tuple(x.shape)} {x.dtype} {x.device}")
        x = x.contiguous()
        B = x.shape[0]
        y = y.to(device=x.device, dtype=torch.int64).contiguous()
        if out is None:
            out = torch.empty_like(x)
        ws = self.workspace(B, x.device)
        _lib.check(_lib.lib().sdp_net_forward(self._h, x.data_ptr(), y.data_ptr(), out.data_ptr(), B, ws.data_ptr(),
                                              ws.numel(), _lib.stream()), "net_forward")
        return out

    __call__ = forward

    def forward_langevin(self, x: torch.Tensor, y: torch.Tensor, ref: torch.Tensor, mask: torch.Tensor,
                         noise: torch.Tensor | None, seed: int, offset: int, step: float, nscale: float,
                         grad_ref: float, nan_to_num: bool, lik: torch.Tensor | None, absmax: torch.Tensor | None,
                         grad_out: torch.Tensor | None = None) -> None:
        if not self._ready:
            raise RuntimeError("ScoreNet: load weights first")
        if not x.is_cuda or x.dtype != torch.float32 or x.dim() != 4 or x.shape[1:] != (self.channels, self.H, self.W) \
                or not x.is_contiguous():
            raise ValueError(f"forward_langevin expects contiguous cuda float32 [B,{self.channels},{self.H},{self.W}] "
                             f"(updated in place), got {tuple(x.shape)} {x.dtype} {x.device}")
        for name, t, dt in (("ref", ref, torch.float32), ("mask", mask, torch.int32), ("noise", noise, torch.float32),
                            ("lik", lik, torch.float32), ("grad_out", grad_out, torch.float32)):
            if t is not None and (t.shape != x.shape or t.dtype != dt or not t.is_contiguous() or t.device != x.device):
                raise ValueError(f"forward_langevin: {name} must be contiguous {dt} {tuple(x.shape)} on {x.device}")
        if absmax is not None and (absmax.dtype != torch.int32 or absmax.device != x.device):
            raise ValueError("forward_langevin: absmax must be an int32 device tensor")
        B = x.shape[0]
        y = y.to(device=x.device, dtype=torch.int64).contiguous()
        ws = self.workspace(B, x.device)
        p = _lib.LangevinParams(ref.data_ptr(), mask.data_ptr(), _lib.ptr(noise), int(seed) & 0xFFFFFFFFFFFFFFFF,
                                int(offset), float(step), float(nscale), float(grad_ref), 1 if nan_to_num else 0,
                                _lib.ptr(lik), _lib.ptr(absmax), _lib.ptr(grad_out))
        _lib.check(_lib.lib().sdp_net_forward_langevin(self._h, x.data_ptr(), y.data_ptr(), B, _lib.C.byref(p),
                                                       ws.data_ptr(), ws.numel(), _lib.stream()), "net_forward_langevin")

    def set_split(self, ways: int):
        _lib.check(_lib.lib().sdp_net_set_split(self._h, int(ways)), "set_split")
        self._ws.clear()

    def set_tape(self, bf16: bool):
        _lib.check(_lib.lib().sdp_net_set_tape(self._h, 1 if bf16 else 0), "set_tape")

    def profile(self, enable: bool = True):
        _lib.check(_lib.lib().sdp_net_profile_enable(self._h, 1 if enable else 0), "profile_enable")

    def profile_read(self):
        buf = _lib.C.create_string_buffer(1 << 16)
        n = _lib.I()
        _lib.check(_lib.lib().sdp_net_profile_read(self._h, buf, len(buf), _lib.C.byref(n)), "profile_read")
        out = {}
        for line in buf.value.decode().splitlines():
            cls, cnt, ms, fl, by = line.split("\t")
            out[cls] = (int(cnt), float(ms), float(fl), float(by))
        return out

    def eval(self):
        return self

    def __del__(self):
        try:
            if getattr(self, "_h", None):
                _lib.lib().sdp_net_destroy(self._h)
                self._h = None
        except Exception:
            pass
```

Measured before the change: 375.6 image-steps/s.

## Store refine-block activations pre-split into bf16 hi/lo operand form for fp32x3 convs

Adds an 'operand form' path in which circular 3x3 convs and maxpool on 256-channel refine-block tensors write their outputs already split into bf16 hi/lo pairs with ELU applied. The next conv can then DMA the patch straight into LDS through three rotating buffers, skipping the per-chunk prologue transform (scale/shift, ELU, split) in registers. This is meant to cut transform ALU work and register pressure inside the MFMA loop of the fp32x3 refine convs. It is on by default. In exchange it adds new kernel template instantiations, more validation paths and a third LDS patch buffer. Residual reads of x in split form need care, and there is a risk of layout mismatch between producers and consumers.

```diff
diff --git a/include/sdp.h b/include/sdp.h
--- a/include/sdp.h
+++ b/include/sdp.h
@@ -50,6 +50,7 @@
 int sdp_net_forward_langevin(sdp_net* net, float* x, const int64_t* labels, int B, const sdp_langevin_params* params,
                              void* workspace, size_t workspace_bytes, void* stream);
 int sdp_net_set_split(sdp_net* net, int ways);
+int sdp_net_set_operand_form(sdp_net* net, int on);
 int sdp_net_profile_enable(sdp_net* net, int enable);
 int sdp_net_profile_read(sdp_net* net, char* buf, size_t cap, int* n_launches);
 
diff --git a/simultaneous-diffusion-for-pointclouds_amd/csrc/aux.hip b/simultaneous-diffusion-for-pointclouds_amd/csrc/aux.hip
--- a/simultaneous-diffusion-for-pointclouds_amd/csrc/aux.hip
+++ b/simultaneous-diffusion-for-pointclouds_amd/csrc/aux.hip
@@ -725,7 +725,7 @@
 #define SDP_MP_MIN_BLOCKS 512
 #endif
 constexpr int MP_COLS = 8, MP_NS = 6, MP_D = 2, MP_MIN_BLOCKS = SDP_MP_MIN_BLOCKS;
-template <bool IDX>
+template <bool IDX, bool OSPLIT = false>
 __global__ __launch_bounds__(256) void maxpool5_kernel(const float* __restrict__ in, float* __restrict__ out,
                                                        uchar4* __restrict__ idx, int B, int H, int W, int C,
                                                        int rows) {
@@ -819,7 +819,20 @@
       if (hm[r].w > m.w) { m.w = hm[r].w; bi.w = ro + hc[r].w; }
     }
     const size_t o = (((size_t)b * H + y) * W + x) * C4 + cg * 32 + c4;
-    reinterpret_cast<float4*>(out)[o] = m;
+    if constexpr (OSPLIT) {
+      const float4 z = make_float4(m.x + 0.0f, m.y + 0.0f, m.z + 0.0f, m.w + 0.0f);
+      const __bf16 h0 = (__bf16)z.x, h1 = (__bf16)z.y, h2 = (__bf16)z.z, h3 = (__bf16)z.w;
+      const uint2 hi = make_uint2(pack_bf2((float)h0, (float)h1), pack_bf2((float)h2, (float)h3));
+      const uint2 lo = make_uint2(pack_bf2(z.x - (float)h0, z.y - (float)h1), pack_bf2(z.z - (float)h2, z.w - (float)h3));
+      const bool odd = c4 & 1;
+      const uint2 send = odd ? hi : lo;
+      const uint2 got = make_uint2((uint32_t)__builtin_amdgcn_mov_dpp((int)send.x, 0xB1, 0xf, 0xf, false),
+                                   (uint32_t)__builtin_amdgcn_mov_dpp((int)send.y, 0xB1, 0xf, 0xf, false));
+      uint4* const op = reinterpret_cast<uint4*>(out) + (o >> 3) * 8 + (odd ? 4 : 0) + ((o & 7) >> 1);
+      *op = odd ? make_uint4(got.x, got.y, lo.x, lo.y) : make_uint4(hi.x, hi.y, got.x, got.y);
+    } else {
+      reinterpret_cast<float4*>(out)[o] = m;
+    }
     if constexpr (IDX) idx[o] = bi;
 #pragma unroll
     for (int r = 0; r < 4; ++r) {
@@ -1025,9 +1038,9 @@
   return hipGetLastError();
 }
 
-hipError_t maxpool5(const float* in, float* out, int B, int H, int W, int C, hipStream_t st, uint8_t* idx, bool h16) {
-  if (C % 128 || W % MP_COLS) return hipErrorInvalidValue;
-  if (h16) {
+hipError_t maxpool5(const float* in, float* out, int B, int H, int W, int C, hipStream_t st, uint8_t* idx, int form) {
+  if (C % 128 || W % MP_COLS || form < 0 || form > 2 || (form == 2 && idx)) return hipErrorInvalidValue;
+  if (form == 1) {
     if (W % MPH_COLS) return hipErrorInvalidValue;
     auto hb = [&](int rows) { return B * ((H + rows - 1) / rows) * (W / MPH_COLS) * (C / 128); };
     const int rows = hb(32) >= 1024 ? 32 : (hb(16) >= 1024 ? 16 : 8), grid = hb(rows);
@@ -1037,7 +1050,9 @@
   }
   auto blocks = [&](int rows) { return B * ((H + rows - 1) / rows) * (W / MP_COLS) * (C / 128); };
   const int rows = blocks(32) >= MP_MIN_BLOCKS ? 32 : 16, grid = blocks(rows);
-  if (idx)
+  if (form == 2)
+    hipLaunchKernelGGL((maxpool5_kernel<false, true>), dim3(grid), dim3(256), 0, st, in, out, nullptr, B, H, W, C, rows);
+  else if (idx)
     hipLaunchKernelGGL(maxpool5_kernel<true>, dim3(grid), dim3(256), 0, st, in, out, reinterpret_cast<uchar4*>(idx), B, H,
                        W, C, rows);
   else
diff --git a/simultaneous-diffusion-for-pointclouds_amd/csrc/common.h b/simultaneous-diffusion-for-pointclouds_amd/csrc/common.h
--- a/simultaneous-diffusion-for-pointclouds_amd/csrc/common.h
+++ b/simultaneous-diffusion-for-pointclouds_amd/csrc/common.h
@@ -23,7 +23,9 @@
 }
 
 enum { MODE_F32 = 0, MODE_F32X3 = 1, MODE_BF16 = 2 };
-enum { PRO_NONE = 0, PRO_ELU = 1, PRO_AFFINE_ELU = 2 };
+enum { PRO_NONE = 0, PRO_ELU = 1, PRO_AFFINE_ELU = 2, PRO_SPLIT = 3 };
+enum { EPI_ELU = 1, EPI_SPLIT = 2 };
+enum { OPF_IN = 1, OPF_OUT = 2 };
 
 typedef __attribute__((ext_vector_type(4))) int i32x4;
 SDP_DEV i32x4 buffer_desc(const void* base, uint32_t bytes) {
diff --git a/simultaneous-diffusion-for-pointclouds_amd/csrc/conv.hip b/simultaneous-diffusion-for-pointclouds_amd/csrc/conv.hip
--- a/simultaneous-diffusion-for-pointclouds_amd/csrc/conv.hip
+++ b/simultaneous-diffusion-for-pointclouds_amd/csrc/conv.hip
@@ -68,8 +68,34 @@
   }
   if (a.up && ((a.H & 1) || (a.W & 1) || a.H < 2 || a.W < 2)) { *why = "conv: upsample needs even H,W"; return hipErrorInvalidValue; }
   if (!a.circular && d != 1) { *why = "conv: zero padding only for d=1"; return hipErrorInvalidValue; }
-  if (!a.pro_ss) { *why = "conv: prologue scale/shift table missing"; return hipErrorInvalidValue; }
-  if (a.Cin > 1024 && a.ss_bstride == 0) { *why = "conv: identity table holds 1024 channels"; return hipErrorInvalidValue; }
+  if (!a.circular && ks == 3 && !pool && !a.s2) {
+    *why = "conv: a zero-padded 3x3 runs pooled or as the 4x4 stride-2 form only";
+    return hipErrorInvalidValue;
+  }
+  if (a.pro_mode < PRO_NONE || a.pro_mode > PRO_SPLIT || (a.epi_elu & ~(EPI_ELU | EPI_SPLIT))) {
+    *why = "conv: unknown prologue mode or epilogue bits";
+    return hipErrorInvalidValue;
+  }
+  if (a.pro_mode != PRO_SPLIT) {
+    if (!a.pro_ss) { *why = "conv: prologue scale/shift table missing"; return hipErrorInvalidValue; }
+    if (a.Cin > 1024 && a.ss_bstride == 0) { *why = "conv: identity table holds 1024 channels"; return hipErrorInvalidValue; }
+  }
+  const int opf = (a.pro_mode == PRO_SPLIT ? OPF_IN : 0) | ((a.epi_elu & EPI_SPLIT) ? OPF_OUT : 0);
+  if (opf) {
+    if (mode != MODE_F32X3 || a.io16 || a.s2 || ks != 3 || pool || d != 1 || !a.circular || a.dact || tc != 16) {
+      *why = "conv: operand form needs fp32x3 and a circular 3x3 with d=1 on 8 x 16 pixel tiles";
+      return hipErrorInvalidValue;
+    }
+#ifdef SDP_CONV_BENCH_ONLY
+    *why = "conv: operand form is not built into conv_bench";
+    return hipErrorInvalidValue;
+#else
+    if (opf == OPF_IN) return conv_launch_nj2<MODE_F32X3, false, 4, false, OPF_IN>(a, st);
+    if (opf == (OPF_IN | OPF_OUT)) return conv_launch_nj2<MODE_F32X3, false, 4, false, OPF_IN | OPF_OUT>(a, st);
+    return a.pro_mode == PRO_NONE ? conv_launch_nj2<MODE_F32X3, false, 4, false, OPF_OUT>(a, st)
+                                  : conv_launch_nj2<MODE_F32X3, true, 4, false, OPF_OUT>(a, st);
+#endif
+  }
   if (a.s2) {
     if (!sh16 || a.io16 || ks != 3 || pool || d != 1 || a.circular || a.up || a.pro_mode == PRO_NONE || a.dact ||
         (a.H % 16) || (a.W % 32)) {
diff --git a/simultaneous-diffusion-for-pointclouds_amd/csrc/conv_inst.hip b/simultaneous-diffusion-for-pointclouds_amd/csrc/conv_inst.hip
--- a/simultaneous-diffusion-for-pointclouds_amd/csrc/conv_inst.hip
+++ b/simultaneous-diffusion-for-pointclouds_amd/csrc/conv_inst.hip
@@ -46,7 +46,7 @@
   return hipGetLastError();
 }
 
-template <int MODE, bool PELU, int NW, bool IO16>
+template <int MODE, bool PELU, int NW, bool IO16, int OPF>
 hipError_t conv_launch_nj2(ConvArgs a, hipStream_t st) {
   using T = ConvTile<1, 16, 3, NW, 2, IO16>;
   a.tiles_per_img = a.H * a.W / (T::TR * 16);
@@ -55,8 +55,8 @@
   const bool strip = NW == 8 || SDP_NJ2_STRIP == 2 || (SDP_NJ2_STRIP == 1 && a.cpair);
   a.strip_w = strip ? conv_strip_w(a.H / a.dil / T::TR, a.W / a.dil / 16) : 0;
   dim3 grid(a.B * a.tiles_per_img * (a.cpair ? 2 : 1), a.cpair ? 1 : a.Cout / T::NTILE);
-  hipLaunchKernelGGL((conv_mfma_kernel<MODE, 1, 16, 3, false, false, PELU, 16, NW, false, 2, IO16>), grid, dim3(T::NTH), 0,
-                     st, a);
+  hipLaunchKernelGGL((conv_mfma_kernel<MODE, 1, 16, 3, false, false, PELU, 16, NW, false, 2, IO16, false, OPF>), grid,
+                     dim3(T::NTH), 0, st, a);
   return hipGetLastError();
 }
 
@@ -125,7 +125,11 @@
 template <> struct DgradShape<4> { static constexpr int WM = 1, TC = 32, KS = 3; static constexpr bool ZP = false; };
 template <> struct DgradShape<5> { static constexpr int WM = 1, TC = 16, KS = 3; static constexpr bool ZP = false; };
 
-#if defined(SDP_INST) && SDP_INST >= 4000
+#if defined(SDP_INST) && SDP_INST >= 5000
+constexpr int kPelu = (SDP_INST / 10) % 10, kOpf = SDP_INST % 10;
+static_assert(SDP_INST < 5020 && kOpf >= 1 && kOpf <= 3 && (kPelu == 0 || kOpf == OPF_OUT), "SDP_INST: bad operand-form code");
+template hipError_t conv_launch_nj2<MODE_F32X3, (kPelu != 0), 4, false, kOpf>(ConvArgs, hipStream_t);
+#elif defined(SDP_INST) && SDP_INST >= 4000
 static_assert(SDP_INST - 4000 == MODE_F32X3 || SDP_INST - 4000 == MODE_BF16, "SDP_INST: bad 4x4 stride-2 code");
 template hipError_t conv_launch_s2<SDP_INST - 4000>(ConvArgs, hipStream_t);
 #elif defined(SDP_INST) && SDP_INST >= 3000
diff --git a/simultaneous-diffusion-for-pointclouds_amd/csrc/conv_kernel.h b/simultaneous-diffusion-for-pointclouds_amd/csrc/conv_kernel.h
--- a/simultaneous-diffusion-for-pointclouds_amd/csrc/conv_kernel.h
+++ b/simultaneous-diffusion-for-pointclouds_amd/csrc/conv_kernel.h
@@ -83,7 +83,7 @@
 }
 
 template <int MODE, int WM, int TC, int KS, bool POOL, bool ZP, bool PELU, int SH = 32, int NW = 4, bool TRN = false,
-          int NJ = 4, bool IO16 = false, bool S2 = false>
+          int NJ = 4, bool IO16 = false, bool S2 = false, int OPF = 0>
 __global__ __launch_bounds__(64 * NW, NJ == 2 ? 2 : 1) void conv_mfma_kernel(ConvArgs a) {
 #if defined(__HIP_DEVICE_COMPILE__)
   static_assert(!IO16 || MODE == MODE_BF16, "the bf16 tape runs in bf16 mode");
@@ -91,6 +91,11 @@
   constexpr int CPU = IO16 ? 8 : 4;
   constexpr int USH = IO16 ? 2 : 3;
   constexpr int PPU = CPU / 2;
+  constexpr bool ISPLIT = (OPF & OPF_IN) != 0, OSPLIT = (OPF & OPF_OUT) != 0;
+  static_assert(OPF == 0 || (MODE == MODE_F32X3 && NJ == 2 && NW == 4 && TC == 16 && KS == 3 && !POOL && !ZP && !TRN &&
+                             !IO16 && !S2),
+                "operand form: the fp32x3 16-wide circular 3x3 tiles on 32-Cout waves");
+  static_assert(!ISPLIT || !PELU, "operand-form input carries its prologue already");
   constexpr bool COPY = IO16 && !PELU;
   static_assert((SH == 32) == (MODE == MODE_F32), "bf16 modes: 16x16 shape; exact fp32: 32x32");
   static_assert(NW == 4 || (SH == 16 && !POOL), "2-wave workgroups: the 16x16 non-pooled forward only");
@@ -224,6 +229,7 @@
   float4 ssv[2][PPU];
   auto load_ss = [&](auto buf, int chunk) __attribute__((always_inline)) {
     constexpr int SB = decltype(buf)::value;
+    if constexpr (ISPLIT) return;
     static_for<0, PPU>([&](auto kc) { ssv[SB][kc] = ld4(ssb + (chunk * 32 + my_cv * CPU) * 2 + 4 * decltype(kc)::value); });
   };
 
@@ -266,6 +272,31 @@
     const uint32_t base = (uint32_t)(uintptr_t)(raw + ((tid & ~63) + k * NTH) * 16);
     dma16_lds_opaque(irs_o, base, uoff[k], chunk_soff(chunk));
   };
+  constexpr int SPP = PSTRIDE / 16, NSLOT = T::NPIX * SPP;
+  constexpr int NUD = (NSLOT + NTH - 1) / NTH;
+  constexpr int PBD = T::NPIX * PSTRIDE;
+  static_assert(!ISPLIT || (PSTRIDE % 16 == 0 && 3 * PBD <= T::LDS_BYTES), "three direct-landing patch buffers fit");
+  int uoffd[ISPLIT ? NUD : 1];
+  if constexpr (ISPLIT) {
+    static_for<0, NUD>([&](auto kc) {
+      constexpr int k = decltype(kc)::value;
+      const int U = min(tid + k * NTH, NSLOT - 1);
+      const int pix = U / SPP, cv = min(U - pix * SPP, T::UPP - 1);
+      const int pr = pix / T::PC, pc = pix - pr * T::PC;
+      int sr = sr0 - T::HALO + pr, sc = sc0 - T::HALO + pc;
+      sr = sr < 0 ? sr + Hs : (sr >= Hs ? sr - Hs : sr);
+      sc = sc < 0 ? sc + Ws : (sc >= Ws ? sc - Ws : sc);
+      uoffd[k] = ((sr * a.W + sc) * Cin + cv * CPU) * ES;
+    });
+  }
+  auto load_unit_d = [&](auto kc, int chunk, int buf) __attribute__((always_inline)) {
+    constexpr int k = decltype(kc)::value;
+    if constexpr (SDP_KO & 1) return;
+    if (k < NUD - 1 || tid + k * NTH < NSLOT) {
+      const uint32_t base = (uint32_t)(uintptr_t)(lds + buf * PBD + ((tid & ~63) + k * NTH) * 16);
+      dma16_lds_opaque(irs_o, base, uoffd[k], chunk_soff(chunk));
+    }
+  };
   auto xform_load = [&](auto kc) __attribute__((always_inline)) {
     constexpr int k = decltype(kc)::value;
     return *reinterpret_cast<const float4*>(raw + (tid + k * NTH) * 16);
@@ -370,12 +401,18 @@
   SDP_T(1);
   load_b(std::integral_constant<int, 0>{}, 0, 0);
   static_for<1, NBUF - 1>([&](auto j) { load_b(j, 0, decltype(j)::value); });
-  load_ss(std::integral_constant<int, 0>{}, 0);
-  static_for<0, NU>([&](auto k) { load_unit(k, 0); });
-  static_for<0, NU>([&](auto k) { xform_unit(k, std::integral_constant<int, 0>{}); });
-  if (nchunks > 1) {
-    load_ss(std::integral_constant<int, 1>{}, chunk_cc(1));
-    static_for<0, NU>([&](auto k) { load_unit(k, 1); });
+  if constexpr (ISPLIT) {
+    static_for<0, NUD>([&](auto k) { load_unit_d(k, 0, 0); });
+    static_for<0, NUD>([&](auto k) { load_unit_d(k, 1, 1); });
+    __builtin_amdgcn_s_waitcnt(0);
+  } else {
+    load_ss(std::integral_constant<int, 0>{}, 0);
+    static_for<0, NU>([&](auto k) { load_unit(k, 0); });
+    static_for<0, NU>([&](auto k) { xform_unit(k, std::integral_constant<int, 0>{}); });
+    if (nchunks > 1) {
+      load_ss(std::integral_constant<int, 1>{}, chunk_cc(1));
+      static_for<0, NU>([&](auto k) { load_unit(k, 1); });
+    }
   }
   __syncthreads();
   SDP_T(2);
@@ -538,9 +575,10 @@
     const u32x4 v = __builtin_amdgcn_raw_buffer_load_b128(wrs, wq16[nj], so, 0);
     bq[J][nj >> 1][2 * (nj & 1) + part] = make_uint4(v.x, v.y, v.z, v.w);
   };
-  auto do_chunk9 = [&](auto parity, auto phase_c, int chunk) __attribute__((always_inline)) {
+  using XPC = std::conditional_t<ISPLIT, XformPlan<NUD, NT, 5>, XP>;
+  auto do_chunk9 = [&](auto parity, auto phase_c, int chunk, int rb = 0, int wb = 0) __attribute__((always_inline)) {
     constexpr int P = decltype(parity)::value, PHS = decltype(phase_c)::value;
-    const char* pat = lds + P * T::PATCH_BYTES;
+    const char* pat = lds + (ISPLIT ? rb * PBD : P * T::PATCH_BYTES);
     bf16x8 ca[2][4], cb[2][4];
     static_for<0, 4>([&](auto i) {
       using POS0 = std::integral_constant<int, S2 ? s2_pos(PHS, 0) : 0>;
@@ -554,7 +592,7 @@
       constexpr int CUR = tap % NBUF, NXT = (tap + DIST) % NBUF;
       using POS = std::integral_constant<int, S2 ? s2_pos(PHS, tap) : tap>;
       using POSN = std::integral_constant<int, S2 ? s2_pos(PHS, tap + 1 < NT ? tap + 1 : 0) : tap + 1>;
-      constexpr int U0 = XP::first(tap), UN = XP::count(tap), Q = COPY ? UN : UN * PPU * XP::NSTG;
+      constexpr int U0 = XPC::first(tap), UN = XPC::count(tap), Q = ISPLIT ? 0 : COPY ? UN : UN * PPU * XP::NSTG;
       constexpr int UNA = UN > 0 ? UN : 1;
       const int wchunk = tap + DIST < NT ? chunk : min(chunk + 1, nchunks - 1);
       constexpr int wtap = tap + DIST < NT ? tap + DIST : tap + DIST - NT;
@@ -659,7 +697,7 @@
       static_for<0, NBLK>([&](auto blk_c) {
         constexpr int blk = decltype(blk_c)::value;
         constexpr int s = blk / (4 * NJ), nj = (blk / 4) % NJ, i = blk & 3, mb = 4 * s + i;
-        if constexpr (blk < UN) xr[blk] = xform_load(std::integral_constant<int, U0 + blk>{});
+        if constexpr (!ISPLIT && blk < UN) xr[blk] = xform_load(std::integral_constant<int, U0 + blk>{});
         {
           const uint4 h4 = bq[CUR][nj >> 1][2 * (nj & 1)], l4 = bq[CUR][nj >> 1][2 * (nj & 1) + 1];
           const bf16x8 bhi = *reinterpret_cast<const bf16x8*>(&h4);
@@ -699,8 +737,10 @@
             else stage(std::integral_constant<int, q / XP::NSTG>{}, std::integral_constant<int, q % XP::NSTG>{});
           }
         });
-        if constexpr (UN > 0 && blk >= NBLK - UN)
-          load_unit_o(std::integral_constant<int, U0 + blk - (NBLK - UN)>{}, chunk + 2);
+        if constexpr (UN > 0 && blk >= NBLK - UN) {
+          if constexpr (ISPLIT) load_unit_d(std::integral_constant<int, U0 + blk - (NBLK - UN)>{}, chunk + 2, wb);
+          else load_unit_o(std::integral_constant<int, U0 + blk - (NBLK - UN)>{}, chunk + 2);
+        }
         __builtin_amdgcn_sched_barrier(0);
       });
     });
@@ -724,9 +764,19 @@
     }
   } else if constexpr (MODE != MODE_F32 && NT == 9 && (!TRANS || (IO16 && SDP_DGRAD16_TAPS))) {
     static_assert(XP::max_count() * PPU * XP::NSTG <= 2 * (NBLK - 2), "at most two transform stages per block");
-    for (int chunk = 0; chunk < nchunks; chunk += 2) {
-      do_chunk9(I0{}, I0{}, chunk);
-      do_chunk9(I1{}, I0{}, chunk + 1);
+    if constexpr (ISPLIT) {
+      int rb = 0;
+      for (int chunk = 0; chunk < nchunks; chunk += 2) {
+        do_chunk9(I0{}, I0{}, chunk, rb, rb == 0 ? 2 : rb - 1);
+        rb = rb == 2 ? 0 : rb + 1;
+        do_chunk9(I1{}, I0{}, chunk + 1, rb, rb == 0 ? 2 : rb - 1);
+        rb = rb == 2 ? 0 : rb + 1;
+      }
+    } else {
+      for (int chunk = 0; chunk < nchunks; chunk += 2) {
+        do_chunk9(I0{}, I0{}, chunk);
+        do_chunk9(I1{}, I0{}, chunk + 1);
+      }
     }
   } else {
     for (int chunk = 0; chunk < nchunks; chunk += 2) {
@@ -954,6 +1004,30 @@
         for (int i = 0; i < NV; ++i) __builtin_amdgcn_raw_buffer_store_b32(__float_as_uint(w[i]), r, SDP_EPI16_OFF(i, NJC), AUX);
       }
     };
+    auto store_split = [&](const float (&w)[NV], auto nj_c) __attribute__((always_inline)) {
+      constexpr int NJC = decltype(nj_c)::value;
+      if constexpr (OSPLIT) {
+        constexpr int HP = PER / 2;
+        const bool odd = lane & 1;
+#pragma unroll
+        for (int f = 0; f < NF; ++f) {
+          const int vb = vbase[f] - 2 * lcol + (odd ? HP * xs - 2 : 0);
+#pragma unroll
+          for (int k = 0; k < HP; ++k) {
+            const float mine = odd ? w[f * PER + HP + k] : w[f * PER + k];
+            const float send = odd ? w[f * PER + k] : w[f * PER + HP + k];
+            const float got = __int_as_float(__builtin_amdgcn_mov_dpp(__float_as_int(send), 0xB1, 0xf, 0xf, false));
+            const float c0 = odd ? got : mine, c1 = odd ? mine : got;
+            const __bf16 h0 = (__bf16)c0, h1 = (__bf16)c1;
+            const uint32_t hi = pack_bf2((float)h0, (float)h1);
+            const uint32_t lo = pack_bf2(c0 - (float)h0, c1 - (float)h1);
+            const int so = __builtin_amdgcn_readfirstlane(k * xs + NJC * 32);
+            __builtin_amdgcn_raw_buffer_store_b32(hi, ors, vb, so, SDP_STORE_AUX);
+            __builtin_amdgcn_raw_buffer_store_b32(lo, ors, vb, so + 64, SDP_STORE_AUX);
+          }
+        }
+      }
+    };
     float pre[NJ][NV], biasv[NJ];
     static_for<0, NJ>([&](auto nj) { biasv[nj] = a.bias ? a.bias[n0 + wn * 16 * NJ + nj * 16 + lcol] : 0.f; });
     if (a.res || a.out2) {
@@ -1031,12 +1105,28 @@
         for (int i = 0; i < NV; ++i) r2[i] = v[i] + r2[i];
         store_vals(r2, o2rs, njc, std::integral_constant<int, 0>{});
       }
-      if (a.epi_elu) {
-#pragma unroll
-        for (int i = 0; i < NV; ++i) v[i] = elu(v[i]);
-      }
-      if constexpr (!(SDP_KO & 16))
-        store_vals(v, ors, njc, std::integral_constant<int, IO16 ? SDP_STORE_AUX16 : SDP_STORE_AUX>{});
+      if constexpr (OSPLIT) {
+        float w[NV];
+        if (a.epi_elu & EPI_ELU) {
+#pragma unroll
+          for (int i = 0; i < NV; ++i) w[i] = elu_max(v[i] + 0.0f);
+        } else {
+#pragma unroll
+          for (int i = 0; i < NV; ++i) w[i] = v[i] + 0.0f;
+        }
+        if constexpr (!(SDP_KO & 16)) store_split(w, njc);
+        if ((a.epi_elu & EPI_ELU) && a.stats) {
+#pragma unroll
+          for (int i = 0; i < NV; ++i) v[i] = elu(v[i]);
+        }
+      } else {
+        if (a.epi_elu) {
+#pragma unroll
+          for (int i = 0; i < NV; ++i) v[i] = elu(v[i]);
+        }
+        if constexpr (!(SDP_KO & 16))
+          store_vals(v, ors, njc, std::integral_constant<int, IO16 ? SDP_STORE_AUX16 : SDP_STORE_AUX>{});
+      }
       if (a.stats) {
         float sum = 0.f;
 #pragma unroll
diff --git a/simultaneous-diffusion-for-pointclouds_amd/csrc/conv_launch.h b/simultaneous-diffusion-for-pointclouds_amd/csrc/conv_launch.h
--- a/simultaneous-diffusion-for-pointclouds_amd/csrc/conv_launch.h
+++ b/simultaneous-diffusion-for-pointclouds_amd/csrc/conv_launch.h
@@ -9,7 +9,7 @@
 template <int MODE, bool PELU>
 hipError_t conv_launch_half(ConvArgs a, hipStream_t st);
 
-template <int MODE, bool PELU, int NW, bool IO16 = false>
+template <int MODE, bool PELU, int NW, bool IO16 = false, int OPF = 0>
 hipError_t conv_launch_nj2(ConvArgs a, hipStream_t st);
 
 template <int MODE>
diff --git a/simultaneous-diffusion-for-pointclouds_amd/csrc/kernel_entry.hip b/simultaneous-diffusion-for-pointclouds_amd/csrc/kernel_entry.hip
--- a/simultaneous-diffusion-for-pointclouds_amd/csrc/kernel_entry.hip
+++ b/simultaneous-diffusion-for-pointclouds_amd/csrc/kernel_entry.hip
@@ -112,7 +112,8 @@
 size_t sdpk_wgrad_part_floats(int splits, int Cin, int Cout, int ks) { return wgrad_part_floats(splits, Cin, Cout, ks); }
 
 int sdpk_maxpool5(const void* in, void* out, uint8_t* idx, int B, int H, int W, int C, int h16, void* stream) {
-  return done(maxpool5(F(in), F(out), B, H, W, C, S(stream), idx, h16 != 0), "sdpk_maxpool5");
+  if (h16 < 0 || h16 > 2) return sdp_fail("sdpk_maxpool5: h16 must be 0, 1 or 2");
+  return done(maxpool5(F(in), F(out), B, H, W, C, S(stream), idx, h16), "sdpk_maxpool5");
 }
 
 int sdpk_maxpool5_backward(const uint8_t* idx, const void* dp, const void* res, void* dst, int B, int H, int W, int C,
diff --git a/simultaneous-diffusion-for-pointclouds_amd/csrc/kernels.h b/simultaneous-diffusion-for-pointclouds_amd/csrc/kernels.h
--- a/simultaneous-diffusion-for-pointclouds_amd/csrc/kernels.h
+++ b/simultaneous-diffusion-for-pointclouds_amd/csrc/kernels.h
@@ -13,7 +13,7 @@
 hipError_t inpp_finalize(const float* stats, int B, int T, float cnt, int C, const float* alpha, const float* gamma,
                          const float* beta, float* ss, hipStream_t st, float* nst, void* scratch);
 hipError_t maxpool5(const float* in, float* out, int B, int H, int W, int C, hipStream_t st, uint8_t* idx = nullptr,
-                    bool h16 = false);
+                    int form = 0);
 hipError_t avgpool2(const float* in, float* out, int B, int H, int W, int C, hipStream_t st);
 hipError_t langevin_step(float* x, const float* g, const float* ref, const int32_t* mask, const float* noise,
                          uint64_t seed, uint64_t offset, float step, float nscale, float gref, int n2n, int B, int C,
diff --git a/simultaneous-diffusion-for-pointclouds_amd/csrc/net.hip b/simultaneous-diffusion-for-pointclouds_amd/csrc/net.hip
--- a/simultaneous-diffusion-for-pointclouds_amd/csrc/net.hip
+++ b/simultaneous-diffusion-for-pointclouds_amd/csrc/net.hip
@@ -40,7 +40,12 @@
     bool circular = true;
     bool pool = false;
     bool s2 = false;
+    bool out_split = false;
   };
+
+  bool opf(const Buf& t) const {
+    return net->mode == MODE_F32X3 && net->operand_form && t.C == 256 && t.H % 8 == 0 && t.W % 16 == 0;
+  }
 
   void conv(const Buf& in, const std::string& wkey, const Buf& out, const Opt& o) {
     const auto& hp = net->host.at(wkey + ".weight");
@@ -56,7 +61,7 @@
     a.out2 = o.out2;
     a.res2 = o.res2;
     a.up = o.up;
-    a.pro_ss = o.pro == PRO_AFFINE_ELU ? ss : net->P("#ident_ss");
+    a.pro_ss = o.pro == PRO_AFFINE_ELU ? ss : o.pro == PRO_SPLIT ? nullptr : net->P("#ident_ss");
     a.ss_bstride = o.pro == PRO_AFFINE_ELU ? 2 * in.C : 0;
     a.stats = o.stats ? stats : nullptr;
     a.B = B;
@@ -67,7 +72,7 @@
     a.dil = o.dil;
     a.circular = o.circular ? 1 : 0;
     a.pro_mode = o.pro;
-    a.epi_elu = o.epi_elu ? 1 : 0;
+    a.epi_elu = (o.epi_elu ? EPI_ELU : 0) | (o.out_split ? EPI_SPLIT : 0);
     if ((int)hp.shape[1] != in.C || (int)hp.shape[0] != out.C) throw std::runtime_error("conv shape mismatch " + wkey);
     const char* why = "conv launch";
     const int ks = (int)hp.shape[2];
@@ -120,10 +125,10 @@
           "inpp_finalize");
     });
   }
-  void pool(const Buf& X, const Buf& P) {
+  void pool(const Buf& X, const Buf& P, bool out_split = false) {
     const double bytes = 2.0 * B * X.H * X.W * X.C * 4;
     prof_launch("maxpool5 " + std::to_string(X.C) + " @" + std::to_string(X.H) + "x" + std::to_string(X.W), bytes,
-                [&] { chk(maxpool5(X.p, P.p, B, X.H, X.W, X.C, st), "maxpool5"); });
+                [&] { chk(maxpool5(X.p, P.p, B, X.H, X.W, X.C, st, nullptr, out_split ? 2 : 0), "maxpool5"); });
   }
   static int tiles(const Buf& b) { return b.H * b.W / 128; }
 
@@ -167,15 +172,19 @@
   }
 
   Buf rcu(const std::string& k, Buf x, int nblocks, const Buf& tmp, const Buf& o0, const Buf& o1, bool final_elu,
-          bool final_stats) {
+          bool final_stats, bool split_out = false) {
     Buf outs[2] = {o0, o1};
+    const bool sp = opf(x);
     for (int i = 0; i < nblocks; ++i) {
       Opt a;
       a.pro = PRO_ELU;
       a.bias = false;
+      a.epi_elu = sp;
+      a.out_split = sp;
       conv(x, k + "." + std::to_string(i + 1) + "_1_conv", tmp, a);
       Opt b;
-      b.pro = PRO_ELU;
+      b.pro = sp ? PRO_SPLIT : PRO_ELU;
+      b.out_split = sp && split_out && i == nblocks - 1;
       b.bias = false;
       b.res = x.p;
       b.epi_elu = final_elu && i == nblocks - 1;
@@ -188,14 +197,17 @@
   }
 
   Buf crp(const std::string& k, const Buf& X, const Buf& P, const Buf& Qp, const Buf& R, const Buf& S) {
-    pool(X, P);
+    const bool sp = opf(X);
+    pool(X, P, sp);
     Opt a;
+    a.pro = sp ? PRO_SPLIT : PRO_NONE;
     a.bias = false;
     a.out2 = R.p;
     a.res2 = X.p;
     conv(P, k + ".convs.0", Qp, a);
-    pool(Buf{Qp.p, X.H, X.W, X.C}, P);
+    pool(Buf{Qp.p, X.H, X.W, X.C}, P, sp);
     Opt b;
+    b.pro = sp ? PRO_SPLIT : PRO_NONE;
     b.bias = false;
     b.res = R.p;
     conv(P, k + ".convs.1", S, b);
@@ -247,36 +259,42 @@
   Buf a1 = f.rcu("refine1.adapt_convs.0", L4, 2, QA, QB, QC, true, false);
   Buf x2 = f.crp("refine1.crp", a1, QA, QB, QD, QE);
   Buf ref1 = f.rcu("refine1.output_convs", x2, 1, QA, QB, QC, false, false);
-  Buf hA = f.rcu("refine2.adapt_convs.0", L3, 2, QA, QC, QD, false, false);
-  Buf hB = f.rcu("refine2.adapt_convs.1", ref1, 2, QA, QC, QE, false, false);
+  Buf hA = f.rcu("refine2.adapt_convs.0", L3, 2, QA, QC, QD, false, false, true);
+  Buf hB = f.rcu("refine2.adapt_convs.1", ref1, 2, QA, QC, QE, false, false, true);
   {
     Opt o;
+    o.pro = f.opf(hA) ? PRO_SPLIT : PRO_NONE;
     f.conv(hA, "refine2.msf.convs.0", QA, o);
     Opt o1;
+    o1.pro = o.pro;
     o1.res = QA.p;
     o1.epi_elu = true;
     f.conv(hB, "refine2.msf.convs.1", QB, o1);
   }
   x2 = f.crp("refine2.crp", QB, QA, QC, QD, QE);
   Buf ref2 = f.rcu("refine2.output_convs", x2, 1, QA, QB, QC, false, false);
-  hA = f.rcu("refine3.adapt_convs.0", L2, 2, QA, QC, QD, false, false);
-  hB = f.rcu("refine3.adapt_convs.1", ref2, 2, QA, QC, QE, false, false);
+  hA = f.rcu("refine3.adapt_convs.0", L2, 2, QA, QC, QD, false, false, true);
+  hB = f.rcu("refine3.adapt_convs.1", ref2, 2, QA, QC, QE, false, false, true);
   {
     Opt o;
+    o.pro = f.opf(hA) ? PRO_SPLIT : PRO_NONE;
     f.conv(hA, "refine3.msf.convs.0", half128(QA), o);
     Opt o1;
+    o1.pro = o.pro;
     o1.res = QA.p;
     o1.epi_elu = true;
     f.conv(hB, "refine3.msf.convs.1", half128(QB), o1);
   }
   x2 = f.crp("refine3.crp", half128(QB), half128(QA), half128(QC), half128(QD), half128(QE));
   Buf ref3 = f.rcu("refine3.output_convs", x2, 1, half128(QA), half128(QB), half128(QC), false, false);
-  hA = f.rcu("refine4.adapt_convs.0", L1, 2, FA, FB, FC, false, false);
-  hB = f.rcu("refine4.adapt_convs.1", ref3, 2, half128(QA), half128(QC), half128(QD), false, false);
+  hA = f.rcu("refine4.adapt_convs.0", L1, 2, FA, FB, FC, false, false, true);
+  hB = f.rcu("refine4.adapt_convs.1", ref3, 2, half128(QA), half128(QC), half128(QD), false, false, true);
   {
     Opt o;
+    o.pro = f.opf(hB) ? PRO_SPLIT : PRO_NONE;
     f.conv(hB, "refine4.msf.convs.1", half128(QA), o);
     Opt o1;
+    o1.pro = f.opf(hA) ? PRO_SPLIT : PRO_NONE;
     o1.up = QA.p;
     o1.epi_elu = true;
     f.conv(hA, "refine4.msf.convs.0", FD, o1);
@@ -551,6 +569,12 @@
   return 0;
 }
 
+int sdp_net_set_operand_form(sdp_net* net, int on) {
+  if (!net || on < 0 || on > 1) return fail("sdp_net_set_operand_form: on must be 0 or 1");
+  net->operand_form = on != 0;
+  return 0;
+}
+
 int sdp_net_profile_enable(sdp_net* net, int enable) {
   if (!net) return fail("sdp_net_profile_enable: null net");
   net->profile = enable != 0;
diff --git a/simultaneous-diffusion-for-pointclouds_amd/csrc/net_internal.h b/simultaneous-diffusion-for-pointclouds_amd/csrc/net_internal.h
--- a/simultaneous-diffusion-for-pointclouds_amd/csrc/net_internal.h
+++ b/simultaneous-diffusion-for-pointclouds_amd/csrc/net_internal.h
@@ -55,6 +55,7 @@
   int mode = sdp::MODE_F32X3;
   sdp::TrainPlan* plan = nullptr;
   int split = 0;
+  bool operand_form = true;
   hipStream_t aux_stream[sdp::SDP_MAX_SPLIT - 1] = {};
   hipEvent_t ev_fork = nullptr, ev_join[sdp::SDP_MAX_SPLIT - 1] = {};
 
diff --git a/simultaneous-diffusion-for-pointclouds_amd/sdp/_lib.py b/simultaneous-diffusion-for-pointclouds_amd/sdp/_lib.py
--- a/simultaneous-diffusion-for-pointclouds_amd/sdp/_lib.py
+++ b/simultaneous-diffusion-for-pointclouds_amd/sdp/_lib.py
@@ -43,6 +43,7 @@
     "sdp_net_forward": (I, [P, P, P, P, I, P, SZ, P]),
     "sdp_net_forward_langevin": (I, [P, P, P, I, C.POINTER(LangevinParams), P, SZ, P]),
     "sdp_net_set_split": (I, [P, I]),
+    "sdp_net_set_operand_form": (I, [P, I]),
     "sdp_net_set_tape": (I, [P, I]),
     "sdp_net_destroy": (I, [P]),
     "sdp_net_profile_enable": (I, [P, I]),
diff --git a/simultaneous-diffusion-for-pointclouds_amd/sdp/scorenet.py b/simultaneous-diffusion-for-pointclouds_amd/sdp/scorenet.py
--- a/simultaneous-diffusion-for-pointclouds_amd/sdp/scorenet.py
+++ b/simultaneous-diffusion-for-pointclouds_amd/sdp/scorenet.py
@@ -108,6 +108,9 @@
         _lib.check(_lib.lib().sdp_net_set_split(self._h, int(ways)), "set_split")
         self._ws.clear()
 
+    def set_operand_form(self, on: bool):
+        _lib.check(_lib.lib().sdp_net_set_operand_form(self._h, 1 if on else 0), "set_operand_form")
+
     def set_tape(self, bf16: bool):
         _lib.check(_lib.lib().sdp_net_set_tape(self._h, 1 if bf16 else 0), "set_tape")
 
```

Result: no change. 376.0 image-steps/s (median of 6 runs) (+0.1%).
